# CV-Project2025/Project-NeRF

Measured on AMD Instinct MI355X. Metric: train rays/sec + 800x800 render FPS, NeRF-Synthetic Lego; PSNR parity, higher is better.
Workload: dtype bf16; 1 GPU; Part 2 vanilla NeRF train step (L10/L4 Fourier, 8x256 skip-4 MLP, view 128), batch sampling included; rays_per_gpu=4096, samples_per_ray=64, global_rays=4096, parallelism=ray-dp1, weights=random init (seed 0), frames=100 x 800x800 RGBA resident in HBM (uniform noise)

## Files before the change

### include/nerf_hip.h

```cpp
#ifndef NERF_HIP_H
#define NERF_HIP_H

#include <stddef.h>
#include <stdint.h>

#ifdef __cplusplus
extern "C" {
#endif

#define NERF_OK 0
#define NERF_EINVAL (-22)
#define NERF_ELAUNCH (-5)
#define NERF_ENOSYS (-38)

#define NERF_ABI_VERSION 12

typedef void* nerf_stream_t;

const char* nerf_last_error(void);
int nerf_abi_version(void);

int nerf_set_option(const char* name, int value);
int nerf_get_option(const char* name, int* value_out);

int nerf_sample_rays(const float* rays_o, const float* rays_d, const float* u,
                     int64_t n_rays, int n_samples, float near_plane, float far_plane,
                     float* z_out, float* pts_out, float* dirs_out, nerf_stream_t stream);

int nerf_gather_rays(const float* images, const float* poses, const int64_t* img_idx, const int64_t* pix_y,
                     const int64_t* pix_x, int64_t batch, int n_images, int H, int W, float focal,
                     float scene_scale, float* rays_o, float* rays_d, float* rgba, nerf_stream_t stream);

int nerf_gather_batch(const float* images, const float* poses, const int64_t* flat_idx, int64_t batch, int n_images,
                      int H, int W, float focal, float scene_scale, const float* bg, float* rays_o, float* rays_d,
                      float* rgba, float* target, nerf_stream_t stream);

int nerf_train_batch(const float* images, const float* poses, int n_images, int H, int W, float focal,
                     float scene_scale, const float* bg, uint64_t seed, uint64_t counter, int64_t batch,
                     int n_samples, float near_plane, float far_plane, int perturb, float* rays_o, float* rays_d,
                     float* rgba, float* target, float* z_out, nerf_stream_t stream);

int nerf_train_batch_shard(const float* images, const float* poses, int n_images, int H, int W, float focal,
                     float scene_scale, const float* bg, uint64_t seed, uint64_t counter, int64_t first_ray, int64_t batch,
                     int n_samples, float near_plane, float far_plane, int perturb, float* rays_o, float* rays_d,
                     float* rgba, float* target, float* z_out, nerf_stream_t stream);

int nerf_active_mask(const float* pts, int64_t n, const uint8_t* binary_grid, int resolution,
                     float bound, uint8_t* mask_out, int64_t* idx_out, nerf_stream_t stream);

int nerf_sample_compact(const float* rays_o, const float* rays_d, const float* u, int64_t n_rays,
                        int n_samples, float near_plane, float far_plane, const uint8_t* binary_grid,
                        int resolution, float bound, float* z_out, int* slot_of_sample, float* pts_compact,
                        float* dirs_compact, unsigned* active_count, nerf_stream_t stream);
int nerf_sample_compact_jitter(const float* rays_o, const float* rays_d, uint64_t seed, uint64_t counter,
                               int64_t n_rays, int n_samples, float near_plane, float far_plane,
                               const uint8_t* binary_grid, int resolution, float bound, float* z_out,
                               int* slot_of_sample, float* pts_compact, float* dirs_compact,
                               unsigned* active_count, nerf_stream_t stream);
int nerf_sample_compact_jitter_shard(const float* rays_o, const float* rays_d, uint64_t seed, uint64_t counter,
                                     int64_t first_ray, int64_t n_rays, int n_samples, float near_plane, float far_plane,
                                     const uint8_t* binary_grid, int resolution, float bound, float* z_out,
                                     int* slot_of_sample, float* pts_compact, float* dirs_compact,
                                     unsigned* active_count, nerf_stream_t stream);
#define NERF_COMPACT_CHAIN_WORDS 40
int nerf_sample_compact_jitter_chain(const float* rays_o, const float* rays_d, uint64_t seed, uint64_t counter,
                                     int64_t first_ray, int64_t n_rays, int n_samples, float near_plane, float far_plane,
                                     const uint8_t* binary_grid, int resolution, float bound, float* z_out,
                                     int* slot_of_sample, float* pts_compact, float* dirs_compact,
// ... 41 lines not shown
                        nerf_stream_t stream);

int nerf_composite_fwd(const float* rgb, const float* sigma, const float* z, const float* rays_d,
                       const float* bg, int64_t bg_rows, const float* extra,
                       int64_t n_rays, int n_samples,
                       float* out_rgb, float* out_depth, float* out_acc,
                       float* extra_map, float* weights_out, nerf_stream_t stream);

int nerf_composite_bwd(const float* rgb, const float* sigma, const float* z, const float* rays_d,
                       const float* bg, int64_t bg_rows, const float* extra,
                       const float* g_rgb, const float* g_depth, const float* g_acc,
                       const float* g_extra, int64_t n_rays, int n_samples,
                       float* d_rgb, float* d_sigma, float* d_extra, nerf_stream_t stream);

int nerf_composite_fwd_indexed(const float* rgb_compact, const float* sigma_compact, const int* slot_of_sample,
                               const float* z, const float* rays_d, const float* bg, int64_t bg_rows,
                               int64_t n_rays, int n_samples, float* out_rgb, float* out_depth,
                               float* out_acc, nerf_stream_t stream);
int nerf_composite_bwd_indexed(const float* rgb_compact, const float* sigma_compact, const int* slot_of_sample,
                               const float* z, const float* rays_d, const float* bg, int64_t bg_rows,
                               const float* g_rgb, const float* g_depth, const float* g_acc, int64_t n_rays,
                               int n_samples, float* d_rgb_compact, float* d_sigma_compact,
                               nerf_stream_t stream);

#define NERF_MLP_PARAM_COUNT 595844

size_t nerf_mlp_packed_bytes(void);
int nerf_mlp_pack(const float* params_f32, void* packed, nerf_stream_t stream);
int nerf_mlp_pack_streams(const float* params_f32, void* packed, int which, nerf_stream_t stream);

size_t nerf_mlp_stash_bytes(int64_t n);
int nerf_mlp_fwd(const void* packed, const float* rays_o, const float* rays_d, const float* z,
                 int64_t n, int n_samples, float* rgb, float* sigma, void* stash,
                 nerf_stream_t stream);

int nerf_mlp_fwd_encoded(const void* packed, const float* x_enc, const float* d_enc, int64_t n, float* rgb,
                         float* sigma, void* stash, nerf_stream_t stream);

size_t nerf_mlp_bwd_workspace_bytes(int64_t n);
int nerf_mlp_bwd(const void* packed, const void* stash, const float* rgb, const float* sigma,
                 const float* d_rgb, const float* d_sigma, int64_t n, float* grads_f32,
                 void* workspace, nerf_stream_t stream);
int nerf_mlp_bwd_dgrad(const void* packed, const void* stash, const float* rgb, const float* sigma,
                       const float* d_rgb, const float* d_sigma, int64_t n, void* workspace,
                       nerf_stream_t stream);
int nerf_mlp_bwd_dgrad_ex(const void* packed, const void* stash, const float* rgb, const float* sigma,
                          const float* d_rgb, const float* d_sigma, int64_t n, void* workspace,
                          const float* amax_dev, nerf_stream_t stream);
int64_t nerf_mlp_wgrad_part_split(void);
int nerf_mlp_bwd_wgrad_part(const void* stash, const void* workspace, int64_t n, float* grads_f32, int part,
                            nerf_stream_t stream);
int nerf_mlp_bwd_wgrad(const void* stash, const void* workspace, int64_t n, float* grads_f32,
                       nerf_stream_t stream);

int nerf_hash_encode_fwd(const float* pts, int64_t n, const float* table, int n_levels,
                         const float* scale_host, const unsigned* res_host, const unsigned* size_host,
                         const unsigned* offset_host, const unsigned* dense_host, float bound,
                         float* out_f32, void* out_nat_bf16, unsigned* idx_out, nerf_stream_t stream);
int nerf_hash_encode_fwd_f16(const float* pts, int64_t n, const void* table_f16, int n_levels,
                         const float* scale_host, const unsigned* res_host, const unsigned* size_host,
                         const unsigned* offset_host, const unsigned* dense_host, float bound,
                         float* out_f32, void* out_nat_bf16, nerf_stream_t stream);
int nerf_hash_encode_fwd_nat(const float* pts, int64_t n, const float* table_f32, const void* table_f16, int n_levels,
                             const float* scale_host, const unsigned* res_host, const unsigned* size_host,
                             const unsigned* offset_host, const unsigned* dense_host, float bound,
                             void* out_nat, int nat_dtype, nerf_stream_t stream);
int nerf_hash_encode_fwd_nat_tables(const float* pts, int64_t n, const void* tables_f16, int n_tables, int64_t table_stride,
                                    int n_levels, const float* scale_host, const unsigned* res_host, const unsigned* size_host,
                                    const unsigned* offset_host, const unsigned* dense_host, float bound, void* out_nat,
                                    int64_t out_stride_bytes, int nat_dtype, nerf_stream_t stream);
int nerf_f32_to_f16(const float* src, void* dst_f16, int64_t n, nerf_stream_t stream);
int nerf_hash_encode_bwd(const float* pts, int64_t n, int n_levels, const float* scale_host,
                         const unsigned* res_host, const unsigned* size_host, const unsigned* offset_host,
                         const unsigned* dense_host, float bound, const float* d_feat, float* d_table,
                         nerf_stream_t stream);
int nerf_hash_encode_bwd_levels(const float* pts, int64_t n, int n_levels, const float* scale_host,
                         const unsigned* res_host, const unsigned* size_host, const unsigned* offset_host,
                         const unsigned* dense_host, float bound, const float* d_feat, float* d_table, int first_level, int end_level,
                         nerf_stream_t stream);
size_t nerf_hash_encode_bwd_workspace_bytes(int64_t n, int n_levels);
int nerf_hash_encode_bwd_ws(const float* pts, int64_t n, int n_levels, const float* scale_host,
                         const unsigned* res_host, const unsigned* size_host, const unsigned* offset_host,
                         const unsigned* dense_host, float bound, const float* d_feat, float* d_table, int first_level, int end_level,
                         void* workspace, size_t workspace_bytes, nerf_stream_t stream);
int nerf_hash_encode_bwd_ws_store(const float* pts, int64_t n, int n_levels, const float* scale_host,
                                  const unsigned* res_host, const unsigned* size_host, const unsigned* offset_host,
                                  const unsigned* dense_host, float bound, const float* d_feat, float* d_table,
                                  int first_level, int end_level, void* workspace, size_t workspace_bytes,
                                  nerf_stream_t stream);
size_t nerf_hash_encode_bwd_tables_workspace_bytes(int64_t n, int n_levels, int n_tables);
int nerf_hash_encode_bwd_ws_store_tables(const float* pts, int64_t n, int n_tables, int64_t table_stride, int n_levels,
                                         const float* scale_host, const unsigned* res_host, const unsigned* size_host,
                                         const unsigned* offset_host, const unsigned* dense_host, float bound,
                                         const float* d_feat, int64_t dfeat_stride, float* d_table, void* workspace,
                                         size_t workspace_bytes, nerf_stream_t stream);
int nerf_hash_encode_bwd_ws_store_tables_spec(const float* pts, int64_t n, int n_tables, int64_t table_stride, int n_levels,
                                              const float* scale_host, const unsigned* res_host, const unsigned* size_host,
                                              const unsigned* offset_host, const unsigned* dense_host, float bound,
                                              const float* d_feat, int64_t dfeat_stride, float* d_table, void* workspace,
                                              size_t workspace_bytes, void* status_host, nerf_stream_t stream);
int nerf_hash_encode_fwd_f16_hist(const float* pts, int64_t n, const void* table_f16, int n_levels,
                                  const float* scale_host, const unsigned* res_host, const unsigned* size_host,
                                  const unsigned* offset_host, const unsigned* dense_host, float bound,
                                  void* out_nat_bf16, void* bwd_workspace, size_t bwd_workspace_bytes, nerf_stream_t stream);
#define NERF_AMAX_WORDS 32
int nerf_hash_encode_bwd_ws_slots(void* workspace, int64_t n, int n_levels, void** amax_bits_out, void** grad_lm_out);
// ... 21 lines not shown
int nerf_hash_encode_bwd_input_f16_accum(const float* pts, int64_t n, const void* table_f16, int n_levels,
                                         const float* scale_host, const unsigned* res_host, const unsigned* size_host,
                                         const unsigned* offset_host, const unsigned* dense_host, float bound,
                                         const float* d_feat, float* d_pts, nerf_stream_t stream);
int nerf_hash_encode_bwd_input_lm_f16(const float* pts, int64_t n, const void* table_f16, int n_levels,
                                      const float* scale_host, const unsigned* res_host, const unsigned* size_host,
                                      const unsigned* offset_host, const unsigned* dense_host, float bound,
                                      const void* grad_lm, float* d_pts, int accumulate, nerf_stream_t stream);


size_t nerf_imlp_packed_bytes(void);
size_t nerf_imlp_workspace_bytes(int64_t n);
size_t nerf_imlp_hash_operand_offset(int64_t n);
int nerf_imlp_pack(const float* params_f32, void* packed, nerf_stream_t stream);
int nerf_imlp_fwd(const void* packed, void* workspace, const float* dirs, int64_t n, float* rgb,
                  float* sigma, int train, nerf_stream_t stream);
int nerf_imlp_fwd_encoded(const void* packed, void* workspace, const float* x_enc, const float* d_enc, int64_t n,
                          float* rgb, float* sigma, int train, nerf_stream_t stream);
int nerf_imlp_bwd(const void* packed, void* workspace, const float* rgb, const float* sigma,
                  const float* d_rgb, const float* d_sigma, int64_t n, float* grads_f32,
                  float* d_feat, nerf_stream_t stream);
int nerf_imlp_bwd_lm(const void* packed, void* workspace, const float* rgb, const float* sigma,
                     const float* d_rgb, const float* d_sigma, int64_t n, float* grads_f32,
                     void* grad_lm, void* amax_bits, nerf_stream_t stream);

size_t nerf_render_rays_workspace_bytes(int64_t chunk_rays, int n_samples);
int nerf_render_rays_fwd(const void* packed, const float* rays_o, const float* rays_d, int64_t n_rays,
                         int n_samples, float near_plane, float far_plane, const float* bg, int64_t bg_rows,
                         int64_t chunk_rays, void* workspace, float* out_rgb, float* out_depth, float* out_acc,
                         nerf_stream_t stream);

size_t nerf_instant_render_workspace_bytes(int64_t chunk_rays, int n_samples);
int nerf_instant_render_rays_fwd(const void* imlp_packed, const float* table_f32, const void* table_f16, int n_levels,
                                 const float* scale_host, const unsigned* res_host, const unsigned* size_host,
                                 const unsigned* offset_host, const unsigned* dense_host, float hash_bound,
                                 const uint8_t* binary_grid, int grid_resolution, float grid_bound,
                                 const float* rays_o, const float* rays_d, int64_t n_rays, int n_samples,
                                 float near_plane, float far_plane, const float* bg, int64_t bg_rows,
                                 int64_t chunk_rays, void* workspace, float* out_rgb, float* out_depth, float* out_acc,
                                 nerf_stream_t stream);

size_t nerf_render_rays_grid_workspace_bytes(int64_t chunk_rays, int n_samples);
int nerf_render_rays_grid_fwd(const void* packed, const uint8_t* binary_grid, int grid_resolution, float grid_bound,
                              const float* rays_o, const float* rays_d, int64_t n_rays, int n_samples,
                              float near_plane, float far_plane, const float* bg, int64_t bg_rows,
                              int64_t chunk_rays, void* workspace, float* out_rgb, float* out_depth, float* out_acc,
                              nerf_stream_t stream);

#define NERF_SUM_WS_FLOATS 12288
int nerf_composite_mse_bwd(const float* rgb, const float* sigma, const int* slot_of_sample, const float* z,
                           const float* rays_d, const float* bg, int64_t bg_rows, const float* target,
                           float loss_weight, int64_t n_rays, int n_samples, float* pred_out, float* loss_accum,
                           float* d_rgb, float* d_sigma, float* amax_accum, float* sum_ws, nerf_stream_t stream);
int nerf_composite_mse_reg_bwd(const float* rgb, const float* sigma, const int* slot_of_sample, const float* z,
                               const float* rays_d, const float* bg, int64_t bg_rows, const float* target,
                               float loss_weight, const float* extra, float reg_weight, int64_t n_rays, int n_samples,
                               float* pred_out, float* extra_map, float* loss_accum, float* reg_accum, float* d_rgb,
                               float* d_sigma, float* d_extra, float* sum_ws, nerf_stream_t stream);

int nerf_adam_step(float* params, const float* grads, float* exp_avg, float* exp_avg_sq,
                   int64_t n, int step, float lr, float beta1, float beta2, float eps,
                   float weight_decay, const float* grad_scale_dev, nerf_stream_t stream);

#define NERF_NORMSQ_WS_FLOATS 4136
int nerf_tv_normsq(const float* params, float* grads, int64_t n, float tv_weight, float grad_scale,
                   float* normsq_dev, nerf_stream_t stream);
int nerf_tv_normsq_accum(const float* params, float* grads, int64_t n, float tv_weight, float grad_scale,
                         float* normsq_dev, nerf_stream_t stream);
int nerf_tv_normsq_accum_tables(const float* params, float* grads, int64_t n, int n_tables, float tv_weight, float grad_scale,
                                float* normsq_dev, nerf_stream_t stream);
int nerf_adamw_clip_step(float* params, const float* grads, float* exp_avg, float* exp_avg_sq, int64_t n,
                         int step, float lr, float beta1, float beta2, float eps, float weight_decay,
                         const float* normsq_dev, float max_norm, float grad_scale, nerf_stream_t stream);
int nerf_adamw_clip_step_shadow(float* params, const float* grads, float* exp_avg, float* exp_avg_sq, int64_t n,
                         int step, float lr, float beta1, float beta2, float eps, float weight_decay,
                         const float* normsq_dev, float max_norm, float grad_scale, void* params_f16_out, nerf_stream_t stream);

size_t nerf_tv_codes_bytes(int64_t n);
int nerf_tv_normsq_codes(const float* params, const float* grads, int64_t n, int n_tables, float tv_weight, float grad_scale,
                         float* normsq_dev, int accumulate, void* tv_codes, nerf_stream_t stream);
int nerf_adamw_clip_step_tv(float* params, const float* grads, float* exp_avg, float* exp_avg_sq, int64_t n, int step, float lr,
                            float beta1, float beta2, float eps, float weight_decay, const float* normsq_dev, float max_norm,
                            float grad_scale, const void* tv_codes, int64_t tv_split, float tv_weight_lo, int64_t seg_lo,
                            float tv_weight_hi, int64_t seg_hi, int64_t lr_split, float lr_hi, void* params_f16_out,
                            nerf_stream_t stream);

int nerf_tv_normsq_codes_piece(const float* params, const float* grads, int64_t n, int64_t table_elems, int halo, float tv_weight,
                               float grad_scale, float* normsq_dev, int accumulate, void* tv_codes, nerf_stream_t stream);
int nerf_adamw_clip_step_tv_piece(float* params, const float* grads, float* exp_avg, float* exp_avg_sq, int64_t n, int step, float lr,
                                  float beta1, float beta2, float eps, float weight_decay, const float* normsq_dev, float max_norm,
                                  float grad_scale, const void* tv_codes, float tv_weight, int64_t table_elems, int halo_lo,
                                  void* params_f16_out, nerf_stream_t stream);

int nerf_clip_adamw_small(float* params, float* grads, float* exp_avg, float* exp_avg_sq, int64_t n, int step, float lr, float beta1,
                          float beta2, float eps, float weight_decay, float max_norm, float grad_scale, float* normsq_out,
                          int zero_grads, nerf_stream_t stream);

int64_t nerf_p4_param_count(void);
size_t nerf_p4_packed_bytes(void);
size_t nerf_p4_workspace_bytes(int64_t n);
size_t nerf_p4_infer_workspace_bytes(int64_t n);
size_t nerf_p4_workspace_offset(int64_t n, int which);
int nerf_p4_pack(const float* params_f32, void* packed, nerf_stream_t stream);
int nerf_p4_sample_inputs(const int* slot_of_sample, const float* pts_compact, const float* ray_times, int64_t n_rays,
                          int n_samples, float coord_noise_std, float time_noise_std, uint64_t seed, uint64_t counter,
                          int64_t first_ray, float* x_deform, float* t_deform, nerf_stream_t stream);
int nerf_p4_deform_fwd(const void* packed, const float* params_f32, void* workspace, const float* pts, const float* t_deform,
                       const float* blend, int64_t n, float* delta_x, float* x_canonical, int train, nerf_stream_t stream);
int nerf_p4_canon_fwd(const void* packed, void* workspace, const float* t_deform, const float* dirs, int64_t n, float* rgb,
                      float* sigma, int train, nerf_stream_t stream);
int nerf_p4_canon_bwd(const void* packed, void* workspace, const float* rgb, const float* sigma, const float* d_rgb,
                      const float* d_sigma, int64_t n, float* grads_f32, void* amax_bits, void* grad_lm, nerf_stream_t stream);
int nerf_p4_deform_bwd(const void* packed, const float* params_f32, void* workspace, const float* d_delta_x, int64_t n,
                       float* grads_f32, void* amax_bits, void* grad_lm, nerf_stream_t stream);

// ... 58 lines not shown
```

### project-nerf_amd/_lib.py

```python
import ctypes
import os

_HERE = os.path.dirname(os.path.abspath(__file__))
LIB_PATH = os.path.join(_HERE, "libnerf_hip.so")

c_f32p = ctypes.c_void_p
c_ptr = ctypes.c_void_p
i64 = ctypes.c_int64
i32 = ctypes.c_int
f32 = ctypes.c_float
size_t = ctypes.c_size_t

PROTOTYPES = {
    "nerf_last_error": (ctypes.c_char_p, []),
    "nerf_abi_version": (i32, []),
    "nerf_set_option": (i32, [ctypes.c_char_p, i32]),
    "nerf_get_option": (i32, [ctypes.c_char_p, ctypes.POINTER(i32)]),
    "nerf_sample_rays": (i32, [c_ptr, c_ptr, c_ptr, i64, i32, f32, f32, c_ptr, c_ptr, c_ptr, c_ptr]),
    "nerf_gather_rays": (i32, [c_ptr, c_ptr, c_ptr, c_ptr, c_ptr, i64, i32, i32, i32, f32, f32, c_ptr, c_ptr, c_ptr, c_ptr]),
    "nerf_gather_batch": (i32, [c_ptr, c_ptr, c_ptr, i64, i32, i32, i32, f32, f32, c_ptr, c_ptr, c_ptr, c_ptr, c_ptr, c_ptr]),
    "nerf_train_batch": (i32, [c_ptr, c_ptr, i32, i32, i32, f32, f32, c_ptr, ctypes.c_uint64, ctypes.c_uint64, i64, i32, f32, f32,
                               i32, c_ptr, c_ptr, c_ptr, c_ptr, c_ptr, c_ptr]),
    "nerf_train_batch_shard": (i32, [c_ptr, c_ptr, i32, i32, i32, f32, f32, c_ptr, ctypes.c_uint64, ctypes.c_uint64, i64, i64, i32, f32, f32,
                                     i32, c_ptr, c_ptr, c_ptr, c_ptr, c_ptr, c_ptr]),
    "nerf_active_mask": (i32, [c_ptr, i64, c_ptr, i32, f32, c_ptr, c_ptr, c_ptr]),
    "nerf_sample_compact": (i32, [c_ptr, c_ptr, c_ptr, i64, i32, f32, f32, c_ptr, i32, f32, c_ptr, c_ptr, c_ptr, c_ptr, c_ptr, c_ptr]),
    "nerf_sample_compact_jitter": (i32, [c_ptr, c_ptr, ctypes.c_uint64, ctypes.c_uint64, i64, i32, f32, f32, c_ptr, i32, f32,
                                         c_ptr, c_ptr, c_ptr, c_ptr, c_ptr, c_ptr]),
    "nerf_sample_compact_jitter_shard": (i32, [c_ptr, c_ptr, ctypes.c_uint64, ctypes.c_uint64, i64, i64, i32, f32, f32, c_ptr, i32, f32,
                                               c_ptr, c_ptr, c_ptr, c_ptr, c_ptr, c_ptr]),
    "nerf_sample_compact_jitter_chain": (i32, [c_ptr, c_ptr, ctypes.c_uint64, ctypes.c_uint64, i64, i64, i32, f32, f32, c_ptr, i32, f32,
                                               c_ptr, c_ptr, c_ptr, c_ptr, c_ptr, i32, c_ptr, ctypes.c_uint32, c_ptr]),
    "nerf_train_batch_compact": (i32, [c_ptr, c_ptr, i32, i32, i32, f32, f32, c_ptr, ctypes.c_uint64, ctypes.c_uint64, i64, i64, i32, f32, f32,
                                       c_ptr, i32, f32, c_ptr, c_ptr, c_ptr, c_ptr, c_ptr, c_ptr, c_ptr, c_ptr, c_ptr, c_ptr]),
    "nerf_train_batch_compact_chain": (i32, [c_ptr, c_ptr, i32, i32, i32, f32, f32, c_ptr, ctypes.c_uint64, ctypes.c_uint64, i64, i64, i32, f32,
                                             f32, c_ptr, i32, f32, c_ptr, c_ptr, c_ptr, c_ptr, c_ptr, c_ptr, c_ptr, c_ptr, c_ptr, i32, c_ptr,
                                             ctypes.c_uint32, c_ptr]),
    "nerf_composite_fwd_indexed": (i32, [c_ptr, c_ptr, c_ptr, c_ptr, c_ptr, c_ptr, i64, i64, i32, c_ptr, c_ptr, c_ptr, c_ptr]),
    "nerf_composite_bwd_indexed": (i32, [c_ptr, c_ptr, c_ptr, c_ptr, c_ptr, c_ptr, i64, c_ptr, c_ptr, c_ptr, i64, i32, c_ptr, c_ptr, c_ptr]),
    "nerf_sample_pdf": (i32, [c_ptr, c_ptr, c_ptr, i64, i32, i32, c_ptr, c_ptr]),
    "nerf_grid_lattice": (i32, [f32, i32, c_ptr, c_ptr]),
    "nerf_grid_update": (i32, [c_ptr, c_ptr, c_ptr, i64, f32, i32, f32, c_ptr, c_ptr]),
    "nerf_instant_grid_update_workspace_bytes": (size_t, [i64]),
    "nerf_instant_grid_update": (i32, [c_ptr, c_ptr, c_ptr, i32, c_ptr, c_ptr, c_ptr, c_ptr, c_ptr, f32, c_ptr, i64, i32, f32, c_ptr, c_ptr, f32, i32,
                                       f32, c_ptr, i64, c_ptr, c_ptr]),
    "nerf_fourier_encode": (i32, [c_ptr, i64, i32, i32, c_ptr, c_ptr]),
    "nerf_composite_fwd": (i32, [c_ptr, c_ptr, c_ptr, c_ptr, c_ptr, i64, c_ptr, i64, i32,
                                 c_ptr, c_ptr, c_ptr, c_ptr, c_ptr, c_ptr]),
    "nerf_composite_bwd": (i32, [c_ptr, c_ptr, c_ptr, c_ptr, c_ptr, i64, c_ptr, c_ptr, c_ptr, c_ptr,
                                 c_ptr, i64, i32, c_ptr, c_ptr, c_ptr, c_ptr]),
    "nerf_render_rays_workspace_bytes": (size_t, [i64, i32]),
    "nerf_render_rays_fwd": (i32, [c_ptr, c_ptr, c_ptr, i64, i32, f32, f32, c_ptr, i64, i64, c_ptr, c_ptr, c_ptr, c_ptr, c_ptr]),
    "nerf_instant_render_workspace_bytes": (size_t, [i64, i32]),
    "nerf_instant_render_rays_fwd": (i32, [c_ptr, c_ptr, c_ptr, i32, c_ptr, c_ptr, c_ptr, c_ptr, c_ptr, f32, c_ptr, i32, f32, c_ptr, c_ptr, i64, i32,
                                           f32, f32, c_ptr, i64, i64, c_ptr, c_ptr, c_ptr, c_ptr, c_ptr]),
    "nerf_render_rays_grid_workspace_bytes": (size_t, [i64, i32]),
    "nerf_render_rays_grid_fwd": (i32, [c_ptr, c_ptr, i32, f32, c_ptr, c_ptr, i64, i32, f32, f32, c_ptr, i64, i64, c_ptr, c_ptr, c_ptr, c_ptr,
                                        c_ptr]),
    "nerf_mlp_packed_bytes": (size_t, []),
    "nerf_mlp_pack": (i32, [c_ptr, c_ptr, c_ptr]),
    "nerf_mlp_pack_streams": (i32, [c_ptr, c_ptr, i32, c_ptr]),
    "nerf_mlp_stash_bytes": (size_t, [i64]),
    "nerf_mlp_fwd": (i32, [c_ptr, c_ptr, c_ptr, c_ptr, i64, i32, c_ptr, c_ptr, c_ptr, c_ptr]),
    "nerf_mlp_fwd_encoded": (i32, [c_ptr, c_ptr, c_ptr, i64, c_ptr, c_ptr, c_ptr, c_ptr]),
    "nerf_mlp_bwd_workspace_bytes": (size_t, [i64]),
    "nerf_mlp_bwd": (i32, [c_ptr, c_ptr, c_ptr, c_ptr, c_ptr, c_ptr, i64, c_ptr, c_ptr, c_ptr]),
    "nerf_mlp_bwd_dgrad": (i32, [c_ptr, c_ptr, c_ptr, c_ptr, c_ptr, c_ptr, i64, c_ptr, c_ptr]),
    "nerf_mlp_bwd_wgrad": (i32, [c_ptr, c_ptr, i64, c_ptr, c_ptr]),
    "nerf_mlp_bwd_dgrad_ex": (i32, [c_ptr, c_ptr, c_ptr, c_ptr, c_ptr, c_ptr, i64, c_ptr, c_ptr, c_ptr]),
    "nerf_composite_mse_bwd": (i32, [c_ptr, c_ptr, c_ptr, c_ptr, c_ptr, c_ptr, i64, c_ptr, f32, i64, i32, c_ptr, c_ptr,
                                     c_ptr, c_ptr, c_ptr, c_ptr, c_ptr]),
    "nerf_mlp_wgrad_part_split": (i64, []),
    "nerf_mlp_bwd_wgrad_part": (i32, [c_ptr, c_ptr, i64, c_ptr, i32, c_ptr]),
    "nerf_hash_encode_fwd": (i32, [c_ptr, i64, c_ptr, i32, c_ptr, c_ptr, c_ptr, c_ptr, c_ptr, f32, c_ptr, c_ptr, c_ptr, c_ptr]),
    "nerf_hash_encode_fwd_f16": (i32, [c_ptr, i64, c_ptr, i32, c_ptr, c_ptr, c_ptr, c_ptr, c_ptr, f32, c_ptr, c_ptr, c_ptr]),
    "nerf_hash_encode_fwd_nat": (i32, [c_ptr, i64, c_ptr, c_ptr, i32, c_ptr, c_ptr, c_ptr, c_ptr, c_ptr, f32, c_ptr, i32, c_ptr]),
    "nerf_hash_encode_fwd_nat_tables": (i32, [c_ptr, i64, c_ptr, i32, i64, i32, c_ptr, c_ptr, c_ptr, c_ptr, c_ptr, f32, c_ptr, i64, i32, c_ptr]),
    "nerf_f32_to_f16": (i32, [c_ptr, c_ptr, i64, c_ptr]),
    "nerf_hash_encode_bwd": (i32, [c_ptr, i64, i32, c_ptr, c_ptr, c_ptr, c_ptr, c_ptr, f32, c_ptr, c_ptr, c_ptr]),
    "nerf_hash_encode_bwd_levels": (i32, [c_ptr, i64, i32, c_ptr, c_ptr, c_ptr, c_ptr, c_ptr, f32, c_ptr, c_ptr, i32, i32, c_ptr]),
    "nerf_hash_encode_bwd_workspace_bytes": (size_t, [i64, i32]),
    "nerf_hash_encode_bwd_ws": (i32, [c_ptr, i64, i32, c_ptr, c_ptr, c_ptr, c_ptr, c_ptr, f32, c_ptr, c_ptr, i32, i32, c_ptr, size_t, c_ptr]),
    "nerf_hash_encode_bwd_ws_store": (i32, [c_ptr, i64, i32, c_ptr, c_ptr, c_ptr, c_ptr, c_ptr, f32, c_ptr, c_ptr, i32, i32, c_ptr, size_t, c_ptr]),
    "nerf_hash_encode_bwd_tables_workspace_bytes": (size_t, [i64, i32, i32]),
    "nerf_hash_encode_bwd_ws_store_tables": (i32, [c_ptr, i64, i32, i64, i32, c_ptr, c_ptr, c_ptr, c_ptr, c_ptr, f32, c_ptr, i64, c_ptr, c_ptr, size_t, c_ptr]),
    "nerf_hash_encode_bwd_ws_store_tables_spec": (i32, [c_ptr, i64, i32, i64, i32, c_ptr, c_ptr, c_ptr, c_ptr, c_ptr, f32, c_ptr, i64, c_ptr, c_ptr, size_t,
                                                        c_ptr, c_ptr]),
    "nerf_hash_encode_fwd_f16_hist": (i32, [c_ptr, i64, c_ptr, i32, c_ptr, c_ptr, c_ptr, c_ptr, c_ptr, f32, c_ptr, c_ptr, size_t, c_ptr]),
    "nerf_hash_encode_bwd_ws_slots": (i32, [c_ptr, i64, i32, ctypes.POINTER(c_ptr), ctypes.POINTER(c_ptr)]),
    "nerf_hash_encode_bwd_ws_store_precounted": (i32, [c_ptr, i64, i32, c_ptr, c_ptr, c_ptr, c_ptr, c_ptr, f32, c_ptr, c_ptr, size_t, c_ptr]),
    "nerf_hash_encode_bwd_spec_begin": (i32, [c_ptr, c_ptr]),
    "nerf_hash_encode_bwd_ws_store_spec": (i32, [c_ptr, i64, i32, c_ptr, c_ptr, c_ptr, c_ptr, c_ptr, f32, c_ptr, c_ptr, c_ptr, size_t, c_ptr, c_ptr]),
    "nerf_imlp_bwd_amax": (i32, [c_ptr, c_ptr, c_ptr, c_ptr, c_ptr, c_ptr, i64, c_ptr, c_ptr, c_ptr, c_ptr]),
    "nerf_hash_encode_bwd_spec_status": (c_ptr, [c_ptr]),
    "nerf_imlp_bwd_lm": (i32, [c_ptr, c_ptr, c_ptr, c_ptr, c_ptr, c_ptr, i64, c_ptr, c_ptr, c_ptr, c_ptr]),
    "nerf_hash_encode_bwd_input": (i32, [c_ptr, i64, c_ptr, i32, c_ptr, c_ptr, c_ptr, c_ptr, c_ptr, f32, c_ptr, c_ptr, c_ptr]),
    "nerf_hash_encode_bwd_input_f16": (i32, [c_ptr, i64, c_ptr, i32, c_ptr, c_ptr, c_ptr, c_ptr, c_ptr, f32, c_ptr, c_ptr, c_ptr]),
    "nerf_hash_encode_bwd_input_f16_accum": (i32, [c_ptr, i64, c_ptr, i32, c_ptr, c_ptr, c_ptr, c_ptr, c_ptr, f32, c_ptr, c_ptr, c_ptr]),
    "nerf_hash_encode_bwd_input_lm_f16": (i32, [c_ptr, i64, c_ptr, i32, c_ptr, c_ptr, c_ptr, c_ptr, c_ptr, f32, c_ptr, c_ptr, i32, c_ptr]),
    "nerf_imlp_packed_bytes": (size_t, []),
    "nerf_imlp_workspace_bytes": (size_t, [i64]),
    "nerf_imlp_hash_operand_offset": (size_t, [i64]),
    "nerf_imlp_pack": (i32, [c_ptr, c_ptr, c_ptr]),
    "nerf_imlp_fwd": (i32, [c_ptr, c_ptr, c_ptr, i64, c_ptr, c_ptr, i32, c_ptr]),
    "nerf_imlp_fwd_encoded": (i32, [c_ptr, c_ptr, c_ptr, c_ptr, i64, c_ptr, c_ptr, i32, c_ptr]),
    "nerf_imlp_bwd": (i32, [c_ptr, c_ptr, c_ptr, c_ptr, c_ptr, c_ptr, i64, c_ptr, c_ptr, c_ptr]),
    "nerf_adam_step": (i32, [c_ptr, c_ptr, c_ptr, c_ptr, i64, i32, f32, f32, f32, f32, f32, c_ptr, c_ptr]),
    "nerf_tv_normsq": (i32, [c_ptr, c_ptr, i64, f32, f32, c_ptr, c_ptr]),
    "nerf_tv_normsq_accum": (i32, [c_ptr, c_ptr, i64, f32, f32, c_ptr, c_ptr]),
    "nerf_tv_normsq_accum_tables": (i32, [c_ptr, c_ptr, i64, i32, f32, f32, c_ptr, c_ptr]),
    "nerf_composite_mse_reg_bwd": (i32, [c_ptr, c_ptr, c_ptr, c_ptr, c_ptr, c_ptr, i64, c_ptr, f32, c_ptr, f32, i64, i32, c_ptr, c_ptr,
                                         c_ptr, c_ptr, c_ptr, c_ptr, c_ptr, c_ptr, c_ptr]),
    "nerf_sample_compact_ordered_scratch_bytes": (size_t, [i64, i32]),
    "nerf_sample_compact_ordered": (i32, [c_ptr, c_ptr, c_ptr, i32, ctypes.c_uint64, ctypes.c_uint64, i64, i64, i32, f32, f32, c_ptr, i32, f32,
                                          c_ptr, c_ptr, c_ptr, c_ptr, c_ptr, c_ptr, size_t, c_ptr]),
    "nerf_p4_param_count": (i64, []),
    "nerf_p4_packed_bytes": (size_t, []),
    "nerf_p4_workspace_bytes": (size_t, [i64]),
    "nerf_p4_infer_workspace_bytes": (size_t, [i64]),
    "nerf_p4_workspace_offset": (size_t, [i64, i32]),
    "nerf_p4_pack": (i32, [c_ptr, c_ptr, c_ptr]),
    "nerf_p4_sample_inputs": (i32, [c_ptr, c_ptr, c_ptr, i64, i32, f32, f32, ctypes.c_uint64, ctypes.c_uint64, i64, c_ptr, c_ptr, c_ptr]),
    "nerf_p4_deform_fwd": (i32, [c_ptr, c_ptr, c_ptr, c_ptr, c_ptr, c_ptr, i64, c_ptr, c_ptr, i32, c_ptr]),
    "nerf_p4_canon_fwd": (i32, [c_ptr, c_ptr, c_ptr, c_ptr, i64, c_ptr, c_ptr, i32, c_ptr]),
    "nerf_p4_canon_bwd": (i32, [c_ptr, c_ptr, c_ptr, c_ptr, c_ptr, c_ptr, i64, c_ptr, c_ptr, c_ptr, c_ptr]),
    "nerf_p4_deform_bwd": (i32, [c_ptr, c_ptr, c_ptr, c_ptr, i64, c_ptr, c_ptr, c_ptr, c_ptr]),
    "nerf_p3_deform_param_count": (i64, []),
    "nerf_p3_deform_packed_bytes": (size_t, []),
    "nerf_p3_deform_workspace_bytes": (size_t, [i64]),
    "nerf_p3_deform_pack": (i32, [c_ptr, c_ptr, c_ptr]),
    "nerf_p3_deform_fwd": (i32, [c_ptr, c_ptr, c_ptr, c_ptr, c_ptr, i64, c_ptr, c_ptr, i32, c_ptr]),
    "nerf_p3_deform_bwd": (i32, [c_ptr, c_ptr, c_ptr, i64, c_ptr, c_ptr]),
    "nerf_p3_canon_param_count": (i64, [i32]),
    "nerf_p3_canon_packed_bytes": (size_t, []),
    "nerf_p3_canon_workspace_bytes": (size_t, [i64]),
    "nerf_p3_canon_pack": (i32, [c_ptr, i32, c_ptr, c_ptr]),
    "nerf_p3_canon_fwd": (i32, [c_ptr, c_ptr, c_ptr, c_ptr, c_ptr, i64, c_ptr, c_ptr, i32, c_ptr]),
    "nerf_p3_canon_bwd": (i32, [c_ptr, c_ptr, c_ptr, c_ptr, c_ptr, c_ptr, c_ptr, i64, i32, c_ptr, c_ptr, c_ptr]),
    "nerf_p1_param_count": (i64, [i32, i32, i32, i32]),
    "nerf_p1_packed_bytes": (size_t, [i32, i32, i32, i32]),
    "nerf_p1_workspace_bytes": (size_t, [i64, i32, i32, i32, i32]),
    "nerf_p1_pack": (i32, [c_ptr, i32, i32, i32, i32, c_ptr, c_ptr]),
    "nerf_p1_fwd": (i32, [c_ptr, c_ptr, i64, i32, i32, i32, i32, c_ptr, c_ptr]),
    "nerf_p1_fwd_loss_bwd": (i32, [c_ptr, c_ptr, c_ptr, c_ptr, c_ptr, i64, i32, i32, i32, i32, c_ptr, c_ptr, c_ptr]),
    "nerf_p2_param_count": (i64, [i32] * 6),
    "nerf_p2_packed_bytes": (size_t, [i32] * 6),
    "nerf_p2_workspace_bytes": (size_t, [i64] + [i32] * 6),
    "nerf_p2_pack": (i32, [c_ptr] + [i32] * 6 + [c_ptr, c_ptr]),
    "nerf_p2_fwd": (i32, [c_ptr, c_ptr, c_ptr, c_ptr, i64, i32] + [i32] * 6 + [c_ptr, c_ptr, c_ptr]),
    "nerf_p2_fwd_train": (i32, [c_ptr, c_ptr, c_ptr, c_ptr, c_ptr, i64, i32] + [i32] * 6 + [c_ptr, c_ptr, c_ptr]),
    "nerf_p2_bwd": (i32, [c_ptr, c_ptr, c_ptr, c_ptr, c_ptr, c_ptr, i64] + [i32] * 6 + [c_ptr, c_ptr]),
    "nerf_imlp_shape_param_count": (i64, [i32] * 3),
    "nerf_imlp_shape_packed_bytes": (size_t, [i32] * 3),
    "nerf_imlp_shape_workspace_bytes": (size_t, [i64] + [i32] * 3),
    "nerf_imlp_shape_hash_operand_offset": (size_t, [i64] + [i32] * 3),
    "nerf_imlp_shape_pack": (i32, [c_ptr] + [i32] * 3 + [c_ptr, c_ptr]),
    "nerf_imlp_shape_fwd": (i32, [c_ptr, c_ptr, c_ptr, i64] + [i32] * 3 + [c_ptr, c_ptr, i32, c_ptr]),
    "nerf_imlp_shape_bwd": (i32, [c_ptr, c_ptr, c_ptr, c_ptr, c_ptr, c_ptr, i64] + [i32] * 3 + [c_ptr, c_ptr, c_ptr]),
    "nerf_tv_codes_bytes": (size_t, [i64]),
    "nerf_tv_normsq_codes": (i32, [c_ptr, c_ptr, i64, i32, f32, f32, c_ptr, i32, c_ptr, c_ptr]),
    "nerf_clip_adamw_small": (i32, [c_ptr, c_ptr, c_ptr, c_ptr, i64, i32, f32, f32, f32, f32, f32, f32, f32, c_ptr, i32, c_ptr]),
    "nerf_adamw_clip_step_tv": (i32, [c_ptr, c_ptr, c_ptr, c_ptr, i64, i32, f32, f32, f32, f32, f32, c_ptr, f32, f32, c_ptr, i64, f32, i64,
                                      f32, i64, i64, f32, c_ptr, c_ptr]),
    "nerf_tv_normsq_codes_piece": (i32, [c_ptr, c_ptr, i64, i64, i32, f32, f32, c_ptr, i32, c_ptr, c_ptr]),
    "nerf_adamw_clip_step_tv_piece": (i32, [c_ptr, c_ptr, c_ptr, c_ptr, i64, i32, f32, f32, f32, f32, f32, c_ptr, f32, f32, c_ptr, f32, i64, i32,
                                            c_ptr, c_ptr]),
    "nerf_adamw_clip_step": (i32, [c_ptr, c_ptr, c_ptr, c_ptr, i64, i32, f32, f32, f32, f32, f32, c_ptr, f32, f32, c_ptr]),
    "nerf_adamw_clip_step_shadow": (i32, [c_ptr, c_ptr, c_ptr, c_ptr, i64, i32, f32, f32, f32, f32, f32, c_ptr, f32, f32, c_ptr, c_ptr]),
}

ABI_VERSION = 12

_lib = None


class NerfHipError(RuntimeError):
    pass


def load():
    global _lib
    if _lib is not None:
        return _lib
    if not os.path.exists(LIB_PATH):
        raise NerfHipError(
            f"{LIB_PATH} not found: build it with `python project-nerf_amd/build.py` "
            "(hipcc --offload-arch=gfx950).  There is no fallback path.")
    import torch
    lib = ctypes.CDLL(LIB_PATH, mode=ctypes.RTLD_GLOBAL)
    for name, (res, args) in PROTOTYPES.items():
        fn = getattr(lib, name)
        fn.restype = res
        fn.argtypes = args
    if lib.nerf_abi_version() != ABI_VERSION:
        raise NerfHipError(f"ABI version mismatch: {LIB_PATH} reports {lib.nerf_abi_version()}, this binding was written against "
                           f"{ABI_VERSION} (rebuild with `python project-nerf_amd/build.py`)")
    _lib = lib
    return lib


NORMSQ_WS_FLOATS = 4136
COMPACT_CHAIN_WORDS = 40
SUM_WS_FLOATS = 12288


def set_option(name: str, value: int) -> None:
    check(load().nerf_set_option(name.encode(), int(value)), f"nerf_set_option({name})")


def get_option(name: str) -> int:
    out = i32(0)
    check(load().nerf_get_option(name.encode(), ctypes.byref(out)), f"nerf_get_option({name})")
    return out.value


def check(code, what):
    if code != 0:
        msg = load().nerf_last_error().decode("utf-8", "replace")
        raise NerfHipError(f"{what} failed ({code}): {msg}")
```

### project-nerf_amd/csrc/adam.hip

```cpp
#include "common.h"

namespace nerf {

typedef float f4 __attribute__((ext_vector_type(4)));

__device__ __forceinline__ void adam_update(float& p, float g, float& m, float& v, float lr, float beta1, float beta2,
                                            float eps, float wd, float inv_bc1, float inv_sqrt_bc2) {
  float pi = p;
  if (wd != 0.0f) pi *= (1.0f - lr * wd);
  const float mi = beta1 * m + (1.0f - beta1) * g;
  const float vi = beta2 * v + (1.0f - beta2) * g * g;
  m = mi;
  v = vi;
  p = pi - (lr * inv_bc1) * (mi / (sqrtf(vi) * inv_sqrt_bc2 + eps));
}

template <bool VEC>
__device__ __forceinline__ void adam_sweep(float* __restrict__ p, const float* __restrict__ g, float* __restrict__ m,
                                           float* __restrict__ v, int64_t n, float gs, float lr, float beta1, float beta2,
                                           float eps, float wd, float inv_bc1, float inv_sqrt_bc2, _Float16* __restrict__ shadow = nullptr) {
  const int64_t tid = blockIdx.x * (int64_t)blockDim.x + threadIdx.x, stride = (int64_t)gridDim.x * blockDim.x;
  const int64_t n4 = VEC ? n / 4 : 0;
  for (int64_t i = tid; i < n4; i += stride) {
    f4 pp = reinterpret_cast<f4*>(p)[i], mm = reinterpret_cast<f4*>(m)[i], vv = reinterpret_cast<f4*>(v)[i];
    const f4 gg = reinterpret_cast<const f4*>(g)[i];
#pragma unroll
    for (int e = 0; e < 4; ++e) {
      float pe = pp[e], me = mm[e], ve = vv[e];
      adam_update(pe, gg[e] * gs, me, ve, lr, beta1, beta2, eps, wd, inv_bc1, inv_sqrt_bc2);
      pp[e] = pe; mm[e] = me; vv[e] = ve;
    }
    reinterpret_cast<f4*>(m)[i] = mm;
    reinterpret_cast<f4*>(v)[i] = vv;
    reinterpret_cast<f4*>(p)[i] = pp;
    if (shadow != nullptr) {
      typedef _Float16 h4 __attribute__((ext_vector_type(4)));
      h4 hh = {(_Float16)pp[0], (_Float16)pp[1], (_Float16)pp[2], (_Float16)pp[3]};
      reinterpret_cast<h4*>(shadow)[i] = hh;
    }
  }
  for (int64_t i = 4 * n4 + tid; i < n; i += stride) {
    adam_update(p[i], g[i] * gs, m[i], v[i], lr, beta1, beta2, eps, wd, inv_bc1, inv_sqrt_bc2);
    if (shadow != nullptr) shadow[i] = (_Float16)p[i];
  }
}

template <bool VEC>
__global__ void __launch_bounds__(256)
adam_kernel(float* __restrict__ p, const float* __restrict__ g, float* __restrict__ m,
            float* __restrict__ v, int64_t n, float lr, float beta1, float beta2, float eps, float wd,
            float inv_bc1, float inv_sqrt_bc2, const float* __restrict__ grad_scale) {
  adam_sweep<VEC>(p, g, m, v, n, grad_scale ? *grad_scale : 1.0f, lr, beta1, beta2, eps, wd, inv_bc1, inv_sqrt_bc2);
}

__host__ inline bool aligned16(const void* a, const void* b, const void* c, const void* d) {
  return (((uintptr_t)a | (uintptr_t)b | (uintptr_t)c | (uintptr_t)d) & 15) == 0;
}

}

extern "C" int nerf_adam_step(float* params, const float* grads, float* exp_avg, float* exp_avg_sq,
                              int64_t n, int step, float lr, float beta1, float beta2, float eps,
                              float weight_decay, const float* grad_scale_dev, nerf_stream_t stream) {
  NERF_REQUIRE(n >= 0 && step >= 1, "nerf_adam_step: n=%lld step=%d", (long long)n, step);
  if (n == 0) return NERF_OK;
  NERF_REQUIRE(params && grads && exp_avg && exp_avg_sq, "nerf_adam_step: NULL pointer");
  const double bc1 = 1.0 - pow((double)beta1, step), bc2 = 1.0 - pow((double)beta2, step);
  int64_t blocks = (n / 4 + 255) / 256 + 1;
  if (blocks > 2048) blocks = 2048;
  if (nerf::aligned16(params, grads, exp_avg, exp_avg_sq))
    hipLaunchKernelGGL(nerf::adam_kernel<true>, dim3((int)blocks), dim3(256), 0, nerf::as_stream(stream), params,
                       grads, exp_avg, exp_avg_sq, n, lr, beta1, beta2, eps, weight_decay,
                       (float)(1.0 / bc1), (float)(1.0 / sqrt(bc2)), grad_scale_dev);
  else
    hipLaunchKernelGGL(nerf::adam_kernel<false>, dim3((int)blocks), dim3(256), 0, nerf::as_stream(stream), params,
                       grads, exp_avg, exp_avg_sq, n, lr, beta1, beta2, eps, weight_decay,
                       (float)(1.0 / bc1), (float)(1.0 / sqrt(bc2)), grad_scale_dev);
  return nerf::check_launch("nerf_adam_step");
}

namespace nerf {

__device__ __forceinline__ float sgn(float x) { return (x > 0.0f) - (x < 0.0f); }

__device__ __forceinline__ float tv_term(float prev, float cur, float next, bool has_prev, bool has_next) {
  float t = 0.0f;
  if (has_prev) t += sgn(cur - prev);
  if (has_next) t -= sgn(next - cur);
  return t;
}

template <bool VEC>
__global__ void __launch_bounds__(256)
tv_normsq_kernel(const float* __restrict__ p, float* __restrict__ g, int64_t n, float tv_scale, float grad_scale,
                 float* __restrict__ normsq, int64_t seg) {
  auto starts = [seg](int64_t e) { return e == 0 || e == seg || e == 2 * seg || e == 3 * seg; };
  const bool rewrite = tv_scale != 0.0f || grad_scale != 1.0f;
  float local = 0.0f;
  const int64_t tid = blockIdx.x * (int64_t)blockDim.x + threadIdx.x, stride = (int64_t)gridDim.x * blockDim.x;
  const int64_t n4 = VEC ? n / 4 : 0;
  for (int64_t i = tid; i < n4; i += stride) {
    f4 gg = reinterpret_cast<f4*>(g)[i];
    gg[0] *= grad_scale; gg[1] *= grad_scale; gg[2] *= grad_scale; gg[3] *= grad_scale;
    if (tv_scale != 0.0f) {
      const f4 pp = reinterpret_cast<const f4*>(p)[i];
      const int64_t e0 = 4 * i;
      const bool has_prev = !starts(e0), has_next = e0 + 4 < n && !starts(e0 + 4);
      const float before = has_prev ? p[e0 - 1] : 0.0f, after = has_next ? p[e0 + 4] : 0.0f;
      gg[0] += tv_scale * tv_term(before, pp[0], pp[1], has_prev, true);
      gg[1] += tv_scale * tv_term(pp[0], pp[1], pp[2], true, true);
      gg[2] += tv_scale * tv_term(pp[1], pp[2], pp[3], true, true);
      gg[3] += tv_scale * tv_term(pp[2], pp[3], after, true, has_next);
    }
    if (rewrite) reinterpret_cast<f4*>(g)[i] = gg;
    local += gg[0] * gg[0] + gg[1] * gg[1] + gg[2] * gg[2] + gg[3] * gg[3];
  }
  for (int64_t i = 4 * n4 + tid; i < n; i += stride) {
    float gi = g[i] * grad_scale;
    if (tv_scale != 0.0f) {
      const bool has_prev = !starts(i), has_next = i + 1 < n && !starts(i + 1);
      gi += tv_scale * tv_term(has_prev ? p[i - 1] : 0.0f, p[i], has_next ? p[i + 1] : 0.0f, has_prev, has_next);
    }
    if (rewrite) g[i] = gi;
    local += gi * gi;
  }
  __shared__ float part[4];
  local = wave_sum(local);
  if ((threadIdx.x & 63) == 0) part[threadIdx.x >> 6] = local;
  __syncthreads();
  const float val[1] = {(part[0] + part[1]) + (part[2] + part[3])};
// ... 445 lines not shown
```

### project-nerf_amd/csrc/api.cpp

```cpp
#include <stdlib.h>
#include <string.h>
#include <mutex>
#include "common.h"

namespace nerf {
static thread_local char g_err[512] = "";

int fail(int code, const char* fmt, ...) {
  va_list ap;
  va_start(ap, fmt);
  vsnprintf(g_err, sizeof(g_err), fmt, ap);
  va_end(ap);
  return code;
}

struct OptionSlot { const char* name; const char* env; int Options::*field; };
static const OptionSlot kSlots[] = {
    {"chain_legacy", "NERF_CHAIN_LEGACY", &Options::chain_legacy},
    {"fwd_cycles", "NERF_FWD_CYCLES", &Options::fwd_cycles},
    {"wgrad_overhead", "NERF_WGRAD_OVH", &Options::wgrad_overhead},
    {"wgrad_bw_x16", "NERF_WGRAD_BW", &Options::wgrad_bw_x16},
    {"wgrad_fixed", "NERF_WGRAD_FIXED", &Options::wgrad_fixed},
    {"wgrad_debug", "NERF_WGRAD_DEBUG", &Options::wgrad_debug},
    {"wgrad_small_span", "NERF_WGRAD_SMALL_SPAN", &Options::wgrad_small_span},
    {"wgrad_small_cap", "NERF_WGRAD_SMALL_CAP", &Options::wgrad_small_cap},
    {"wgrad_only", "NERF_WGRAD_ONLY", &Options::wgrad_only},
    {"hash_bwd_only_level", "NERF_HASH_BWD_ONLY_LEVEL", &Options::hash_bwd_only_level},
    {"hash_bwd_atomic", "NERF_HASH_BWD_ATOMIC", &Options::hash_bwd_atomic},
    {"wgrad_atomic", "NERF_WGRAD_ATOMIC", &Options::wgrad_atomic},
    {"wgrad_k16", "NERF_WGRAD_K16", &Options::wgrad_k16},
    {"wgrad_big_only", "NERF_WGRAD_BIG_ONLY", &Options::wgrad_big_only},
    {"infer_shape32", "NERF_INFER_SHAPE32", &Options::infer_shape32},
    {"infer64", "NERF_INFER64", &Options::infer64},
    {"stash_fp8", "NERF_STASH_FP8", &Options::stash_fp8},
    {"chain_grid", "NERF_CHAIN_GRID", &Options::chain_grid},
    {"wgrad_grid", "NERF_WGRAD_GRID", &Options::wgrad_grid},
    {"hash_fwd_lds_kb", "NERF_HASH_FWD_LDS_KB", &Options::hash_fwd_lds_kb},
    {"hash_xcd", "NERF_HASH_XCD", &Options::hash_xcd},
    {"composite_wgs_per_cu", "NERF_COMPOSITE_WGS", &Options::composite_wgs_per_cu},
    {"deterministic", "NERF_DETERMINISTIC", &Options::deterministic},
    {"tv_blocks", "NERF_TV_BLOCKS", &Options::tv_blocks},
};

Options& options() {
  static Options o;
  static std::once_flag once;
  std::call_once(once, [] {
    for (const OptionSlot& s : kSlots)
      if (const char* v = getenv(s.env)) o.*(s.field) = (*v == 0) ? 1 : atoi(v);
  });
  return o;
}

namespace {
constexpr int kMaxDevices = 64, kMaxKernels = 64;
struct DeviceFacts {
  int n_cu = 0;
  int n_kernels = 0;
  const void* kernels[kMaxKernels];
};
DeviceFacts g_dev[kMaxDevices];
std::mutex g_dev_mutex;
}

int device_cu_count(int* n_cu) {
  int dev = 0;
  if (hipGetDevice(&dev) != hipSuccess || dev < 0 || dev >= kMaxDevices) return fail(NERF_ELAUNCH, "cannot query the current device");
  std::lock_guard<std::mutex> lock(g_dev_mutex);
  if (g_dev[dev].n_cu == 0) {
    hipDeviceProp_t prop;
    if (hipGetDeviceProperties(&prop, dev) != hipSuccess) return fail(NERF_ELAUNCH, "cannot query device %d", dev);
    g_dev[dev].n_cu = prop.multiProcessorCount;
  }
  *n_cu = g_dev[dev].n_cu;
  return NERF_OK;
}

int ensure_dynamic_lds(const void* kernel, int bytes, const char* what) {
  int dev = 0;
  if (hipGetDevice(&dev) != hipSuccess || dev < 0 || dev >= kMaxDevices) return fail(NERF_ELAUNCH, "cannot query the current device");
  std::lock_guard<std::mutex> lock(g_dev_mutex);
  DeviceFacts& d = g_dev[dev];
  for (int i = 0; i < d.n_kernels; ++i)
    if (d.kernels[i] == kernel) return NERF_OK;
  if (hipFuncSetAttribute(kernel, hipFuncAttributeMaxDynamicSharedMemorySize, bytes) != hipSuccess)
    return fail(NERF_ELAUNCH, "%s: cannot raise the dynamic LDS limit to %d on device %d", what, bytes, dev);
  if (d.n_kernels < kMaxKernels) d.kernels[d.n_kernels++] = kernel;
  return NERF_OK;
}
}

extern "C" const char* nerf_last_error(void) { return nerf::g_err; }
extern "C" int nerf_abi_version(void) { return NERF_ABI_VERSION; }

// ... 20 lines not shown
```

### project-nerf_amd/csrc/common.h

```cpp
#pragma once
#include <hip/hip_runtime.h>
#include <stdarg.h>
#include <stdint.h>
#include <stdio.h>
#include "../../include/nerf_hip.h"

namespace nerf {

constexpr int kWave = 64;

int fail(int code, const char* fmt, ...);

inline int check_launch(const char* what) {
  hipError_t e = hipGetLastError();
  if (e != hipSuccess) return fail(NERF_ELAUNCH, "%s: %s", what, hipGetErrorString(e));
  return NERF_OK;
}

inline hipStream_t as_stream(nerf_stream_t s) { return reinterpret_cast<hipStream_t>(s); }

struct Options {
  int chain_legacy = 0;
  int fwd_cycles = 0;
  int wgrad_overhead = 98304;
  int wgrad_bw_x16 = 192;
  int wgrad_fixed = 2000;
  int wgrad_debug = 0;
  int wgrad_small_span = 32;
  int wgrad_small_cap = 3;
  int wgrad_only = -1;
  int hash_bwd_only_level = -1;
  int wgrad_big_only = 0;
  int wgrad_k16 = 0;
  int wgrad_atomic = 0;
  int hash_bwd_atomic = 0;
  int infer_shape32 = 0;
  int infer64 = 1;
  int stash_fp8 = 0;
  int chain_grid = 0;
  int wgrad_grid = 0;
  int composite_wgs_per_cu = 2;
  int hash_xcd = 1;
  int hash_fwd_lds_kb = 36;
  int tv_blocks = 0;
  int deterministic = 0;
};
Options& options();

int device_cu_count(int* n_cu);
int ensure_dynamic_lds(const void* kernel, int bytes, const char* what);

int hash_fwd_counted(const float* pts, const unsigned* count, int64_t capacity, const float* table_f32, const void* table_f16,
                     int n_levels, const float* scale_host, const unsigned* res_host, const unsigned* size_host,
                     const unsigned* offset_host, const unsigned* dense_host, float bound, void* out_nat, nerf_stream_t stream);
int imlp_fwd_counted(const void* packed, const void* hash_nat, const float* dirs, const unsigned* count, int64_t capacity, float* rgb,
                     float* sigma, nerf_stream_t stream);
int hash_fwd_lattice(int64_t cell0, int64_t n_cells, int resolution, float grid_bound, const float* table_f32, const void* table_f16,
                     int n_levels, const float* scale_host, const unsigned* res_host, const unsigned* size_host,
                     const unsigned* offset_host, const unsigned* dense_host, float bound, void* out_nat, nerf_stream_t stream);
int imlp_sigma_grid(const void* packed, const void* hash_nat, int64_t n_cells, float* grid, uint8_t* binary_grid, float decay, int dynamic,
                    float threshold, unsigned long long* active_count, nerf_stream_t stream);
int mlp_fwd_counted(const void* packed, const float* pts, const float* dirs, const unsigned* count, int64_t capacity, float* rgb,
                    float* sigma, nerf_stream_t stream);

#define NERF_REQUIRE(cond, ...) \
  do {                          \
    if (!(cond)) return ::nerf::fail(NERF_EINVAL, __VA_ARGS__); \
  } while (0)

__device__ __forceinline__ uint32_t squares32(uint64_t ctr, uint64_t key) {
  uint64_t x = ctr * key, y = x, z = y + key;
  x = x * x + y; x = (x >> 32) | (x << 32);
  x = x * x + z; x = (x >> 32) | (x << 32);
  x = x * x + y; x = (x >> 32) | (x << 32);
  return (uint32_t)((x * x + z) >> 32);
}

inline uint64_t squares_key(uint64_t seed) {
  uint64_t key = seed + 0x9E3779B97F4A7C15ull;
  key = (key ^ (key >> 30)) * 0xBF58476D1CE4E5B9ull;
  key = (key ^ (key >> 27)) * 0x94D049BB133111EBull;
  return (key ^ (key >> 31)) | 1ull;
}
__device__ __forceinline__ float squares_uniform(uint64_t counter, uint64_t index, uint64_t key) {
  return (float)(squares32((counter << 40) + index, key) >> 8) * 5.9604644775390625e-08f;
}

__device__ __forceinline__ float mul_rn(float a, float b) {
#pragma clang fp contract(off)
  return a * b;
}
__device__ __forceinline__ float add_rn(float a, float b) {
#pragma clang fp contract(off)
  return a + b;
}
__device__ __forceinline__ float sub_rn(float a, float b) {
#pragma clang fp contract(off)
// ... 111 lines not shown
```

### project-nerf_amd/csrc/composite.hip

```cpp
#include "common.h"

namespace nerf {

constexpr int kMaxPerLane = 16;

template <int K>
struct RayCtx {
  float e[K];
  float alpha[K];
  float q[K];
  float T[K];
  float z[K];
  float delta[K];
};

__device__ __forceinline__ int64_t row_of(const int* __restrict__ slots, int64_t dense_index) {
  return slots == nullptr ? dense_index : (int64_t)slots[dense_index];
}

template <int K>
__device__ __forceinline__ void ray_setup(const float* __restrict__ sigma, const float* __restrict__ z,
                                          const float* __restrict__ rays_d, const int* __restrict__ slots,
                                          int64_t r, int S, int lane, RayCtx<K>& c, float* sig_out, int64_t* row_out) {
  const float dx = rays_d[r * 3 + 0], dy = rays_d[r * 3 + 1], dz = rays_d[r * 3 + 2];
  const float dnorm = sqrtf(dx * dx + dy * dy + dz * dz);
  const int s0 = lane * K;
  float zn[K + 1];
#pragma unroll
  for (int k = 0; k <= K; ++k) {
    const int s = s0 + k;
    zn[k] = s < S ? z[r * S + s] : 0.0f;
  }
  float local = 1.0f;
#pragma unroll
  for (int k = 0; k < K; ++k) {
    const int s = s0 + k;
    const bool valid = s < S;
    const int64_t row = valid ? row_of(slots, r * S + s) : -1;
    row_out[k] = row;
    const float sg = row >= 0 ? sigma[row] : 0.0f;
    sig_out[k] = sg;
    float dl = (s < S - 1) ? (zn[k + 1] - zn[k]) : 1e10f;
    dl = dl * dnorm;
    const float e = valid ? expf(-sg * dl) : 1.0f;
    c.z[k] = zn[k];
    c.delta[k] = dl;
    c.e[k] = e;
    c.alpha[k] = 1.0f - e;
    c.q[k] = valid ? (1.0f - c.alpha[k] + 1e-10f) : 1.0f;
    local *= c.q[k];
  }
  const float incl = wave_inclusive_prod(local);
  float run = dpp_row_shr<1>(incl, 1.0f);
// ... 227 lines not shown
          }
          float* o = d_rgb + row[k] * 3;
          const float d0 = w[k] * gr0, d1 = w[k] * gr1, d2 = w[k] * gr2;
          o[0] = d0; o[1] = d1; o[2] = d2;
          if (amax_out != nullptr)
            amax = fmaxf(amax, fmaxf(fabsf(d0 * col[k][0] * (1.0f - col[k][0])),
                                     fmaxf(fabsf(d1 * col[k][1] * (1.0f - col[k][1])), fabsf(d2 * col[k][2] * (1.0f - col[k][2])))));
        }
        G[k] = g;
        local += g * w[k];
      }
    }
    float after = wave_exclusive_suffix_sum(local);
#pragma unroll
    for (int k = K - 1; k >= 0; --k) {
      const int s = lane * K + k;
      if (s < S && row[k] >= 0) {
        const float dalpha = G[k] * c.T[k] - after / c.q[k];
        const float ds = dalpha * c.delta[k] * c.e[k];
        d_sigma[row[k]] = ds;
        if (amax_out != nullptr && sg[k] > 0.0f) amax = fmaxf(amax, fabsf(ds));
      }
      after += G[k] * w[k];
    }
  }
  __shared__ float part[12];
  loss_local = wave_sum(loss_local);
  reg_local = wave_sum(reg_local);
#pragma unroll
  for (int off = 32; off > 0; off >>= 1) amax = fmaxf(amax, __shfl_xor(amax, off));
  if (lane == 0) { part[threadIdx.x >> 6] = loss_local; part[4 + (threadIdx.x >> 6)] = amax; part[8 + (threadIdx.x >> 6)] = reg_local; }
  __syncthreads();
  if (sum_ws != nullptr) {
    if (threadIdx.x == 0) {
      float* ws = reinterpret_cast<float*>(sum_ws);
      ws[blockIdx.x] = (part[0] + part[1]) + (part[2] + part[3]);
      ws[gridDim.x + blockIdx.x] = (part[8] + part[9]) + (part[10] + part[11]);
      ws[2 * gridDim.x + blockIdx.x] = fmaxf(fmaxf(part[4], part[5]), fmaxf(part[6], part[7]));
    }
    return;
  }
  if (threadIdx.x == 0) {
    atomicAdd(loss_out, (part[0] + part[1]) + (part[2] + part[3]));
    if (reg_out != nullptr) atomicAdd(reg_out, (part[8] + part[9]) + (part[10] + part[11]));
    if (amax_out != nullptr) {
      const float m = fmaxf(fmaxf(part[4], part[5]), fmaxf(part[6], part[7]));
      if (m == m && m < 3.0e38f) atomicMax(reinterpret_cast<unsigned*>(amax_out), __builtin_bit_cast(unsigned, m));
    }
  }
}

__global__ void __launch_bounds__(256) composite_sums_kernel(const float* __restrict__ ws, int n_blocks, float* __restrict__ loss_out,
                                                             float* __restrict__ reg_out, float* __restrict__ amax_out) {
  __shared__ float part[3][4];
  float s0 = 0.0f, s1 = 0.0f, m = 0.0f;
  for (int b = threadIdx.x; b < n_blocks; b += 256) {
    s0 += ws[b];
    s1 += ws[n_blocks + b];
    const float v = ws[2 * n_blocks + b];
    if (v == v && v < 3.0e38f) m = fmaxf(m, v);
  }
  s0 = wave_sum(s0);
  s1 = wave_sum(s1);
#pragma unroll
  for (int off = 32; off > 0; off >>= 1) m = fmaxf(m, __shfl_xor(m, off));
  if ((threadIdx.x & 63) == 0) { part[0][threadIdx.x >> 6] = s0; part[1][threadIdx.x >> 6] = s1; part[2][threadIdx.x >> 6] = m; }
  __syncthreads();
  if (threadIdx.x == 0) {
    *loss_out += (part[0][0] + part[0][1]) + (part[0][2] + part[0][3]);
    if (reg_out != nullptr) *reg_out += (part[1][0] + part[1][1]) + (part[1][2] + part[1][3]);
    if (amax_out != nullptr) *amax_out = fmaxf(*amax_out, fmaxf(fmaxf(part[2][0], part[2][1]), fmaxf(part[2][2], part[2][3])));
  }
}

static int per_lane(int S) {
  const int k = (S + 63) / 64;
  return k <= 4 ? k : (k <= 6 ? 6 : (k <= 8 ? 8 : (k <= 12 ? 12 : 16)));
}

}

using namespace nerf;

#define DISPATCH_K(K, KERNEL, ...)                                                        \
  switch (K) {                                                                            \
    case 1: hipLaunchKernelGGL(KERNEL<1>, grid, dim3(256), 0, as_stream(stream), __VA_ARGS__); break; \
    case 2: hipLaunchKernelGGL(KERNEL<2>, grid, dim3(256), 0, as_stream(stream), __VA_ARGS__); break; \
    case 3: hipLaunchKernelGGL(KERNEL<3>, grid, dim3(256), 0, as_stream(stream), __VA_ARGS__); break; \
    case 4: hipLaunchKernelGGL(KERNEL<4>, grid, dim3(256), 0, as_stream(stream), __VA_ARGS__); break; \
    case 6: hipLaunchKernelGGL(KERNEL<6>, grid, dim3(256), 0, as_stream(stream), __VA_ARGS__); break; \
    case 8: hipLaunchKernelGGL(KERNEL<8>, grid, dim3(256), 0, as_stream(stream), __VA_ARGS__); break; \
    case 12: hipLaunchKernelGGL(KERNEL<12>, grid, dim3(256), 0, as_stream(stream), __VA_ARGS__); break; \
    default: hipLaunchKernelGGL(KERNEL<16>, grid, dim3(256), 0, as_stream(stream), __VA_ARGS__); break; \
  }

static int composite_fwd_impl(const float* rgb, const float* sigma, const float* z, const float* rays_d,
                              const float* bg, int64_t bg_rows, const float* extra, const int* slots,
                              int64_t n_rays, int n_samples, float* out_rgb, float* out_depth, float* out_acc,
                              float* extra_map, float* weights_out, nerf_stream_t stream) {
  NERF_REQUIRE(n_rays >= 0 && n_samples >= 1 && n_samples <= 64 * kMaxPerLane,
               "nerf_composite_fwd: n_rays=%lld n_samples=%d (max %d)", (long long)n_rays, n_samples,
               64 * kMaxPerLane);
  if (n_rays == 0) return NERF_OK;
  NERF_REQUIRE(rgb && sigma && z && rays_d && out_rgb && out_depth && out_acc,
               "nerf_composite_fwd: NULL pointer");
  NERF_REQUIRE(bg == nullptr || bg_rows == 1 || bg_rows == n_rays, "nerf_composite_fwd: bg_rows=%lld",
               (long long)bg_rows);
  NERF_REQUIRE((extra == nullptr) == (extra_map == nullptr), "nerf_composite_fwd: extra/extra_map mismatch");
  int64_t blocks = (n_rays + 3) / 4;
  if (blocks > 256 * 8) blocks = 256 * 8;
  const dim3 grid((int)blocks);
  DISPATCH_K(per_lane(n_samples), composite_fwd_kernel, rgb, sigma, z, rays_d, bg, bg_rows, extra, slots, n_rays,
             n_samples, out_rgb, out_depth, out_acc, extra_map, weights_out);
  return check_launch("nerf_composite_fwd");
}

extern "C" int nerf_composite_fwd(const float* rgb, const float* sigma, const float* z,
                                  const float* rays_d, const float* bg, int64_t bg_rows,
                                  const float* extra, int64_t n_rays, int n_samples, float* out_rgb,
                                  float* out_depth, float* out_acc, float* extra_map,
                                  float* weights_out, nerf_stream_t stream) {
  return composite_fwd_impl(rgb, sigma, z, rays_d, bg, bg_rows, extra, nullptr, n_rays, n_samples, out_rgb, out_depth,
                            out_acc, extra_map, weights_out, stream);
}

extern "C" int nerf_composite_fwd_indexed(const float* rgb_compact, const float* sigma_compact, const int* slot_of_sample,
                                          const float* z, const float* rays_d, const float* bg, int64_t bg_rows,
                                          int64_t n_rays, int n_samples, float* out_rgb, float* out_depth,
                                          float* out_acc, nerf_stream_t stream) {
  NERF_REQUIRE(n_rays == 0 || slot_of_sample != nullptr, "nerf_composite_fwd_indexed: slot map is NULL");
  return composite_fwd_impl(rgb_compact, sigma_compact, z, rays_d, bg, bg_rows, nullptr, slot_of_sample, n_rays, n_samples,
                            out_rgb, out_depth, out_acc, nullptr, nullptr, stream);
}

static int composite_bwd_impl(const float* rgb, const float* sigma, const float* z, const float* rays_d,
                              const float* bg, int64_t bg_rows, const float* extra, const float* g_rgb,
                              const float* g_depth, const float* g_acc, const float* g_extra, const int* slots,
                              int64_t n_rays, int n_samples, float* d_rgb, float* d_sigma, float* d_extra,
                              nerf_stream_t stream) {
  NERF_REQUIRE(n_rays >= 0 && n_samples >= 1 && n_samples <= 64 * kMaxPerLane,
               "nerf_composite_bwd: n_rays=%lld n_samples=%d", (long long)n_rays, n_samples);
  if (n_rays == 0) return NERF_OK;
  NERF_REQUIRE(rgb && sigma && z && rays_d && g_rgb && d_rgb && d_sigma, "nerf_composite_bwd: NULL pointer");
  NERF_REQUIRE(bg == nullptr || bg_rows == 1 || bg_rows == n_rays, "nerf_composite_bwd: bg_rows=%lld",
               (long long)bg_rows);
  int64_t blocks = (n_rays + 3) / 4;
  if (blocks > 256 * 8) blocks = 256 * 8;
  const dim3 grid((int)blocks);
  DISPATCH_K(per_lane(n_samples), composite_bwd_kernel, rgb, sigma, z, rays_d, bg, bg_rows, extra, g_rgb,
             g_depth, g_acc, g_extra, slots, n_rays, n_samples, d_rgb, d_sigma, d_extra);
  return check_launch("nerf_composite_bwd");
}

extern "C" int nerf_composite_bwd(const float* rgb, const float* sigma, const float* z,
                                  const float* rays_d, const float* bg, int64_t bg_rows,
                                  const float* extra, const float* g_rgb, const float* g_depth,
                                  const float* g_acc, const float* g_extra, int64_t n_rays,
                                  int n_samples, float* d_rgb, float* d_sigma, float* d_extra,
                                  nerf_stream_t stream) {
  return composite_bwd_impl(rgb, sigma, z, rays_d, bg, bg_rows, extra, g_rgb, g_depth, g_acc, g_extra, nullptr, n_rays,
                            n_samples, d_rgb, d_sigma, d_extra, stream);
}

extern "C" int nerf_composite_bwd_indexed(const float* rgb_compact, const float* sigma_compact, const int* slot_of_sample,
                                          const float* z, const float* rays_d, const float* bg, int64_t bg_rows,
                                          const float* g_rgb, const float* g_depth, const float* g_acc, int64_t n_rays,
                                          int n_samples, float* d_rgb_compact, float* d_sigma_compact,
                                          nerf_stream_t stream) {
  NERF_REQUIRE(n_rays == 0 || slot_of_sample != nullptr, "nerf_composite_bwd_indexed: slot map is NULL");
  return composite_bwd_impl(rgb_compact, sigma_compact, z, rays_d, bg, bg_rows, nullptr, g_rgb, g_depth, g_acc, nullptr,
                            slot_of_sample, n_rays, n_samples, d_rgb_compact, d_sigma_compact, nullptr, stream);
}

static int64_t mse_blocks(int64_t n_rays, bool partials) {
  int n_cu = 256;
  (void)device_cu_count(&n_cu);
  const int per_cu = partials ? 8 : (options().composite_wgs_per_cu < 1 ? 1 : options().composite_wgs_per_cu);
  int64_t cap = (int64_t)n_cu * per_cu;
  if (cap > kOrderedSumMaxBlocks) cap = kOrderedSumMaxBlocks;
  const int64_t blocks = (n_rays + 3) / 4;
  return blocks < cap ? blocks : cap;
}
static int finish_sums(const float* sum_ws, unsigned n_blocks, float* loss, float* reg, float* amax, nerf_stream_t stream) {
  static_assert(NERF_SUM_WS_FLOATS >= 3 * kOrderedSumMaxBlocks, "three partials per workgroup");
  if (sum_ws == nullptr) return NERF_OK;
  hipLaunchKernelGGL(composite_sums_kernel, dim3(1), dim3(256), 0, as_stream(stream), sum_ws, (int)n_blocks, loss, reg, amax);
  return check_launch("nerf_composite_mse_bwd (sums)");
}

extern "C" int nerf_composite_mse_bwd(const float* rgb, const float* sigma, const int* slot_of_sample, const float* z,
                                      const float* rays_d, const float* bg, int64_t bg_rows, const float* target,
                                      float loss_weight, int64_t n_rays, int n_samples, float* pred_out, float* loss_accum,
                                      float* d_rgb, float* d_sigma, float* amax_accum, float* sum_ws, nerf_stream_t stream) {
  NERF_REQUIRE(n_rays >= 0 && n_samples >= 1 && n_samples <= 64 * kMaxPerLane,
               "nerf_composite_mse_bwd: n_rays=%lld n_samples=%d (max %d)", (long long)n_rays, n_samples, 64 * kMaxPerLane);
  if (n_rays == 0) return NERF_OK;
  NERF_REQUIRE(rgb && sigma && z && rays_d && target && loss_accum && d_rgb && d_sigma, "nerf_composite_mse_bwd: NULL pointer");
  NERF_REQUIRE(bg == nullptr || bg_rows == 1 || bg_rows == n_rays, "nerf_composite_mse_bwd: bg_rows=%lld", (long long)bg_rows);
  const dim3 grid((unsigned)mse_blocks(n_rays, sum_ws != nullptr));
  DISPATCH_K(per_lane(n_samples), composite_mse_bwd_kernel, rgb, sigma, z, rays_d, bg, bg_rows, target, loss_weight,
             slot_of_sample, n_rays, n_samples, pred_out, loss_accum, d_rgb, d_sigma, amax_accum,
             (const float*)nullptr, 0.0f, (float*)nullptr, (float*)nullptr, (float*)nullptr, reinterpret_cast<unsigned*>(sum_ws));
  if (int rc = check_launch("nerf_composite_mse_bwd"); rc != NERF_OK) return rc;
  return finish_sums(sum_ws, grid.x, loss_accum, nullptr, amax_accum, stream);
}

extern "C" int nerf_composite_mse_reg_bwd(const float* rgb, const float* sigma, const int* slot_of_sample, const float* z,
                                          const float* rays_d, const float* bg, int64_t bg_rows, const float* target,
                                          float loss_weight, const float* extra, float reg_weight, int64_t n_rays, int n_samples,
                                          float* pred_out, float* extra_map, float* loss_accum, float* reg_accum, float* d_rgb,
                                          float* d_sigma, float* d_extra, float* sum_ws, nerf_stream_t stream) {
  NERF_REQUIRE(n_rays >= 0 && n_samples >= 1 && n_samples <= 64 * kMaxPerLane,
               "nerf_composite_mse_reg_bwd: n_rays=%lld n_samples=%d (max %d)", (long long)n_rays, n_samples, 64 * kMaxPerLane);
  if (n_rays == 0) return NERF_OK;
  NERF_REQUIRE(rgb && sigma && z && rays_d && target && loss_accum && d_rgb && d_sigma && extra && d_extra && reg_accum,
               "nerf_composite_mse_reg_bwd: NULL pointer");
  NERF_REQUIRE(bg == nullptr || bg_rows == 1 || bg_rows == n_rays, "nerf_composite_mse_reg_bwd: bg_rows=%lld", (long long)bg_rows);
  const dim3 grid((unsigned)mse_blocks(n_rays, sum_ws != nullptr));
  DISPATCH_K(per_lane(n_samples), composite_mse_bwd_kernel, rgb, sigma, z, rays_d, bg, bg_rows, target, loss_weight,
             slot_of_sample, n_rays, n_samples, pred_out, loss_accum, d_rgb, d_sigma, (float*)nullptr, extra, reg_weight, d_extra,
             reg_accum, extra_map, reinterpret_cast<unsigned*>(sum_ws));
  if (int rc = check_launch("nerf_composite_mse_reg_bwd"); rc != NERF_OK) return rc;
  return finish_sums(sum_ws, grid.x, loss_accum, reg_accum, nullptr, stream);
}
```

### project-nerf_amd/csrc/mlp_bwd.hip

```cpp
#include "mlp_chain_body.h"
#include "mlp_stash.h"

namespace nerf {
using namespace plan;

struct BwdArgs {
  const char* packed;
  const float* rgb;
  const float* sigma;
  const float* d_rgb;
  const float* d_sigma;
  int64_t n, n_pad;
  const uint4* st_mask;
  __bf16* dsmall;
  __bf16* dhv;
  __bf16* dfeat;
  __bf16* dh;
  float* amax;
  const float* amax_src;
};

__global__ void __launch_bounds__(256) bwd_amax_kernel(const BwdArgs a) {
  float m = 0.0f;
  for (int64_t n = blockIdx.x * 256 + threadIdx.x; n < a.n; n += (int64_t)gridDim.x * 256) {
    float g0, g1, g2, gs;
    out_derivs(a, n, g0, g1, g2, gs);
    m = fmaxf(fmaxf(m, fabsf(g0)), fmaxf(fmaxf(fabsf(g1), fabsf(g2)), fabsf(gs)));
  }
#pragma unroll
  for (int off = 32; off > 0; off >>= 1) m = fmaxf(m, __shfl_xor(m, off));
  __shared__ float part[4];
  if ((threadIdx.x & 63) == 0) part[threadIdx.x >> 6] = m;
  __syncthreads();
  if (threadIdx.x == 0) {
    m = fmaxf(fmaxf(part[0], part[1]), fmaxf(part[2], part[3]));
    if (m == m && m < 3.0e38f) atomicMax(reinterpret_cast<unsigned*>(a.amax), __builtin_bit_cast(unsigned, m));
  }
}

__global__ void __launch_bounds__(kChainThreads, 2) mlp_bwd_kernel(const BwdArgs a) {
  extern __shared__ __attribute__((aligned(16))) char smem[];
  const int tid = threadIdx.x, lane = tid & 63;
  const int wave = __builtin_amdgcn_readfirstlane(tid >> 6);
  const int col = lane & 31, half = lane >> 5;
  chain_dgrad<kPackBwdOff>(a, smem, tid, lane, wave, col, half);
}

}

#include <stddef.h>
#include "mlp_stream_asm.h"

namespace nerf {

// ... 14 lines not shown
  asm volatile("s_waitcnt vmcnt(0)" ::: "memory");
  __syncthreads();

  const unsigned ab0 = lds_addr(smem + kBiasLdsBytes) + 16u * lane, ab1 = ab0 + kRingSlotBytes;
  const unsigned ldsw = __builtin_amdgcn_readfirstlane(lds_addr(smem + kBiasLdsBytes) + 1024u * wave);
  const unsigned voff = 1024u * wave + 16u * lane;
  const char* src = a.packed + kPackBwdOff;
  const void* karg = (const void*)__builtin_amdgcn_kernarg_segment_ptr();

  float gscale = 1.0f;
  if constexpr (!IMG16) {
    set_fp8_saturate();
    const float amax_in = *a.amax_src;
    if (a.amax_src != a.amax && blockIdx.x == 0 && tid == 0) *a.amax = amax_in;
    gscale = __builtin_bit_cast(float, __builtin_amdgcn_readfirstlane(__builtin_bit_cast(int, grad_image_scale(amax_in))));
  }
  const int64_t n_tiles = a.n_pad / kTileSamples;
  for (int64_t tile = blockIdx.x; tile < n_tiles; tile += gridDim.x) {
    const int64_t wave_tile = tile * 8 + wave;
    const int64_t n = wave_tile * kWaveSamples + col;
    const bool live = n < a.n;
    float g0 = 0.f, g1 = 0.f, g2 = 0.f, gs = 0.f;
    if (live) out_derivs(a, n, g0, g1, g2, gs);
    bf16x8 small, in_rgb, in_sigma;
#pragma unroll
    for (int j = 0; j < 8; ++j) small[j] = in_sigma[j] = (__bf16)0.0f;
    if (half == 0) {
      small[0] = (__bf16)g0; small[1] = (__bf16)g1; small[2] = (__bf16)g2; small[3] = (__bf16)gs;
      in_sigma[0] = (__bf16)gs;
    }
    if constexpr (IMG16) stash_nat(a.dsmall, wave_tile, 1, 0, col, half, small);
    else stash_nat8<true>(reinterpret_cast<char*>(a.dsmall), wave_tile, 1, 0, col, half, small, gscale);
    in_rgb = small;
    in_rgb[3] = (__bf16)0.0f;

    const unsigned lane32 = IMG16 ? block_lane_offset(col, half) : block8_lane_offset(col, half);
    const unsigned blk = IMG16 ? 2048u : 1024u;
    const unsigned so8 = (unsigned)wave_tile * (8u * blk) + lane32, so4 = (unsigned)wave_tile * (4u * blk) + lane32;
    const unsigned mo0 = (unsigned)tile * (72u * 512u * 2u) + 2u * tid;
    const bool more = tile + gridDim.x < n_tiles;
    const unsigned mo0n = more ? (unsigned)(tile + gridDim.x) * (72u * 512u * 2u) + 2u * tid : mo0;
    const unsigned first = __builtin_amdgcn_readfirstlane(tile == (int64_t)blockIdx.x ? 1u : 0u);
    if constexpr (IMG16) bwd16_stream_pass(ab0, ab1, in_rgb, in_sigma, src, voff, ldsw, so8, so4, mo0, mo0n, first, karg, gscale);
    else bwd_stream_pass(ab0, ab1, in_rgb, in_sigma, src, voff, ldsw, so8, so4, mo0, mo0n, first, karg, gscale);
  }
  asm volatile("s_waitcnt vmcnt(0)" ::: "memory");
}

}

using namespace nerf;

int nerf_launch_wgrad(const char* stash, const StashLayout& sl, const char* work, const BwdLayout& bl,
                      int64_t n, float* grads, int part, hipStream_t stream, size_t zero_lo, size_t zero_hi);

extern "C" size_t nerf_mlp_bwd_workspace_bytes(int64_t n) { return n > 0 ? bwd_layout(n).total : 0; }

static int launch_dgrad(const void* packed, const void* stash, const float* rgb, const float* sigma,
                        const float* d_rgb, const float* d_sigma, int64_t n, void* workspace,
                        const float* amax_dev, nerf_stream_t stream) {
  NERF_REQUIRE(n > 0 && n < (int64_t)1 << 31, "nerf_mlp_bwd: n=%lld out of range", (long long)n);
  NERF_REQUIRE(packed && stash && rgb && sigma && d_rgb && d_sigma && workspace, "nerf_mlp_bwd: NULL pointer");
  NERF_REQUIRE(((uintptr_t)packed & 255) == 0 && ((uintptr_t)stash & 255) == 0 && ((uintptr_t)workspace & 255) == 0,
               "nerf_mlp_bwd: packed/stash/workspace must be 256-byte aligned");
  const StashLayout sl = stash_layout(n);
  const BwdLayout bl = bwd_layout(n);
  BwdArgs a{};
  a.packed = static_cast<const char*>(packed);
  a.rgb = rgb; a.sigma = sigma; a.d_rgb = d_rgb; a.d_sigma = d_sigma;
  a.n = n; a.n_pad = bl.n_pad;
  a.st_mask = reinterpret_cast<const uint4*>(static_cast<const char*>(stash) + sl.mask);
  char* w = static_cast<char*>(workspace);
  a.dsmall = reinterpret_cast<__bf16*>(w + bl.dsmall);
  a.dhv = reinterpret_cast<__bf16*>(w + bl.dhv);
  a.dfeat = reinterpret_cast<__bf16*>(w + bl.dfeat);
  a.dh = reinterpret_cast<__bf16*>(w + bl.dh);
  a.amax = reinterpret_cast<float*>(w + bl.amax);
  a.amax_src = amax_dev != nullptr ? amax_dev : a.amax;
  int n_cu = 0;
  if (int rc = device_cu_count(&n_cu); rc != NERF_OK) return rc;
  const bool stream_family = chain_use_stream(n, true);
  const void* kernel = stream_family ? (bl.fp8 ? (const void*)mlp_bwd_stream_kernel<false> : (const void*)mlp_bwd_stream_kernel<true>)
                                     : (const void*)mlp_bwd_kernel;
  if (int rc = ensure_dynamic_lds(kernel, kChainLds, "nerf_mlp_bwd"); rc != NERF_OK) return rc;
  const int64_t tiles = bl.n_pad / kTileSamples;
  if (options().chain_grid > 0 && options().chain_grid < n_cu) n_cu = options().chain_grid;
  const int grid = (int)(tiles < n_cu ? tiles : n_cu);
  if (bl.fp8 && amax_dev == nullptr) {
    if (hipMemsetAsync(a.amax, 0, sizeof(float), as_stream(stream)) != hipSuccess)
      return fail(NERF_ELAUNCH, "nerf_mlp_bwd: memset failed");
    const int64_t want = (n + 1023) / 1024;
    hipLaunchKernelGGL(bwd_amax_kernel, dim3((int)(want < 1024 ? want : 1024)), dim3(256), 0, as_stream(stream), a);
  }
  if (stream_family && bl.fp8)
    hipLaunchKernelGGL(mlp_bwd_stream_kernel<false>, dim3(grid), dim3(kChainThreads), kChainLds, as_stream(stream), a);
  else if (stream_family)
    hipLaunchKernelGGL(mlp_bwd_stream_kernel<true>, dim3(grid), dim3(kChainThreads), kChainLds, as_stream(stream), a);
  else
    hipLaunchKernelGGL(mlp_bwd_kernel, dim3(grid), dim3(kChainThreads), kChainLds, as_stream(stream), a);
  return check_launch("nerf_mlp_bwd (dgrad chain)");
}

static int launch_wgrad(const void* stash, const void* workspace, int64_t n, float* grads_f32, int part,
                        nerf_stream_t stream) {
  NERF_REQUIRE(grads_f32 != nullptr, "nerf_mlp_bwd: grads_f32 is NULL");
  NERF_REQUIRE(part >= 0 && part <= 2, "nerf_mlp_bwd_wgrad_part: part=%d (0 all, 1 late layers, 2 early layers)", part);
  const size_t lo = part == 1 ? (size_t)plan::kW4 : 0, hi = part == 2 ? (size_t)plan::kW4 : (size_t)plan::kParamCount;
  if (n == 0) {
    if (hipMemsetAsync(grads_f32 + lo, 0, sizeof(float) * (hi - lo), as_stream(stream)) != hipSuccess)
      return fail(NERF_ELAUNCH, "nerf_mlp_bwd: memset failed");
    return NERF_OK;
  }
  NERF_REQUIRE(stash && workspace, "nerf_mlp_bwd: NULL pointer");
  return nerf_launch_wgrad(static_cast<const char*>(stash), stash_layout(n), static_cast<const char*>(workspace),
                           bwd_layout(n), n, grads_f32, part, as_stream(stream), lo, hi);
}

extern "C" int nerf_mlp_bwd_dgrad(const void* packed, const void* stash, const float* rgb, const float* sigma,
                                  const float* d_rgb, const float* d_sigma, int64_t n, void* workspace,
                                  nerf_stream_t stream) {
  if (n == 0) return NERF_OK;
  return launch_dgrad(packed, stash, rgb, sigma, d_rgb, d_sigma, n, workspace, nullptr, stream);
}

extern "C" int nerf_mlp_bwd_dgrad_ex(const void* packed, const void* stash, const float* rgb, const float* sigma,
                                     const float* d_rgb, const float* d_sigma, int64_t n, void* workspace,
                                     const float* amax_dev, nerf_stream_t stream) {
  if (n == 0) return NERF_OK;
  return launch_dgrad(packed, stash, rgb, sigma, d_rgb, d_sigma, n, workspace, amax_dev, stream);
}

extern "C" int nerf_mlp_bwd_wgrad(const void* stash, const void* workspace, int64_t n, float* grads_f32,
                                  nerf_stream_t stream) {
  return launch_wgrad(stash, workspace, n, grads_f32, 0, stream);
}

extern "C" int64_t nerf_mlp_wgrad_part_split(void) { return plan::kW4; }

extern "C" int nerf_mlp_bwd_wgrad_part(const void* stash, const void* workspace, int64_t n, float* grads_f32, int part,
                                       nerf_stream_t stream) {
  return launch_wgrad(stash, workspace, n, grads_f32, part, stream);
}

extern "C" int nerf_mlp_bwd(const void* packed, const void* stash, const float* rgb, const float* sigma,
                            const float* d_rgb, const float* d_sigma, int64_t n, float* grads_f32,
                            void* workspace, nerf_stream_t stream) {
  NERF_REQUIRE(n >= 0, "nerf_mlp_bwd: n=%lld", (long long)n);
  if (n > 0) {
    const int rc = launch_dgrad(packed, stash, rgb, sigma, d_rgb, d_sigma, n, workspace, nullptr, stream);
    if (rc != NERF_OK) return rc;
  }
  return launch_wgrad(stash, workspace, n, grads_f32, 0, stream);
}
```

### project-nerf_amd/csrc/mlp_pack.hip

```cpp
#include "common.h"
#include "mlp_plan.h"

namespace nerf {
using namespace plan;

struct FragTable {
  int v[kFwdFrags + kBwdFrags];
};

constexpr FragTable make_frag_table() {
  FragTable t{};
  int f = 0;
  for (int kind = 0; kind < kNumKinds; ++kind) {
    const int ks = step_ks(kind);
    for (int m = 0; m < step_of(kind).mt; ++m)
      for (int k = 0; k < ks; ++k) t.v[f++] = (kind << 16) | (m << 8) | k;
  }
  return t;
}
__constant__ FragTable g_frag_table = make_frag_table();

__device__ __forceinline__ int src_index(int kind, int row, int k, bool nat) {
  if (kind <= F_PTS7) {
    const int l = kind;
    const int in_dim = pts_in_dim(l);
    int col;
    if (l == 0) col = k < 63 ? k : -1;
    else if (l == 4) col = nat ? (k < 63 ? 256 + k : -1) : k;
    else col = k;
    return col < 0 ? -1 : pts_weight_off(l) + row * in_dim + col;
  }
  switch (kind) {
    case F_HEAD: return row < 256 ? kWFeat + row * 256 + k : (row == 256 ? kWSigma + k : -1);
    case F_VIEW: return nat ? (k < 27 ? kWView + row * 283 + 256 + k : -1) : kWView + row * 283 + k;
    case F_RGB: return row < 3 ? kWRgb + row * 128 + k : -1;
    case B_RGB: return k < 3 ? kWRgb + k * 128 + row : -1;
    case B_VIEW: return kWView + k * 283 + row;
    case B_HEAD: return nat ? (k == 0 ? kWSigma + row : -1) : kWFeat + k * 256 + row;
    default: {
      const int l = 7 - (kind - B_PTS7);
      return pts_weight_off(l) + k * pts_in_dim(l) + row;
    }
  }
}

__global__ void __launch_bounds__(256) pack16_kernel(const float* __restrict__ params, __bf16* __restrict__ packed_fwd16) {
  const int total = kFwdFrags * 64;
  for (int t = blockIdx.x * blockDim.x + threadIdx.x; t < total; t += gridDim.x * blockDim.x) {
    const int frag = t >> 6, lane = t & 63;
    const int desc = g_frag_table.v[frag];
    const int kind = desc >> 16, mt = (desc >> 8) & 0xFF, ks = desc & 0xFF;
    const Step st = step_of(kind);
    const int row = mt * 32 + 16 * (ks & 1) + (lane & 15), q = lane >> 4;
    const bool nat = ks >= st.ks_acc;
    const int kk = nat ? (ks - st.ks_acc) >> 1 : ks >> 1;
    typedef __bf16 bf16x8 __attribute__((ext_vector_type(8)));
    bf16x8 out;
#pragma unroll
    for (int j = 0; j < 8; ++j) {
      const int k = nat ? 32 * kk + 8 * q + j : 32 * kk + 16 * (j >> 2) + 4 * q + (j & 3);
      const int src = src_index(kind, row, k, nat);
      out[j] = (__bf16)(src >= 0 ? params[src] : 0.0f);
    }
    *reinterpret_cast<bf16x8*>(packed_fwd16 + (size_t)frag * 512 + lane * 8) = out;
  }
}

__global__ void __launch_bounds__(256)
pack_kernel(const float* __restrict__ params, __bf16* __restrict__ packed_fwd,
            __bf16* __restrict__ packed_bwd, float* __restrict__ bias) {
  const int total = (kFwdFrags + kBwdFrags) * 64;
  for (int t = blockIdx.x * blockDim.x + threadIdx.x; t < total; t += gridDim.x * blockDim.x) {
    const int frag = t >> 6, lane = t & 63;
    const int desc = g_frag_table.v[frag];
    const int kind = desc >> 16, mt = (desc >> 8) & 0xFF, ks = desc & 0xFF;
    const Step st = step_of(kind);
    const int row = mt * 32 + (lane & 31), h = lane >> 5;
    const bool nat = ks >= st.ks_acc;
    typedef __bf16 bf16x8 __attribute__((ext_vector_type(8)));
    bf16x8 out;
#pragma unroll
    for (int j = 0; j < 8; ++j) {
      const int k = frag_column(nat ? ks - st.ks_acc : ks, h, j, nat);
      const int src = src_index(kind, row, k, nat);
      out[j] = (__bf16)(src >= 0 ? params[src] : 0.0f);
    }
    __bf16* dst = frag < kFwdFrags ? packed_fwd + (size_t)frag * 512 : packed_bwd + (size_t)(frag - kFwdFrags) * 512;
    *reinterpret_cast<bf16x8*>(dst + lane * 8) = out;
  }
  for (int i = blockIdx.x * blockDim.x + threadIdx.x; i < kBiasFloats; i += gridDim.x * blockDim.x) {
    float b = 0.0f;
    if (i < 2048) b = params[pts_bias_off(i >> 8) + (i & 255)];
    else if (i < 2048 + 288) { const int r = i - 2048; b = r < 256 ? params[kBFeat + r] : (r == 256 ? params[kBSigma] : 0.0f); }
    else if (i < 2048 + 288 + 128) b = params[kBView + (i - 2048 - 288)];
    else { const int r = i - 2048 - 288 - 128; b = r < 3 ? params[kBRgb + r] : 0.0f; }
    bias[i] = b;
  }
}

}

extern "C" size_t nerf_mlp_packed_bytes(void) { return nerf::plan::kPackBytes; }

extern "C" int nerf_mlp_pack_streams(const float* params_f32, void* packed, int which, nerf_stream_t stream) {
  using namespace nerf;
  NERF_REQUIRE(params_f32 && packed, "nerf_mlp_pack: NULL pointer");
  NERF_REQUIRE(((uintptr_t)packed & 255) == 0, "nerf_mlp_pack: packed buffer must be 256-byte aligned");
  NERF_REQUIRE(which >= 1 && which <= 3, "nerf_mlp_pack_streams: which=%d (1 training streams + biases, 2 inference stream, 3 all)", which);
  char* base = static_cast<char*>(packed);
  if (which & 1)
    hipLaunchKernelGGL(pack_kernel, dim3(512), dim3(256), 0, as_stream(stream), params_f32,
                       reinterpret_cast<__bf16*>(base + plan::kPackFwdOff),
                       reinterpret_cast<__bf16*>(base + plan::kPackBwdOff),
                       reinterpret_cast<float*>(base + plan::kPackBiasOff));
  if (which & 2)
    hipLaunchKernelGGL(pack16_kernel, dim3(304), dim3(256), 0, as_stream(stream), params_f32,
                       reinterpret_cast<__bf16*>(base + plan::kPackFwd16Off));
  return check_launch("nerf_mlp_pack");
}

extern "C" int nerf_mlp_pack(const float* params_f32, void* packed, nerf_stream_t stream) {
  return nerf_mlp_pack_streams(params_f32, packed, 3, stream);
}
```

### project-nerf_amd/csrc/mlp_wgrad.h

```cpp
#pragma once
#include <hip/hip_runtime.h>
#include <stdint.h>

namespace nerf {

constexpr int kMaxJobs = 12;
constexpr int kWgStages = 4;
constexpr int kWgStageA = 16 * 1024, kWgStageB = 16 * 1024, kWgStageN = 4 * 1024;
constexpr int kWgStageBytes = kWgStageA + kWgStageB + kWgStageN;
constexpr int kWgLds = kWgStages * kWgStageBytes;
constexpr int kWgScratch = 256;
constexpr int kMaxTiles = 10;
constexpr size_t kSmallSlabBytes = 8u << 20;

struct WgradJob {
  const char* a;
  const char* b_acc;
  const char* b_nat;
  int a_bytes;
  int b_acc_bytes, b_nat_bytes;
  int a_nat;
  int mt_a;
  int nt_acc, nt_nat, ones;
  int split_n;
  int kind;
  int w_off, w_ld;
  int o_row0, o_valid;
  int acc_valid, acc_col0;
  int nat_valid, nat_col0;
  int bias_off, bias_nat_col;
  const char* a2;
  int w2_off, bias2_off, o2_row, n2;
  long long cost0;
  int cost;
  long long slab_off;
  int part0, n_parts, p_stride;
};

struct WgradArgs {
  WgradJob jobs[kMaxJobs];
  int n_jobs;
  int wave_tiles;
  long long total_cost;
  float* grads;
  float* slab;
  int slab_accumulate;
  const float* amax;
  int k16;
  int debug;
};

static inline WgradJob make_job(const char* w, size_t a_off, int a_bytes, int mt_a, size_t b_off, int nt_acc, size_t bn_off, int nt_nat,
                                int kind) {
  WgradJob j{};
  j.a = w + a_off; j.a_bytes = a_bytes; j.mt_a = mt_a;
  if (nt_acc) { j.b_acc = w + b_off; j.b_acc_bytes = nt_acc * 2048; j.nt_acc = nt_acc; }
  if (nt_nat) { j.b_nat = w + bn_off; j.b_nat_bytes = nt_nat * 2048; j.nt_nat = nt_nat; }
  j.bias_nat_col = -1; j.kind = kind;
  return j;
}

struct InstantImages { size_t hs1, h16, denc, hc1, hc2, dzs2, dzc1, dzc2, dsmall; };
static inline void instant_common_jobs(WgradArgs& wa, const char* w, const InstantImages& o, int s2, int c1, int c2, int c3) {
  { WgradJob j = make_job(w, o.dzs2, 2048, 1, o.hs1, 2, 0, 0, 7); j.w_off = s2; j.w_ld = 64; j.o_valid = 16; j.acc_valid = 64; wa.jobs[1] = j; }
  { WgradJob j = make_job(w, o.dzc1, 4096, 2, o.h16, 1, o.denc, 1, 8); j.w_off = c1; j.w_ld = 48; j.o_valid = 64; j.acc_valid = 16; j.nat_valid = 27; j.nat_col0 = 16; wa.jobs[2] = j; }
  { WgradJob j = make_job(w, o.dzc2, 4096, 2, o.hc1, 2, 0, 0, 7); j.w_off = c2; j.w_ld = 64; j.o_valid = 64; j.acc_valid = 64; wa.jobs[3] = j; }
  { WgradJob j = make_job(w, o.dsmall, 1024, 1, o.hc2, 2, 0, 0, 9); j.a_nat = 1; j.split_n = 1; j.w_off = c3; j.w_ld = 64; j.o_valid = 3; j.acc_valid = 64; wa.jobs[4] = j; }
}

int wgrad_launch(WgradArgs& args, int64_t n_samples, float* grads, hipStream_t stream, float* slab = nullptr,
                 size_t slab_bytes = 0, size_t zero_lo = 0, size_t zero_hi = 0);

}
```

### project-nerf_amd/csrc/mlp_wgrad.hip

```cpp
#include <stdlib.h>
#include "mlp_chain.h"
#include "mlp_stash.h"
#include "mlp_wgrad.h"

namespace nerf {
using namespace plan;

typedef short s16x4 __attribute__((ext_vector_type(4)));
typedef short s16x8 __attribute__((ext_vector_type(8)));
typedef __attribute__((address_space(3))) s16x4* lds_s16x4_t;

__device__ __forceinline__ void dma_1k(const char* gsrc_lane, unsigned lds_dst) {
  unsigned keep;
  asm volatile("s_mov_b32 %0, m0\n\ts_mov_b32 m0, %2\n\ts_nop 0\n\tglobal_load_lds_dwordx4 %1, off nt\n\ts_mov_b32 m0, %0"
               : "=&s"(keep) : "v"(gsrc_lane), "s"(lds_dst) : "memory");
}

template <int STRIDE>
__device__ __forceinline__ bf16x8 tr_frag(const char* p) {
  const s16x4 lo = __builtin_amdgcn_ds_read_tr16_b64_v4i16((lds_s16x4_t)(p));
  const s16x4 hi = __builtin_amdgcn_ds_read_tr16_b64_v4i16((lds_s16x4_t)(p + STRIDE));
  s16x8 v = {lo[0], lo[1], lo[2], lo[3], hi[0], hi[1], hi[2], hi[3]};
  return __builtin_bit_cast(bf16x8, v);
}
// ... 569 lines not shown
      case 6: run_job<0, 1, false, false, false>(args, job, wt0, wt1, smem, g); break;
      case 7: run_job<2, 0, false, false, false>(args, job, wt0, wt1, smem, g); break;
      case 8: run_job<1, 1, false, false, false>(args, job, wt0, wt1, smem, g); break;
      default: run_job<2, 0, false, true, false>(args, job, wt0, wt1, smem, g); break;
    }
    }
  }
}

template <bool P4>
__global__ void __launch_bounds__(512, P4 ? 4 : 6) mlp_wgrad_small_kernel(const WgradArgs args) {
  using Stage = std::conditional_t<P4, SmallStageP4, SmallStage>;
  extern __shared__ __attribute__((aligned(16))) char smem[];
  LaneGeo g;
  g.lane = threadIdx.x & 63;
  g.wave = __builtin_amdgcn_readfirstlane(threadIdx.x >> 6);
  const int grp = g.lane >> 4, i16 = g.lane & 15, q = i16 >> 2, p = i16 & 3;
  const int hh = grp >> 1;
  g.fhalf = grp & 1;
  g.off_acc = 512 * hh + 128 * g.fhalf + 64 * (p & 1) + 16 * q + 8 * (p >> 1);
  g.off_nat = 32 * (8 * hh + q) + 16 * (p >> 1) + 8 * (p & 1) + 1024 * g.fhalf;
  g.off_acc8 = g.off_nat8 = 0;
  const long long lo = args.total_cost * blockIdx.x / gridDim.x;
  const long long hi = args.total_cost * (blockIdx.x + 1) / gridDim.x;
  for (int j = 0; j < args.n_jobs; ++j) {
    const WgradJob job = args.jobs[j];
    const long long j0 = job.cost0, j1 = job.cost0 + (long long)job.cost * args.wave_tiles;
    if (hi <= j0 || lo >= j1) continue;
    const long long a0 = lo > j0 ? lo - j0 : 0, a1 = (hi < j1 ? hi : j1) - j0;
    const int wt0 = (int)((a0 + job.cost - 1) / job.cost), wt1 = (int)((a1 + job.cost - 1) / job.cost);
    if (wt0 >= wt1) continue;
    if constexpr (P4) {
      switch (job.kind) {
        case 10: run_job16<4, 4, 0, 2, 0, true, false, false, Stage>(args, job, wt0, wt1, smem, g); continue;
        case 11: run_job16<4, 4, 2, 2, 1, false, false, false, Stage>(args, job, wt0, wt1, smem, g); continue;
        case 12: run_job16<4, 0, 4, 0, 2, false, false, false, Stage>(args, job, wt0, wt1, smem, g); continue;
        default: break;
      }
    }
    switch (job.kind) {
      case 6: run_job16<4, 0, 2, 0, 1, false, false, false, Stage>(args, job, wt0, wt1, smem, g); break;
      case 7:
        if (job.mt_a == 2) run_job16<4, 4, 0, 2, 0, false, false, false, Stage>(args, job, wt0, wt1, smem, g);
        else run_job16<2, 4, 0, 2, 0, false, false, false, Stage>(args, job, wt0, wt1, smem, g);
        break;
      case 8: run_job16<4, 2, 2, 1, 1, false, false, false, Stage>(args, job, wt0, wt1, smem, g); break;
      default: run_job16<1, 4, 0, 2, 0, false, true, false, Stage>(args, job, wt0, wt1, smem, g); break;
    }
  }
}

__global__ void __launch_bounds__(256) wgrad_reduce_kernel(const WgradArgs args) {
  const WgradJob& job = args.jobs[blockIdx.y];
  const int n_w = job.o_valid * job.w_ld, n_b = n_w + job.o_valid, n_all = n_b + job.n2;
  const float* tile = args.slab + job.slab_off;
  for (int i = blockIdx.x * blockDim.x + threadIdx.x; i < n_all; i += gridDim.x * blockDim.x) {
    float s0 = 0.0f, s1 = 0.0f, s2 = 0.0f, s3 = 0.0f;
    int t = 0;
    for (; t + 4 <= job.n_parts; t += 4) {
      s0 += tile[(long long)(t + 0) * job.p_stride + i];
      s1 += tile[(long long)(t + 1) * job.p_stride + i];
      s2 += tile[(long long)(t + 2) * job.p_stride + i];
      s3 += tile[(long long)(t + 3) * job.p_stride + i];
    }
    for (; t < job.n_parts; ++t) s0 += tile[(long long)t * job.p_stride + i];
    const float sum = (s0 + s1) + (s2 + s3);
    float* dst = i < n_w ? args.grads + job.w_off + i
               : i < n_b ? ((job.ones || job.bias_nat_col >= 0) ? args.grads + job.bias_off + (i - n_w) : nullptr)
               : i < n_all - 1 ? args.grads + job.w2_off + (i - n_b)
                               : args.grads + job.bias2_off;
    if (dst != nullptr) *dst = args.slab_accumulate ? *dst + sum : sum;
  }
}

}

using namespace nerf;

int nerf_launch_wgrad(const char* stash, const StashLayout& sl, const char* work, const BwdLayout& bl,
                      int64_t n, float* grads, int part, hipStream_t stream, size_t zero_lo, size_t zero_hi) {
  WgradArgs args{};
  const size_t np = (size_t)sl.n_pad, eb = sl.fp8 ? 1 : 2;
  if (sl.fp8 != bl.fp8) return fail(NERF_EINVAL, "nerf_mlp_bwd: stash and workspace disagree on the image width");
  args.amax = sl.fp8 ? reinterpret_cast<const float*>(work + bl.amax) : nullptr;
  const char* xenc = stash + sl.xenc;
  const char* denc = stash + sl.denc;
  auto st_h = [&](int l) { return stash + sl.h + (size_t)l * np * 256 * eb; };
  auto dh = [&](int l) { return work + bl.dh + (size_t)l * np * 256 * eb; };
  int nj = 0;
  auto add = [&](WgradJob j) {
    args.jobs[nj++] = j;
  };
  {
    WgradJob j{};
    j.a = dh(0); j.a_bytes = 16384; j.mt_a = 8;
    j.b_nat = xenc; j.b_nat_bytes = 4096; j.nt_nat = 2;
    j.w_off = kW0; j.w_ld = 63; j.o_valid = 256; j.nat_valid = 63; j.nat_col0 = 0;
    j.bias_off = kB0; j.bias_nat_col = 63; j.kind = 2;
    add(j);
  }
  for (int l = 1; l < 8; ++l) {
    WgradJob j{};
    j.a = dh(l); j.a_bytes = 16384; j.mt_a = 8;
    j.b_acc = st_h(l - 1); j.b_acc_bytes = 16384; j.nt_acc = 8;
    j.w_off = pts_weight_off(l); j.w_ld = pts_in_dim(l); j.o_valid = 256; j.acc_valid = 256;
    j.bias_off = pts_bias_off(l);
    if (l == 4) {
      j.b_nat = xenc; j.b_nat_bytes = 4096; j.nt_nat = 2; j.nat_valid = 63; j.nat_col0 = 256; j.bias_nat_col = 63;
      j.kind = 1;
    } else {
      j.ones = 1; j.bias_nat_col = -1; j.kind = 0;
    }
    add(j);
  }
  {
    WgradJob j{};
    j.a = work + bl.dfeat; j.a_bytes = 16384; j.mt_a = 8;
    j.b_acc = st_h(7); j.b_acc_bytes = 16384; j.nt_acc = 8; j.ones = 1; j.bias_nat_col = -1;
    j.w_off = kWFeat; j.w_ld = 256; j.o_valid = 256; j.acc_valid = 256; j.bias_off = kBFeat; j.kind = 0;
    if (!sl.fp8) {
      j.a2 = work + bl.dsmall; j.w2_off = kWSigma; j.bias2_off = kBSigma; j.o2_row = 3; j.n2 = 257; j.kind = 13;
    }
    add(j);
  }
  if (sl.fp8) {
    WgradJob j{};
    j.a = work + bl.dsmall; j.a_bytes = 1024; j.a_nat = 1; j.mt_a = 1; j.split_n = 1;
    j.b_acc = st_h(7); j.b_acc_bytes = 16384; j.nt_acc = 8; j.ones = 1; j.bias_nat_col = -1;
    j.w_off = kWSigma; j.w_ld = 256; j.o_row0 = 3; j.o_valid = 1; j.acc_valid = 256; j.bias_off = kBSigma; j.kind = 4;
    add(j);
  }
  {
    WgradJob j{};
    j.a = work + bl.dhv; j.a_bytes = 8192; j.mt_a = 4;
    j.b_acc = stash + sl.feat; j.b_acc_bytes = 16384; j.nt_acc = 8;
    j.b_nat = denc; j.b_nat_bytes = 2048; j.nt_nat = 1; j.nat_valid = 27; j.nat_col0 = 256; j.bias_nat_col = 27;
    j.w_off = kWView; j.w_ld = 283; j.o_valid = 128; j.acc_valid = 256; j.bias_off = kBView; j.kind = 3;
    add(j);
  }
  {
    WgradJob j{};
    j.a = work + bl.dsmall; j.a_bytes = 1024; j.a_nat = 1; j.mt_a = 1; j.split_n = 1;
    j.b_acc = stash + sl.hv; j.b_acc_bytes = 8192; j.nt_acc = 4; j.ones = 1; j.bias_nat_col = -1;
    j.w_off = kWRgb; j.w_ld = 128; j.o_row0 = 0; j.o_valid = 3; j.acc_valid = 128; j.bias_off = kBRgb; j.kind = 5;
    add(j);
  }
  if (part != 0) {
    const int lo = part == 1 ? 4 : 0, hi = part == 1 ? nj : 4;
    for (int j = lo; j < hi; ++j) args.jobs[j - lo] = args.jobs[j];
    nj = hi - lo;
  }
  args.n_jobs = nj;
  float* slab = bl.slab_bytes ? reinterpret_cast<float*>(const_cast<char*>(work) + bl.slab) : nullptr;
  return wgrad_launch(args, n, grads, stream, slab, bl.slab_bytes, zero_lo, zero_hi);
}

int nerf::wgrad_launch(WgradArgs& args, int64_t n, float* grads, hipStream_t stream, float* slab, size_t slab_bytes,
                       size_t zero_lo, size_t zero_hi) {
  int nj = args.n_jobs;
  const int overhead = options().wgrad_overhead;
  for (int j = 0; j < nj; ++j) {
    WgradJob& jb = args.jobs[j];
    const int bytes = jb.a_bytes + jb.b_acc_bytes + jb.b_nat_bytes + (jb.a2 ? 1024 : 0);
    jb.cost = bytes + overhead;
    if (args.amax != nullptr) {
      const int nt = jb.nt_acc + jb.nt_nat + jb.ones;
      const int per_simd = jb.split_n ? (jb.nt_acc > 4 ? 3 : 2) : (jb.mt_a > 4 ? 2 : 1) * nt;
      const int t_mfma = (jb.split_n || options().wgrad_k16 ? 32 * 4 : 64) * per_simd, t_dma = bytes * 16 / options().wgrad_bw_x16;
      jb.cost = (t_mfma > t_dma ? t_mfma : t_dma) + options().wgrad_fixed;
    }
  }
  args.wave_tiles = args.amax != nullptr ? (int)((n + 63) / 64) : (int)((n + 31) / 32);
  long long c = 0;
  for (int j = 0; j < nj; ++j) {
    args.jobs[j].cost0 = c;
    c += (long long)args.jobs[j].cost * args.wave_tiles;
  }
  args.total_cost = c;
  args.grads = grads;
  args.debug = options().wgrad_debug;
  args.k16 = options().wgrad_k16;
  if (options().wgrad_only >= 0) {
    const int kind = options().wgrad_only;
    int m = 0;
    for (int j = 0; j < args.n_jobs; ++j) if (args.jobs[j].kind == kind) args.jobs[m++] = args.jobs[j];
    args.n_jobs = m;
    nj = m;
    long long cc = 0;
    for (int j = 0; j < nj; ++j) { args.jobs[j].cost0 = cc; cc += (long long)args.jobs[j].cost * args.wave_tiles; }
    args.total_cost = cc;
  }

  int n_cu = 0;
  if (int rc = device_cu_count(&n_cu); rc != NERF_OK) return rc;
  const bool fp8 = args.amax != nullptr;
  if (int rc = ensure_dynamic_lds(fp8 ? (const void*)mlp_wgrad_kernel<true> : (const void*)mlp_wgrad_kernel<false>, kWgLds + kWgScratch,
                                  "nerf_mlp_bwd (wgrad)"); rc != NERF_OK) return rc;
  bool small = args.amax == nullptr && !options().wgrad_big_only, p4 = false;
  for (int j = 0; j < args.n_jobs; ++j) {
    const WgradJob& jb = args.jobs[j];
    p4 = p4 || (jb.kind >= 10 && jb.kind <= 12);
    small = small && jb.kind >= 6 && jb.a_bytes <= SmallStage::A && jb.b_acc_bytes <= SmallStage::B && jb.b_nat_bytes <= SmallStageP4::N;
  }
  if (p4 && !small) return fail(NERF_EINVAL, "wgrad: Part 4 job kinds run on the small-stage kernel only");
  long long want = (long long)args.wave_tiles * nj / 4;
  if (options().wgrad_grid > 0 && options().wgrad_grid < n_cu) n_cu = options().wgrad_grid;
  int grid = (int)(want < 1 ? 1 : (want > n_cu ? n_cu : want));
  if (small) {
    const long long span = options().wgrad_small_span > 0 ? options().wgrad_small_span : 4;
    const long long cap = (long long)(slab != nullptr ? 1 : (options().wgrad_small_cap > 0 ? options().wgrad_small_cap : 3)) * n_cu;
    const long long want3 = (long long)args.wave_tiles * nj / span;
    grid = (int)(want3 < 1 ? 1 : (want3 > cap ? cap : want3));
  }
  args.slab = nullptr;
  args.slab_accumulate = small ? 1 : 0;
  if (slab != nullptr && args.n_jobs > 0 && args.total_cost > 0) {
    bool ok = true;
    long long off = 0;
    for (int j = 0; j < args.n_jobs && ok; ++j) {
      WgradJob& jb = args.jobs[j];
      const long long j0 = jb.cost0, j1 = jb.cost0 + (long long)jb.cost * args.wave_tiles;
      int first = -1, last = -1, count = 0;
      for (int b = 0; b < grid; ++b) {
        const long long lo = args.total_cost * b / grid, hi = args.total_cost * (b + 1) / grid;
        if (hi <= j0 || lo >= j1) continue;
        const long long a0 = lo > j0 ? lo - j0 : 0, a1 = (hi < j1 ? hi : j1) - j0;
        const int wt0 = (int)((a0 + jb.cost - 1) / jb.cost), wt1 = (int)((a1 + jb.cost - 1) / jb.cost);
        if (wt0 >= wt1) continue;
        if (first < 0) first = b;
        last = b;
        ++count;
      }
      ok = count > 0 && count == last - first + 1;
      jb.part0 = first;
      jb.n_parts = count;
      jb.p_stride = (jb.o_valid * jb.w_ld + jb.o_valid + jb.n2 + 63) / 64 * 64;
      jb.slab_off = off;
      off += (long long)count * jb.p_stride;
    }
    if (ok && (size_t)off * sizeof(float) <= slab_bytes) args.slab = slab;
    if (args.slab != nullptr && small && hipMemsetAsync(slab, 0, (size_t)off * sizeof(float), stream) != hipSuccess)
      return fail(NERF_ELAUNCH, "tiny-MLP wgrad: memset failed");
    if (args.slab == nullptr && small) return fail(NERF_EINVAL, "tiny-MLP wgrad (option \"deterministic\"): partial tiles need %zu bytes, %zu given%s",
                                (size_t)off * sizeof(float), slab_bytes, ok ? "" : " (a job's workgroups are not contiguous)");
  }
  if (args.slab == nullptr && zero_hi > zero_lo &&
      hipMemsetAsync(grads + zero_lo, 0, sizeof(float) * (zero_hi - zero_lo), stream) != hipSuccess)
    return fail(NERF_ELAUNCH, "nerf_mlp_bwd: memset failed");
  if (small) {
    if (p4) hipLaunchKernelGGL(mlp_wgrad_small_kernel<true>, dim3(grid), dim3(512), kWgStages * SmallStageP4::Bytes, stream, args);
    else hipLaunchKernelGGL(mlp_wgrad_small_kernel<false>, dim3(grid), dim3(512), kWgStages * SmallStage::Bytes, stream, args);
    if (args.slab != nullptr) {
      if (int rc = check_launch("tiny-MLP wgrad"); rc != NERF_OK) return rc;
      hipLaunchKernelGGL(wgrad_reduce_kernel, dim3(16, args.n_jobs), dim3(256), 0, stream, args);
      return check_launch("tiny-MLP wgrad (reduce)");
    }
    return check_launch("tiny-MLP wgrad");
  }
  if (fp8) hipLaunchKernelGGL(mlp_wgrad_kernel<true>, dim3(grid), dim3(512), kWgLds + kWgScratch, stream, args);
  else hipLaunchKernelGGL(mlp_wgrad_kernel<false>, dim3(grid), dim3(512), kWgLds + kWgScratch, stream, args);
  if (args.slab != nullptr) {
    if (int rc = check_launch("nerf_mlp_bwd (wgrad)"); rc != NERF_OK) return rc;
    hipLaunchKernelGGL(wgrad_reduce_kernel, dim3(160, args.n_jobs), dim3(256), 0, stream, args);
    return check_launch("nerf_mlp_bwd (wgrad reduce)");
  }
  return check_launch("nerf_mlp_bwd (wgrad)");
}
```

### project-nerf_amd/engine.py

```python
from __future__ import annotations

import os
from typing import Dict, Optional, Tuple

import torch

from . import flat_params, ops
from .flat_engine import LapSlots, ViewSlots, cosine_lr, render_chunks, render_counted_chain

Tensor = torch.Tensor


def param_shapes():
    return [(k, shape) for k, _, shape in flat_params.nerf_decoder_table("", 63, 27)]


def default_init(seed: int = 0) -> Tensor:
    g = torch.Generator().manual_seed(seed)
    parts, fan_in = [], 1
    for name, shape in param_shapes():
        if name.endswith("weight"):
            fan_in = shape[1]
        parts.append(((torch.rand(shape, generator=g) * 2 - 1) / fan_in ** 0.5).reshape(-1))
    return torch.cat(parts)


def flatten_state_dict(sd: Dict[str, Tensor], prefix: str = "decoder.") -> Tensor:
    return flat_params.flatten(flat_params.nerf_decoder_table(prefix, 63, 27), sd)


def unflatten(flat: Tensor, prefix: str = "decoder.") -> Dict[str, Tensor]:
    return flat_params.unflatten(flat_params.nerf_decoder_table(prefix, 63, 27), flat)


class VanillaNerfEngine:
    def __init__(self, params: Optional[Tensor] = None, device: str = "cuda", lr: float = 5e-4,
                 near: float = 2.0, far: float = 6.0, white_bkgd: bool = True, seed: int = 0,
                 world_size: int = 1, grid_resolution: int = 128, bound: float = 1.5, grid_threshold: float = 0.01):
        self.device = torch.device(device)
        flat = default_init(seed) if params is None else params.detach().float().reshape(-1)
        assert flat.numel() == ops.MLP_PARAM_COUNT
        self.params = flat.to(self.device).contiguous()
        self.exp_avg = torch.zeros_like(self.params)
        self.exp_avg_sq = torch.zeros_like(self.params)
        self.grads = torch.empty_like(self.params)
        self.packed = torch.empty(ops.mlp_packed_bytes(), dtype=torch.uint8, device=self.device)
        self.lr, self.near, self.far = lr, near, far
        self.bg = (torch.ones(3) if white_bkgd else torch.zeros(3)).to(self.device)
        self.step_count = 0
        self.world_size = world_size
        self.grad_scale = torch.full((1,), 1.0 / world_size, device=self.device)
        self._ws: Dict[Tuple[str, int], Tensor] = {}
        self._scalars = torch.zeros(2, 1024, device=self.device)
        self._slots = LapSlots(self._scalars)
        self._infer_stale = False
        self.grid_resolution, self.bound, self.grid_threshold = int(grid_resolution), float(bound), float(grid_threshold)
        self.grid: Optional[Tensor] = None
        self.binary_grid: Optional[Tensor] = None
        self._grid_ws: Dict[Tuple[int, int], Tensor] = {}
        self.seed, self._jitter_counter = int(seed), 0
        self._grid_train_ws: Dict[str, Tensor] = {}
        self.repack()

    def repack(self, training_only: bool = False) -> None:
        ops.mlp_pack(self.params, self.packed, which=1 if training_only else 3)
        self._infer_stale = training_only

    def _inference_weights(self) -> Tensor:
        if self._infer_stale:
            ops.mlp_pack(self.params, self.packed, which=2)
            self._infer_stale = False
        return self.packed

    def state_dict(self, prefix: str = "decoder.") -> Dict[str, Tensor]:
        return {k: v.clone() for k, v in unflatten(self.params, prefix).items()}

    def load_state_dict(self, sd: Dict[str, Tensor], prefix: str = "decoder.") -> None:
        self.params.copy_(flatten_state_dict(sd, prefix).to(self.device))
        self.repack()

    def _buf(self, kind: str, nbytes: int) -> Tensor:
        key = (kind, nbytes)
        if key not in self._ws:
            self._ws[key] = torch.empty(nbytes, dtype=torch.uint8, device=self.device)
        return self._ws[key]

    GRID_SLACK = (1.25, 1 << 20)

    def _grid_buf(self, kind: str, nbytes: int) -> Tensor:
        buf = self._grid_train_ws.get(kind)
        if buf is None or buf.numel() < nbytes:
            buf = None
            self._grid_train_ws.pop(kind, None)
            buf = self._grid_train_ws[kind] = torch.empty(int(nbytes * self.GRID_SLACK[0]) + self.GRID_SLACK[1], dtype=torch.uint8,
                                                          device=self.device)
        return buf

    def prepare_batch(self, rays_o: Tensor, rays_d: Tensor, n_samples: int = 64, u: Optional[Tensor] = None, first_ray: int = 0):
        grid = self._require_grid("prepare_batch")
        jitter = None
        if u is None:
            self._jitter_counter += 1
            jitter = (self.seed, self._jitter_counter)
        return ops.sample_compact_async(rays_o, rays_d, self.near, self.far, n_samples, grid, self.bound, u=u, jitter=jitter,
                                        first_ray=first_ray)

    def _grid_gradients(self, rays_o: Tensor, rays_d: Tensor, target: Tensor, n_samples: int, u, sync_grads, sync_grads_async, mark,
                        prepared) -> Tensor:
        mark = mark or (lambda name: None)
        if prepared is None:
            prepared = self.prepare_batch(rays_o, rays_d, n_samples, u=u)
        z, slots, pts, dirs = prepared.get()
        mark("sample")
        R, n = rays_o.shape[0], pts.shape[0]
        if n == 0:
            self.grads.zero_()
            loss = ((self.bg.expand(R, 3) - target) ** 2).mean()
            mark("fwd")
            mark("loss")
            mark("dgrad")
            if sync_grads_async is not None:
                split = ops._lib.load().nerf_mlp_wgrad_part_split()
                for h in [sync_grads_async(view) for view in (self.grads[split:], self.grads[:split])]:
                    if h is not None:
                        h.wait()
            mark("wgrad")
            if sync_grads is not None:
                sync_grads(self.grads)
            return loss
        stash = self._grid_buf("stash", ops.mlp_stash_bytes(n))
        rgb, sigma = ops.mlp_fwd(self.packed, pts, dirs, None, stash)
        mark("fwd")
        loss, amax = self._slots.take()
        d_rgb, d_sigma, _ = ops.composite_mse_bwd(rgb, sigma, z, rays_d, self.bg, target, loss, slots=slots, amax_accum=amax)
        mark("loss")
        ws = self._grid_buf("bwd", ops.mlp_bwd_workspace_bytes(n))
        if sync_grads_async is not None:
            ops.mlp_bwd_overlapped(self.packed, stash, rgb, sigma, d_rgb, d_sigma, self.grads, ws, sync_grads_async, amax=amax, mark=mark)
        else:
            ops.mlp_bwd(self.packed, stash, rgb, sigma, d_rgb, d_sigma, self.grads, ws, amax=amax, mark=mark)
        mark("wgrad")
        if sync_grads is not None:
            sync_grads(self.grads)
        return LapSlots.keep(loss)

    def compute_gradients(self, rays_o: Tensor, rays_d: Tensor, target: Tensor, n_samples: int = 64,
                   u: Optional[Tensor] = None, sync_grads=None, sync_grads_async=None, mark=None,
                   z: Optional[Tensor] = None, grid: bool = False, prepared=None) -> Tensor:
        if grid or prepared is not None:
            if z is not None:
                raise ValueError("compute_gradients: the grid step draws its own depths (z is for the dense step)")
            return self._grid_gradients(rays_o, rays_d, target, n_samples, u, sync_grads, sync_grads_async, mark, prepared)
        mark = mark or (lambda name: None)
        R = rays_o.shape[0]
        n = R * n_samples
        if z is None:
            if u is None:
                u = torch.rand(R, n_samples, device=self.device)
            z = ops.sample_rays(rays_o, rays_d, self.near, self.far, n_samples, u=u)
            mark("sample")
        stash = self._buf("stash", ops.mlp_stash_bytes(n))
        rgb, sigma = ops.mlp_fwd(self.packed, rays_o, rays_d, z, stash)
        mark("fwd")
        loss, amax = self._slots.take()
        d_rgb, d_sigma, _ = ops.composite_mse_bwd(rgb.view(R, n_samples, 3), sigma.view(R, n_samples), z, rays_d, self.bg,
                                                  target, loss, amax_accum=amax)
        mark("loss")
        if sync_grads_async is not None:
            ops.mlp_bwd_overlapped(self.packed, stash, rgb, sigma, d_rgb.view(n, 3), d_sigma.view(n), self.grads,
                                   self._buf("bwd", ops.mlp_bwd_workspace_bytes(n)), sync_grads_async, amax=amax, mark=mark)
        else:
            ops.mlp_bwd(self.packed, stash, rgb, sigma, d_rgb.view(n, 3), d_sigma.view(n), self.grads,
                        self._buf("bwd", ops.mlp_bwd_workspace_bytes(n)), amax=amax, mark=mark)
        mark("wgrad")
        if sync_grads is not None:
            sync_grads(self.grads)
        return LapSlots.keep(loss)

    def apply_gradients(self) -> None:
        self.step_count += 1
        ops.adam_step(self.params, self.grads, self.exp_avg, self.exp_avg_sq, self.step_count, self.lr,
                      grad_scale=self.grad_scale if self.world_size > 1 else None)
        self.repack(training_only=True)

    def train_step(self, rays_o: Tensor, rays_d: Tensor, target: Tensor, n_samples: int = 64,
                   u: Optional[Tensor] = None, sync_grads=None, sync_grads_async=None, mark=None,
                   z: Optional[Tensor] = None, grid: bool = False, prepared=None) -> Tensor:
        loss = self.compute_gradients(rays_o, rays_d, target, n_samples, u=u, sync_grads=sync_grads,
                                      sync_grads_async=sync_grads_async, mark=mark, z=z, grid=grid, prepared=prepared)
        self.apply_gradients()
        if mark is not None:
            mark("adam+pack")
        return loss

    @torch.no_grad()
    def render_rays(self, rays_o: Tensor, rays_d: Tensor, n_samples: int, u: Optional[Tensor] = None):
        z = ops.sample_rays(rays_o, rays_d, self.near, self.far, n_samples, u=u)
        rgb, sigma = ops.mlp_fwd(self._inference_weights(), rays_o, rays_d, z)
        R = rays_o.shape[0]
        c, depth, acc, _, _ = ops.composite_fwd(rgb.view(R, n_samples, 3), sigma.view(R, n_samples), z, rays_d, self.bg)
        return c, depth, acc

    @torch.no_grad()
    def render_rays_hierarchical(self, rays_o: Tensor, rays_d: Tensor, n_coarse: int, n_fine: int):
        R = rays_o.shape[0]
        z = ops.sample_rays(rays_o, rays_d, self.near, self.far, n_coarse)
        rgb, sigma = ops.mlp_fwd(self._inference_weights(), rays_o, rays_d, z)
        w = ops.composite_fwd(rgb.view(R, n_coarse, 3), sigma.view(R, n_coarse), z, rays_d, self.bg, want_weights=True)[4]
        z_all = ops.sample_pdf(z, w, n_fine)
        S = n_coarse + n_fine
        rgb, sigma = ops.mlp_fwd(self._inference_weights(), rays_o, rays_d, z_all)
        c, depth, acc, _, _ = ops.composite_fwd(rgb.view(R, S, 3), sigma.view(R, S), z_all, rays_d, self.bg)
        return c, depth, acc

    @torch.no_grad()
    def update_grid(self) -> float:
        res = self.grid_resolution
        pts = ops.grid_lattice(self.bound, res, self.device)
        sig = torch.empty(res ** 3, device=self.device)
        zeros = torch.zeros(2 ** 18, 3, device=self.device)
        packed = self._inference_weights()
        for i in range(0, pts.shape[0], 2 ** 18):
            p = pts[i:i + 2 ** 18]
            sig[i:i + 2 ** 18] = ops.mlp_fwd(packed, p, zeros[:p.shape[0]], None)[1]
        binary, ratio = ops.grid_threshold(sig.view(res, res, res), self.grid_threshold)
        if ratio <= 0.0:
            return 0.0
        self.grid, self.binary_grid = sig.view(res, res, res), binary
        return ratio

    def _require_grid(self, what: str) -> Tensor:
        if self.binary_grid is None:
            raise ValueError(f"{what}: no occupancy grid (call update_grid() or set binary_grid first)")
        return self.binary_grid

    @torch.no_grad()
    def render_rays_grid(self, rays_o: Tensor, rays_d: Tensor, n_samples: int):
        grid = self._require_grid("render_rays_grid")
        z, slots, pts, dirs = ops.sample_compact(rays_o, rays_d, self.near, self.far, n_samples, grid, self.bound)
        R = rays_o.shape[0]
        if pts.shape[0] == 0:
            bg = self.bg.expand(R, 3).clone() if self.bg.dim() == 1 else self.bg.clone()
            return bg, torch.zeros(R, device=self.device), torch.zeros(R, device=self.device)
# ... 351 lines not shown
```

### project-nerf_amd/ops.py

```python
from __future__ import annotations

import weakref
from typing import Optional, Tuple

import torch

from . import _lib

Tensor = torch.Tensor


def _stream() -> int:
    return torch._C._cuda_getCurrentRawStream(torch._C._cuda_getDevice())


def _dev(t: Tensor, name: str, dtype=torch.float32) -> Tensor:
    if not isinstance(t, Tensor):
        raise TypeError(f"{name}: expected a tensor")
    if t.device.type != "cuda":
        raise _lib.NerfHipError(f"{name} is on {t.device}; the hot path only runs on a HIP device (no CPU fallback)")
    if t.dtype != dtype:
        raise TypeError(f"{name}: expected {dtype}, got {t.dtype}")
    return t if t.is_contiguous() else t.contiguous()

# ... 345 lines not shown
    lib = _lib.load()
    x = _dev(x, "x")
    n, dim = x.shape
    out = torch.empty(n, dim + 2 * dim * n_freq, device=x.device, dtype=torch.float32)
    _lib.check(lib.nerf_fourier_encode(_p(x), n, dim, n_freq, _p(out), _stream()), "nerf_fourier_encode")
    return out


def composite_fwd(rgb: Tensor, sigma: Tensor, z: Tensor, rays_d: Tensor, bg: Optional[Tensor] = None,
                  extra: Optional[Tensor] = None, want_weights: bool = False):
    lib = _lib.load()
    rgb, sigma, z, rays_d = _dev(rgb, "rgb"), _dev(sigma, "sigma"), _dev(z, "z"), _dev(rays_d, "rays_d")
    R, S = z.shape
    bg = None if bg is None else _dev(bg, "bg")
    bg_rows = _bg_rows(bg)
    out_rgb = torch.empty(R, 3, device=z.device, dtype=torch.float32)
    depth = torch.empty(R, device=z.device, dtype=torch.float32)
    acc = torch.empty(R, device=z.device, dtype=torch.float32)
    extra_map = None
    if extra is not None:
        extra = _dev(extra, "extra")
        extra_map = torch.empty(R, 3, device=z.device, dtype=torch.float32)
    w = torch.empty(R, S, device=z.device, dtype=torch.float32) if want_weights else None
    _lib.check(lib.nerf_composite_fwd(_p(rgb), _p(sigma), _p(z), _p(rays_d), _p(bg), bg_rows, _p(extra),
                                      R, S, _p(out_rgb), _p(depth), _p(acc), _p(extra_map), _p(w), _stream()),
               "nerf_composite_fwd")
    return out_rgb, depth, acc, extra_map, w


def composite_bwd(rgb, sigma, z, rays_d, bg, extra, g_rgb, g_depth, g_acc, g_extra):
    lib = _lib.load()
    rgb, sigma, z, rays_d = _dev(rgb, "rgb"), _dev(sigma, "sigma"), _dev(z, "z"), _dev(rays_d, "rays_d")
    R, S = z.shape
    bg = None if bg is None else _dev(bg, "bg")
    bg_rows = _bg_rows(bg)
    g_rgb = _dev(g_rgb, "g_rgb")
    g_depth = None if g_depth is None else _dev(g_depth, "g_depth")
    g_acc = None if g_acc is None else _dev(g_acc, "g_acc")
    d_rgb = torch.empty(R, S, 3, device=z.device, dtype=torch.float32)
    d_sigma = torch.empty(R, S, device=z.device, dtype=torch.float32)
    d_extra = None
    if extra is not None and g_extra is not None:
        extra, g_extra = _dev(extra, "extra"), _dev(g_extra, "g_extra")
        d_extra = torch.empty(R, S, 3, device=z.device, dtype=torch.float32)
    else:
        extra = g_extra = None
    _lib.check(lib.nerf_composite_bwd(_p(rgb), _p(sigma), _p(z), _p(rays_d), _p(bg), bg_rows, _p(extra),
                                      _p(g_rgb), _p(g_depth), _p(g_acc), _p(g_extra), R, S,
                                      _p(d_rgb), _p(d_sigma), _p(d_extra), _stream()), "nerf_composite_bwd")
    return d_rgb, d_sigma, d_extra


def composite_mse_bwd(rgb: Tensor, sigma: Tensor, z: Tensor, rays_d: Tensor, bg: Optional[Tensor], target: Tensor,
                      loss_accum: Tensor, slots: Optional[Tensor] = None, amax_accum: Optional[Tensor] = None,
                      loss_weight: Optional[float] = None, want_pred: bool = False):
    lib = _lib.load()
    rgb, sigma, z, rays_d, target = _dev(rgb, "rgb"), _dev(sigma, "sigma"), _dev(z, "z"), _dev(rays_d, "rays_d"), _dev(target, "target")
    R, S = z.shape
    bg = None if bg is None else _dev(bg, "bg")
    bg_rows = _bg_rows(bg)
    d_rgb, d_sigma = torch.empty_like(rgb), torch.empty_like(sigma)
    pred = torch.empty(R, 3, device=z.device) if want_pred else None
    w = 1.0 / (3 * R) if loss_weight is None else loss_weight
    _lib.check(lib.nerf_composite_mse_bwd(_p(rgb), _p(sigma), _p(slots), _p(z), _p(rays_d), _p(bg), bg_rows, _p(target), w, R, S,
                                          _p(pred), _p(loss_accum), _p(d_rgb), _p(d_sigma), _p(amax_accum), _p(sum_ws(z.device)), _stream()),
               "nerf_composite_mse_bwd")
    return d_rgb, d_sigma, pred


class _Composite(torch.autograd.Function):

    @staticmethod
    def forward(ctx, rgb, sigma, z, rays_d, bg, extra):
        out_rgb, depth, acc, extra_map, _ = composite_fwd(rgb, sigma, z, rays_d, bg, extra)
        ctx.save_for_backward(rgb, sigma, z, rays_d, bg, extra)
        if extra_map is None:
            extra_map = out_rgb.new_zeros(0)
        return out_rgb, depth, acc, extra_map

    @staticmethod
    def backward(ctx, g_rgb, g_depth, g_acc, g_extra):
        rgb, sigma, z, rays_d, bg, extra = ctx.saved_tensors
        d_rgb, d_sigma, d_extra = composite_bwd(rgb, sigma, z, rays_d, bg, extra, g_rgb.contiguous(),
                                                g_depth.contiguous(), g_acc.contiguous(),
                                                None if extra is None else g_extra.contiguous())
        return d_rgb, d_sigma, None, None, None, d_extra


def composite(rgb: Tensor, sigma: Tensor, z: Tensor, rays_d: Tensor, bg: Optional[Tensor] = None,
              extra: Optional[Tensor] = None):
    out_rgb, depth, acc, extra_map = _Composite.apply(rgb, sigma, z, rays_d, bg, extra)
    return out_rgb, depth, acc, (extra_map if extra is not None else None)


MLP_PARAM_COUNT = 595844


def mlp_packed_bytes() -> int:
    return _lib.load().nerf_mlp_packed_bytes()


def mlp_pack(params: Tensor, packed: Optional[Tensor] = None, which: int = 3) -> Tensor:
    lib = _lib.load()
    params = _dev(params, "params")
    if params.numel() != MLP_PARAM_COUNT:
        raise ValueError(f"params must have {MLP_PARAM_COUNT} elements, got {params.numel()}")
    if packed is None:
        packed = torch.empty(lib.nerf_mlp_packed_bytes(), device=params.device, dtype=torch.uint8)
    _lib.check(lib.nerf_mlp_pack_streams(_p(params), _p(packed), which, _stream()), "nerf_mlp_pack")
    return packed


def mlp_stash_bytes(n: int) -> int:
    return _lib.load().nerf_mlp_stash_bytes(n)


# ... 19 lines not shown
    rays_o, rays_d = _dev(rays_o, "rays_o"), _dev(rays_d, "rays_d")
    R = rays_o.shape[0]
    chunk = max(1, min(chunk, max(R, 1)))
    need = lib.nerf_render_rays_workspace_bytes(chunk, n_samples)
    if workspace is None or workspace.numel() < need:
        workspace = torch.empty(need, device=rays_o.device, dtype=torch.uint8)
    bg = None if bg is None else _dev(bg, "bg")
    bg_rows = _bg_rows(bg)
    out = torch.empty(R, 3, device=rays_o.device)
    depth, acc = torch.empty(R, device=rays_o.device), torch.empty(R, device=rays_o.device)
    _lib.check(lib.nerf_render_rays_fwd(_p(packed), _p(rays_o), _p(rays_d), R, n_samples, float(near), float(far), _p(bg), bg_rows,
                                        chunk, _p(workspace), _p(out), _p(depth), _p(acc), _stream()), "nerf_render_rays_fwd")
    return out, depth, acc


def render_rays_grid_workspace_bytes(chunk: int, n_samples: int) -> int:
    return _lib.load().nerf_render_rays_grid_workspace_bytes(chunk, n_samples)


def _counted_render_args(name: str, workspace_bytes, packed, binary_grid, rays_o, rays_d, n_samples, bg, chunk, workspace):
    rays_o, rays_d = _dev(rays_o, "rays_o"), _dev(rays_d, "rays_d")
    grid = _dev(binary_grid, "binary_grid", torch.bool)
    packed = _dev(packed, "packed", torch.uint8)
    R = rays_o.shape[0]
    chunk = max(1, min(int(chunk), max(R, 1)))
    need = workspace_bytes(chunk, n_samples)
    if workspace is None:
        workspace = torch.empty(need, device=rays_o.device, dtype=torch.uint8)
    elif _dev(workspace, "workspace", torch.uint8).numel() < need:
        raise ValueError(f"{name}: workspace of {workspace.numel()} bytes, {need} needed for chunk {chunk} x {n_samples}")
    bg = None if bg is None else _dev(bg, "bg")
    out = torch.empty(R, 3, device=rays_o.device)
    depth, acc = torch.empty(R, device=rays_o.device), torch.empty(R, device=rays_o.device)
    return packed, grid, rays_o, rays_d, R, bg, _bg_rows(bg), chunk, workspace, out, depth, acc


def render_rays_grid_fwd(packed: Tensor, binary_grid: Tensor, grid_bound: float, rays_o: Tensor, rays_d: Tensor, n_samples: int,
                         near: float, far: float, bg: Optional[Tensor] = None, chunk: int = 65536, workspace: Optional[Tensor] = None):
    lib = _lib.load()
    packed, grid, rays_o, rays_d, R, bg, bg_rows, chunk, workspace, out, depth, acc = _counted_render_args(
        "render_rays_grid_fwd", lib.nerf_render_rays_grid_workspace_bytes, packed, binary_grid, rays_o, rays_d, n_samples, bg, chunk, workspace)
    _lib.check(lib.nerf_render_rays_grid_fwd(_p(packed), _p(grid), grid.shape[0], float(grid_bound), _p(rays_o), _p(rays_d), R, n_samples,
                                             float(near), float(far), _p(bg), bg_rows, chunk, _p(workspace), _p(out), _p(depth),
                                             _p(acc), _stream()), "nerf_render_rays_grid_fwd")
    return out, depth, acc


def mlp_bwd_workspace_bytes(n: int) -> int:
    return _lib.load().nerf_mlp_bwd_workspace_bytes(n)


def mlp_bwd(packed: Tensor, stash: Tensor, rgb: Tensor, sigma: Tensor, d_rgb: Tensor, d_sigma: Tensor,
            grads: Optional[Tensor] = None, workspace: Optional[Tensor] = None, amax: Optional[Tensor] = None,
            mark=None) -> Tensor:
    lib = _lib.load()
    rgb, sigma = _dev(rgb, "rgb"), _dev(sigma, "sigma")
    d_rgb, d_sigma = _dev(d_rgb, "d_rgb"), _dev(d_sigma, "d_sigma")
    n = sigma.numel()
    if grads is None:
        grads = torch.empty(MLP_PARAM_COUNT, device=rgb.device, dtype=torch.float32)
    if workspace is None:
        workspace = torch.empty(lib.nerf_mlp_bwd_workspace_bytes(n), device=rgb.device, dtype=torch.uint8)
    if amax is None:
        _lib.check(lib.nerf_mlp_bwd(_p(packed), _p(stash), _p(rgb), _p(sigma), _p(d_rgb), _p(d_sigma), n,
                                    _p(grads), _p(workspace), _stream()), "nerf_mlp_bwd")
    else:
        _lib.check(lib.nerf_mlp_bwd_dgrad_ex(_p(packed), _p(stash), _p(rgb), _p(sigma), _p(d_rgb), _p(d_sigma), n,
                                             _p(workspace), _p(amax), _stream()), "nerf_mlp_bwd_dgrad_ex")
        if mark is not None:
            mark("dgrad")
        _lib.check(lib.nerf_mlp_bwd_wgrad(_p(stash), _p(workspace), n, _p(grads), _stream()), "nerf_mlp_bwd_wgrad")
    return grads


def mlp_bwd_overlapped(packed: Tensor, stash: Tensor, rgb: Tensor, sigma: Tensor, d_rgb: Tensor, d_sigma: Tensor,
                       grads: Tensor, workspace: Tensor, reduce_async, amax: Optional[Tensor] = None, mark=None) -> None:
    lib = _lib.load()
    n = sigma.numel()
    _lib.check(lib.nerf_mlp_bwd_dgrad_ex(_p(packed), _p(stash), _p(rgb), _p(sigma), _p(d_rgb), _p(d_sigma), n,
                                         _p(workspace), _p(amax), _stream()), "nerf_mlp_bwd_dgrad")
    if mark is not None:
        mark("dgrad")
    split = lib.nerf_mlp_wgrad_part_split()
    handles = []
    for part, view in ((1, grads[split:]), (2, grads[:split])):
        _lib.check(lib.nerf_mlp_bwd_wgrad_part(_p(stash), _p(workspace), n, _p(grads), part, _stream()),
                   "nerf_mlp_bwd_wgrad_part")
        handles.append(reduce_async(view))
    for h in handles:
        if h is not None:
            h.wait()


class _Decoder(torch.autograd.Function):

    @staticmethod
    def forward(ctx, params, packed, rays_o, rays_d, z):
        n = z.numel() if z is not None else rays_o.shape[0]
        stash = torch.empty(mlp_stash_bytes(n), device=params.device, dtype=torch.uint8)
        rgb, sigma = mlp_fwd(packed, rays_o, rays_d, z, stash)
        ctx.save_for_backward(packed, stash, rgb, sigma)
        return rgb, sigma

    @staticmethod
    def backward(ctx, d_rgb, d_sigma):
        packed, stash, rgb, sigma = ctx.saved_tensors
        grads = mlp_bwd(packed, stash, rgb, sigma, d_rgb.contiguous(), d_sigma.contiguous())
        return grads, None, None, None, None


class _DecoderEncoded(torch.autograd.Function):

    @staticmethod
    def forward(ctx, params, packed, x_enc, d_enc, train):
        lib = _lib.load()
        n = x_enc.shape[0]
        rgb = torch.empty(n, 3, device=x_enc.device)
        sigma = torch.empty(n, device=x_enc.device)
        stash = torch.empty(mlp_stash_bytes(n), device=x_enc.device, dtype=torch.uint8) if train else None
        _lib.check(lib.nerf_mlp_fwd_encoded(_p(packed), _p(x_enc), _p(d_enc), n, _p(rgb), _p(sigma), _p(stash), _stream()),
                   "nerf_mlp_fwd_encoded")
        if train:
            ctx.save_for_backward(packed, stash, rgb, sigma)
        return rgb, sigma
# ... 362 lines not shown
        res, shape = 0, (pts.shape[0],)
    else:
        pts, res = None, int(source)
        if res < 2:
            raise ValueError(f"instant_grid_update: resolution {res} (at least 2)")
        shape = (res, res, res)
    n = 1
    for s in shape:
        n *= s
    slab_cells = int(slab_cells)
    need = lib.nerf_instant_grid_update_workspace_bytes(slab_cells)
    if prev is not None:
        grid = _dev(prev, "prev")
        if grid is not prev or grid.numel() != n:
            raise ValueError("instant_grid_update: prev must be a contiguous tensor of one value per cell (it is updated in place)")
    else:
        grid = torch.empty(shape, device=packed.device, dtype=torch.float32)
    if workspace is None:
        workspace = torch.empty(need, device=packed.device, dtype=torch.uint8)
    elif _dev(workspace, "workspace", torch.uint8).numel() < need:
        raise ValueError(f"instant_grid_update: workspace of {workspace.numel()} bytes, {need} needed for slabs of {slab_cells} cells")
    binary = torch.empty(shape, device=packed.device, dtype=torch.bool)
    if n == 0:
        return grid, binary, torch.zeros(1, device=packed.device, dtype=torch.int64)
    count = torch.empty(1, device=packed.device, dtype=torch.int64)
    _lib.check(lib.nerf_instant_grid_update(_p(packed), table_f32, table_f16, levels.n_levels,
                                            *levels.host_args(), float(hash_bound), _p(pts), n, res, float(grid_bound), _p(grid), _p(binary),
                                            float(decay), 0 if prev is None else 1, float(threshold), _p(count), slab_cells, _p(workspace),
                                            _stream()), "nerf_instant_grid_update")
    return grid, binary, count


def instant_field(table: Tensor, net_params: Tensor, packed: Tensor, pts: Tensor, dirs: Tensor,
                  levels: HashLevelTable, bound: float):
    pts, dirs = _dev(pts, "pts"), _dev(dirs, "dirs")
    if pts.shape[0] == 0:
        return pts.new_zeros(0, 3), pts.new_zeros(0)
    train = torch.is_grad_enabled() and (table.requires_grad or net_params.requires_grad)
    return _InstantField.apply(table, net_params, packed, pts, dirs, levels, bound, train)


def adam_step(params: Tensor, grads: Tensor, exp_avg: Tensor, exp_avg_sq: Tensor, step: int, lr: float,
              beta1: float = 0.9, beta2: float = 0.999, eps: float = 1e-8, weight_decay: float = 0.0,
              grad_scale: Optional[Tensor] = None) -> None:
    lib = _lib.load()
    for t, nm in ((params, "params"), (grads, "grads"), (exp_avg, "exp_avg"), (exp_avg_sq, "exp_avg_sq")):
        if _dev(t, nm) is not t:
            raise ValueError(f"{nm} must be contiguous")
    _lib.check(lib.nerf_adam_step(_p(params), _p(grads), _p(exp_avg), _p(exp_avg_sq), params.numel(), step,
                                  lr, beta1, beta2, eps, weight_decay, _p(grad_scale), _stream()),
               "nerf_adam_step")


SMALL_GROUP = 65536


def tv_clip_adamw_step(params: Tensor, grads: Tensor, exp_avg: Tensor, exp_avg_sq: Tensor, step: int, lr: float,
                       tv_weight: float = 0.0, max_norm: float = 0.0, weight_decay: float = 0.0,
                       beta1: float = 0.9, beta2: float = 0.999, eps: float = 1e-8, grad_scale: float = 1.0,
                       scratch: Optional[Tensor] = None, shadow_f16: Optional[Tensor] = None, tv_codes: Optional[Tensor] = None) -> None:
    lib = _lib.load()
    for t, nm in ((params, "params"), (grads, "grads"), (exp_avg, "exp_avg"), (exp_avg_sq, "exp_avg_sq")):
        if _dev(t, nm) is not t:
            raise ValueError(f"{nm} must be contiguous")
    normsq = scratch if (scratch is not None and scratch.numel() >= _lib.NORMSQ_WS_FLOATS) else normsq_ws(params.device)
    n = params.numel()
    if shadow_f16 is not None and (shadow_f16.dtype != torch.float16 or shadow_f16.numel() != n or not shadow_f16.is_contiguous()):
        raise ValueError("shadow_f16 must be a contiguous torch.float16 tensor of the parameters' size")
    if tv_weight != 0.0:
        if tv_codes is None or tv_codes.numel() < (n + 3) // 4:
            tv_codes = torch.empty((n + 3) // 4, dtype=torch.uint8, device=params.device)
    else:
        tv_codes = None
    if tv_codes is None and shadow_f16 is None and n <= SMALL_GROUP:
        _lib.check(lib.nerf_clip_adamw_small(_p(params), _p(grads), _p(exp_avg), _p(exp_avg_sq), n, step, lr, beta1, beta2, eps, weight_decay,
                                             max_norm, grad_scale, _p(normsq), 0, _stream()), "nerf_clip_adamw_small")
        return
    _lib.check(lib.nerf_tv_normsq_codes(_p(params), _p(grads), n, 1, tv_weight, grad_scale, _p(normsq), 0, _p(tv_codes), _stream()),
               "nerf_tv_normsq_codes")
    _lib.check(lib.nerf_adamw_clip_step_tv(_p(params), _p(grads), _p(exp_avg), _p(exp_avg_sq), n, step, lr, beta1, beta2, eps, weight_decay,
                                           _p(normsq), max_norm, grad_scale, _p(tv_codes), n, tv_weight, n, 0.0, 0, 0, 0.0, _p(shadow_f16),
                                           _stream()), "nerf_adamw_clip_step_tv")
```

Baseline: 3.874 million rays/s.

## Fuse wgrad reduction, loss sum, Adam and repack into a single step-tail kernel

Adds a deferred path for the vanilla train step. The composite loss partial sums and the wgrad final reduction are left unreduced, and a new step-tail kernel finishes the loss sum, completes the gradient reduction, applies Adam and repacks the weights in one launch. The aim is to remove several small kernel launches and a round trip of the gradient buffer at the end of each step. It only runs for single-GPU runs with no gradient sync, and it adds a new fused kernel whose Adam arithmetic has to match the original.

```diff
diff --git a/include/nerf_hip.h b/include/nerf_hip.h
--- a/include/nerf_hip.h
+++ b/include/nerf_hip.h
@@ -13,7 +13,7 @@
 #define NERF_ELAUNCH (-5)
 #define NERF_ENOSYS (-38)
 
-#define NERF_ABI_VERSION 12
+#define NERF_ABI_VERSION 13
 
 typedef void* nerf_stream_t;
 
@@ -161,6 +161,8 @@
                             nerf_stream_t stream);
 int nerf_mlp_bwd_wgrad(const void* stash, const void* workspace, int64_t n, float* grads_f32,
                        nerf_stream_t stream);
+int nerf_mlp_bwd_wgrad_deferred(const void* stash, const void* workspace, int64_t n, float* grads_f32,
+                                nerf_stream_t stream);
 
 int nerf_hash_encode_fwd(const float* pts, int64_t n, const float* table, int n_levels,
                          const float* scale_host, const unsigned* res_host, const unsigned* size_host,
@@ -288,6 +290,10 @@
                            const float* rays_d, const float* bg, int64_t bg_rows, const float* target,
                            float loss_weight, int64_t n_rays, int n_samples, float* pred_out, float* loss_accum,
                            float* d_rgb, float* d_sigma, float* amax_accum, float* sum_ws, nerf_stream_t stream);
+int nerf_composite_mse_bwd_deferred(const float* rgb, const float* sigma, const int* slot_of_sample, const float* z,
+                                    const float* rays_d, const float* bg, int64_t bg_rows, const float* target,
+                                    float loss_weight, int64_t n_rays, int n_samples, float* pred_out, float* d_rgb,
+                                    float* d_sigma, float* sum_ws, nerf_stream_t stream);
 int nerf_composite_mse_reg_bwd(const float* rgb, const float* sigma, const int* slot_of_sample, const float* z,
                                const float* rays_d, const float* bg, int64_t bg_rows, const float* target,
                                float loss_weight, const float* extra, float reg_weight, int64_t n_rays, int n_samples,
@@ -297,6 +303,13 @@
 int nerf_adam_step(float* params, const float* grads, float* exp_avg, float* exp_avg_sq,
                    int64_t n, int step, float lr, float beta1, float beta2, float eps,
                    float weight_decay, const float* grad_scale_dev, nerf_stream_t stream);
+
+int nerf_vanilla_step_tail(const void* workspace, int64_t n, const float* sum_ws, int64_t n_rays, float* loss_out,
+                           float* params, float* grads, float* exp_avg, float* exp_avg_sq, int step, float lr, float beta1,
+                           float beta2, float eps, float weight_decay, const float* grad_scale_dev, void* packed,
+                           nerf_stream_t stream);
+int nerf_vanilla_step_tail_available(int64_t n);
+int nerf_vanilla_step_tail_selfcheck(void);
 
 #define NERF_NORMSQ_WS_FLOATS 4136
 int nerf_tv_normsq(const float* params, float* grads, int64_t n, float tv_weight, float grad_scale,
diff --git a/project-nerf_amd/_lib.py b/project-nerf_amd/_lib.py
--- a/project-nerf_amd/_lib.py
+++ b/project-nerf_amd/_lib.py
@@ -70,6 +70,13 @@
     "nerf_mlp_bwd_dgrad_ex": (i32, [c_ptr, c_ptr, c_ptr, c_ptr, c_ptr, c_ptr, i64, c_ptr, c_ptr, c_ptr]),
     "nerf_composite_mse_bwd": (i32, [c_ptr, c_ptr, c_ptr, c_ptr, c_ptr, c_ptr, i64, c_ptr, f32, i64, i32, c_ptr, c_ptr,
                                      c_ptr, c_ptr, c_ptr, c_ptr, c_ptr]),
+    "nerf_composite_mse_bwd_deferred": (i32, [c_ptr, c_ptr, c_ptr, c_ptr, c_ptr, c_ptr, i64, c_ptr, f32, i64, i32, c_ptr,
+                                              c_ptr, c_ptr, c_ptr, c_ptr]),
+    "nerf_mlp_bwd_wgrad_deferred": (i32, [c_ptr, c_ptr, i64, c_ptr, c_ptr]),
+    "nerf_vanilla_step_tail": (i32, [c_ptr, i64, c_ptr, i64, c_ptr, c_ptr, c_ptr, c_ptr, c_ptr, i32, f32, f32, f32, f32, f32, c_ptr, c_ptr,
+                                     c_ptr]),
+    "nerf_vanilla_step_tail_available": (i32, [i64]),
+    "nerf_vanilla_step_tail_selfcheck": (i32, []),
     "nerf_mlp_wgrad_part_split": (i64, []),
     "nerf_mlp_bwd_wgrad_part": (i32, [c_ptr, c_ptr, i64, c_ptr, i32, c_ptr]),
     "nerf_hash_encode_fwd": (i32, [c_ptr, i64, c_ptr, i32, c_ptr, c_ptr, c_ptr, c_ptr, c_ptr, f32, c_ptr, c_ptr, c_ptr, c_ptr]),
@@ -169,7 +176,7 @@
     "nerf_adamw_clip_step_shadow": (i32, [c_ptr, c_ptr, c_ptr, c_ptr, i64, i32, f32, f32, f32, f32, f32, c_ptr, f32, f32, c_ptr, c_ptr]),
 }
 
-ABI_VERSION = 12
+ABI_VERSION = 13
 
 _lib = None
 
diff --git a/project-nerf_amd/csrc/adam.h b/project-nerf_amd/csrc/adam.h
--- /dev/null
+++ b/project-nerf_amd/csrc/adam.h
@@ -0,0 +1,36 @@
+#pragma once
+#include <math.h>
+#include "common.h"
+
+namespace nerf {
+
+__device__ __forceinline__ void adam_update(float& p, float g, float& m, float& v, float lr, float beta1, float beta2,
+                                            float eps, float wd, float inv_bc1, float inv_sqrt_bc2) {
+  float pi = p;
+  if (wd != 0.0f) pi *= (1.0f - lr * wd);
+  const float mi = beta1 * m + (1.0f - beta1) * g;
+  const float vi = beta2 * v + (1.0f - beta2) * g * g;
+  m = mi;
+  v = vi;
+  p = pi - (lr * inv_bc1) * (mi / (sqrtf(vi) * inv_sqrt_bc2 + eps));
+}
+
+__device__ __forceinline__ void adam_update_fused(float& p, float g, float& m, float& v, float lr, float beta1, float beta2,
+                                                  float eps, float wd, float inv_bc1, float inv_sqrt_bc2) {
+#pragma clang fp contract(off)
+  float pi = p;
+  if (wd != 0.0f) pi *= __builtin_fmaf(-lr, wd, 1.0f);
+  const float mi = __builtin_fmaf(beta1, m, (1.0f - beta1) * g);
+  const float vi = __builtin_fmaf(beta2, v, ((1.0f - beta2) * g) * g);
+  m = mi;
+  v = vi;
+  p = __builtin_fmaf(-(lr * inv_bc1), mi / __builtin_fmaf(sqrtf(vi), inv_sqrt_bc2, eps), pi);
+}
+
+inline void adam_bias_correction(float beta1, float beta2, int step, float* inv_bc1, float* inv_sqrt_bc2) {
+  const double bc1 = 1.0 - pow((double)beta1, step), bc2 = 1.0 - pow((double)beta2, step);
+  *inv_bc1 = (float)(1.0 / bc1);
+  *inv_sqrt_bc2 = (float)(1.0 / sqrt(bc2));
+}
+
+}
diff --git a/project-nerf_amd/csrc/adam.hip b/project-nerf_amd/csrc/adam.hip
--- a/project-nerf_amd/csrc/adam.hip
+++ b/project-nerf_amd/csrc/adam.hip
@@ -1,19 +1,9 @@
 #include "common.h"
+#include "adam.h"
 
 namespace nerf {
 
 typedef float f4 __attribute__((ext_vector_type(4)));
-
-__device__ __forceinline__ void adam_update(float& p, float g, float& m, float& v, float lr, float beta1, float beta2,
-                                            float eps, float wd, float inv_bc1, float inv_sqrt_bc2) {
-  float pi = p;
-  if (wd != 0.0f) pi *= (1.0f - lr * wd);
-  const float mi = beta1 * m + (1.0f - beta1) * g;
-  const float vi = beta2 * v + (1.0f - beta2) * g * g;
-  m = mi;
-  v = vi;
-  p = pi - (lr * inv_bc1) * (mi / (sqrtf(vi) * inv_sqrt_bc2 + eps));
-}
 
 template <bool VEC>
 __device__ __forceinline__ void adam_sweep(float* __restrict__ p, const float* __restrict__ g, float* __restrict__ m,
@@ -65,17 +55,16 @@
   NERF_REQUIRE(n >= 0 && step >= 1, "nerf_adam_step: n=%lld step=%d", (long long)n, step);
   if (n == 0) return NERF_OK;
   NERF_REQUIRE(params && grads && exp_avg && exp_avg_sq, "nerf_adam_step: NULL pointer");
-  const double bc1 = 1.0 - pow((double)beta1, step), bc2 = 1.0 - pow((double)beta2, step);
+  float inv_bc1, inv_sqrt_bc2;
+  nerf::adam_bias_correction(beta1, beta2, step, &inv_bc1, &inv_sqrt_bc2);
   int64_t blocks = (n / 4 + 255) / 256 + 1;
   if (blocks > 2048) blocks = 2048;
   if (nerf::aligned16(params, grads, exp_avg, exp_avg_sq))
     hipLaunchKernelGGL(nerf::adam_kernel<true>, dim3((int)blocks), dim3(256), 0, nerf::as_stream(stream), params,
-                       grads, exp_avg, exp_avg_sq, n, lr, beta1, beta2, eps, weight_decay,
-                       (float)(1.0 / bc1), (float)(1.0 / sqrt(bc2)), grad_scale_dev);
+                       grads, exp_avg, exp_avg_sq, n, lr, beta1, beta2, eps, weight_decay, inv_bc1, inv_sqrt_bc2, grad_scale_dev);
   else
     hipLaunchKernelGGL(nerf::adam_kernel<false>, dim3((int)blocks), dim3(256), 0, nerf::as_stream(stream), params,
-                       grads, exp_avg, exp_avg_sq, n, lr, beta1, beta2, eps, weight_decay,
-                       (float)(1.0 / bc1), (float)(1.0 / sqrt(bc2)), grad_scale_dev);
+                       grads, exp_avg, exp_avg_sq, n, lr, beta1, beta2, eps, weight_decay, inv_bc1, inv_sqrt_bc2, grad_scale_dev);
   return nerf::check_launch("nerf_adam_step");
 }
 
diff --git a/project-nerf_amd/csrc/api.cpp b/project-nerf_amd/csrc/api.cpp
--- a/project-nerf_amd/csrc/api.cpp
+++ b/project-nerf_amd/csrc/api.cpp
@@ -40,6 +40,7 @@
     {"composite_wgs_per_cu", "NERF_COMPOSITE_WGS", &Options::composite_wgs_per_cu},
     {"deterministic", "NERF_DETERMINISTIC", &Options::deterministic},
     {"tv_blocks", "NERF_TV_BLOCKS", &Options::tv_blocks},
+    {"step_tail", "NERF_STEP_TAIL", &Options::step_tail},
 };
 
 Options& options() {
diff --git a/project-nerf_amd/csrc/common.h b/project-nerf_amd/csrc/common.h
--- a/project-nerf_amd/csrc/common.h
+++ b/project-nerf_amd/csrc/common.h
@@ -43,6 +43,7 @@
   int hash_xcd = 1;
   int hash_fwd_lds_kb = 36;
   int tv_blocks = 0;
+  int step_tail = 1;
   int deterministic = 0;
 };
 Options& options();
diff --git a/project-nerf_amd/csrc/composite.hip b/project-nerf_amd/csrc/composite.hip
--- a/project-nerf_amd/csrc/composite.hip
+++ b/project-nerf_amd/csrc/composite.hip
@@ -1,4 +1,5 @@
 #include "common.h"
+#include "composite_sums.h"
 
 namespace nerf {
 
@@ -332,25 +333,7 @@
 
 __global__ void __launch_bounds__(256) composite_sums_kernel(const float* __restrict__ ws, int n_blocks, float* __restrict__ loss_out,
                                                              float* __restrict__ reg_out, float* __restrict__ amax_out) {
-  __shared__ float part[3][4];
-  float s0 = 0.0f, s1 = 0.0f, m = 0.0f;
-  for (int b = threadIdx.x; b < n_blocks; b += 256) {
-    s0 += ws[b];
-    s1 += ws[n_blocks + b];
-    const float v = ws[2 * n_blocks + b];
-    if (v == v && v < 3.0e38f) m = fmaxf(m, v);
-  }
-  s0 = wave_sum(s0);
-  s1 = wave_sum(s1);
-#pragma unroll
-  for (int off = 32; off > 0; off >>= 1) m = fmaxf(m, __shfl_xor(m, off));
-  if ((threadIdx.x & 63) == 0) { part[0][threadIdx.x >> 6] = s0; part[1][threadIdx.x >> 6] = s1; part[2][threadIdx.x >> 6] = m; }
-  __syncthreads();
-  if (threadIdx.x == 0) {
-    *loss_out += (part[0][0] + part[0][1]) + (part[0][2] + part[0][3]);
-    if (reg_out != nullptr) *reg_out += (part[1][0] + part[1][1]) + (part[1][2] + part[1][3]);
-    if (amax_out != nullptr) *amax_out = fmaxf(*amax_out, fmaxf(fmaxf(part[2][0], part[2][1]), fmaxf(part[2][2], part[2][3])));
-  }
+  composite_sums<false>(ws, n_blocks, loss_out, reg_out, amax_out);
 }
 
 static int per_lane(int S) {
@@ -452,7 +435,8 @@
                             slot_of_sample, n_rays, n_samples, d_rgb_compact, d_sigma_compact, nullptr, stream);
 }
 
-static int64_t mse_blocks(int64_t n_rays, bool partials) {
+static int64_t mse_blocks(int64_t n_rays, bool partials) { return composite_mse_blocks(n_rays, partials); }
+int64_t nerf::composite_mse_blocks(int64_t n_rays, bool partials) {
   int n_cu = 256;
   (void)device_cu_count(&n_cu);
   const int per_cu = partials ? 8 : (options().composite_wgs_per_cu < 1 ? 1 : options().composite_wgs_per_cu);
@@ -483,6 +467,23 @@
              (const float*)nullptr, 0.0f, (float*)nullptr, (float*)nullptr, (float*)nullptr, reinterpret_cast<unsigned*>(sum_ws));
   if (int rc = check_launch("nerf_composite_mse_bwd"); rc != NERF_OK) return rc;
   return finish_sums(sum_ws, grid.x, loss_accum, nullptr, amax_accum, stream);
+}
+
+extern "C" int nerf_composite_mse_bwd_deferred(const float* rgb, const float* sigma, const int* slot_of_sample, const float* z,
+                                               const float* rays_d, const float* bg, int64_t bg_rows, const float* target,
+                                               float loss_weight, int64_t n_rays, int n_samples, float* pred_out, float* d_rgb,
+                                               float* d_sigma, float* sum_ws, nerf_stream_t stream) {
+  NERF_REQUIRE(n_rays >= 0 && n_samples >= 1 && n_samples <= 64 * kMaxPerLane,
+               "nerf_composite_mse_bwd_deferred: n_rays=%lld n_samples=%d (max %d)", (long long)n_rays, n_samples, 64 * kMaxPerLane);
+  if (n_rays == 0) return NERF_OK;
+  NERF_REQUIRE(rgb && sigma && z && rays_d && target && d_rgb && d_sigma, "nerf_composite_mse_bwd_deferred: NULL pointer");
+  NERF_REQUIRE(sum_ws != nullptr, "nerf_composite_mse_bwd_deferred: sum_ws is NULL (the partial sums have nowhere to stay)");
+  NERF_REQUIRE(bg == nullptr || bg_rows == 1 || bg_rows == n_rays, "nerf_composite_mse_bwd_deferred: bg_rows=%lld", (long long)bg_rows);
+  const dim3 grid((unsigned)mse_blocks(n_rays, true));
+  DISPATCH_K(per_lane(n_samples), composite_mse_bwd_kernel, rgb, sigma, z, rays_d, bg, bg_rows, target, loss_weight,
+             slot_of_sample, n_rays, n_samples, pred_out, (float*)nullptr, d_rgb, d_sigma, (float*)nullptr,
+             (const float*)nullptr, 0.0f, (float*)nullptr, (float*)nullptr, (float*)nullptr, reinterpret_cast<unsigned*>(sum_ws));
+  return check_launch("nerf_composite_mse_bwd_deferred");
 }
 
 extern "C" int nerf_composite_mse_reg_bwd(const float* rgb, const float* sigma, const int* slot_of_sample, const float* z,
diff --git a/project-nerf_amd/csrc/composite_sums.h b/project-nerf_amd/csrc/composite_sums.h
--- /dev/null
+++ b/project-nerf_amd/csrc/composite_sums.h
@@ -0,0 +1,34 @@
+#pragma once
+#include "common.h"
+
+namespace nerf {
+
+int64_t composite_mse_blocks(int64_t n_rays, bool partials);
+
+template <bool STORE>
+__device__ __forceinline__ void composite_sums(const float* __restrict__ ws, int n_blocks, float* __restrict__ loss_out,
+                                               float* __restrict__ reg_out, float* __restrict__ amax_out) {
+  __shared__ float part[3][4];
+  float s0 = 0.0f, s1 = 0.0f, m = 0.0f;
+  for (int b = threadIdx.x; b < n_blocks; b += 256) {
+    s0 += ws[b];
+    s1 += ws[n_blocks + b];
+    const float v = ws[2 * n_blocks + b];
+    if (v == v && v < 3.0e38f) m = fmaxf(m, v);
+  }
+  s0 = wave_sum(s0);
+  s1 = wave_sum(s1);
+#pragma unroll
+  for (int off = 32; off > 0; off >>= 1) m = fmaxf(m, __shfl_xor(m, off));
+  if ((threadIdx.x & 63) == 0) { part[0][threadIdx.x >> 6] = s0; part[1][threadIdx.x >> 6] = s1; part[2][threadIdx.x >> 6] = m; }
+  __syncthreads();
+  if (threadIdx.x == 0) {
+    const float loss = (part[0][0] + part[0][1]) + (part[0][2] + part[0][3]);
+    if (STORE) *loss_out = 0.0f + loss;
+    else *loss_out += loss;
+    if (reg_out != nullptr) *reg_out += (part[1][0] + part[1][1]) + (part[1][2] + part[1][3]);
+    if (amax_out != nullptr) *amax_out = fmaxf(*amax_out, fmaxf(fmaxf(part[2][0], part[2][1]), fmaxf(part[2][2], part[2][3])));
+  }
+}
+
+}
diff --git a/project-nerf_amd/csrc/mlp_bwd.hip b/project-nerf_amd/csrc/mlp_bwd.hip
--- a/project-nerf_amd/csrc/mlp_bwd.hip
+++ b/project-nerf_amd/csrc/mlp_bwd.hip
@@ -1,5 +1,6 @@
 #include "mlp_chain_body.h"
 #include "mlp_stash.h"
+#include "mlp_wgrad.h"
 
 namespace nerf {
 using namespace plan;
@@ -120,7 +121,8 @@
 using namespace nerf;
 
 int nerf_launch_wgrad(const char* stash, const StashLayout& sl, const char* work, const BwdLayout& bl,
-                      int64_t n, float* grads, int part, hipStream_t stream, size_t zero_lo, size_t zero_hi);
+                      int64_t n, float* grads, int part, hipStream_t stream, size_t zero_lo, size_t zero_hi, WgradMode mode,
+                      WgradArgs* plan_out);
 
 extern "C" size_t nerf_mlp_bwd_workspace_bytes(int64_t n) { return n > 0 ? bwd_layout(n).total : 0; }
 
@@ -170,7 +172,7 @@
 }
 
 static int launch_wgrad(const void* stash, const void* workspace, int64_t n, float* grads_f32, int part,
-                        nerf_stream_t stream) {
+                        nerf_stream_t stream, WgradMode mode = kWgradAll) {
   NERF_REQUIRE(grads_f32 != nullptr, "nerf_mlp_bwd: grads_f32 is NULL");
   NERF_REQUIRE(part >= 0 && part <= 2, "nerf_mlp_bwd_wgrad_part: part=%d (0 all, 1 late layers, 2 early layers)", part);
   const size_t lo = part == 1 ? (size_t)plan::kW4 : 0, hi = part == 2 ? (size_t)plan::kW4 : (size_t)plan::kParamCount;
@@ -181,7 +183,7 @@
   }
   NERF_REQUIRE(stash && workspace, "nerf_mlp_bwd: NULL pointer");
   return nerf_launch_wgrad(static_cast<const char*>(stash), stash_layout(n), static_cast<const char*>(workspace),
-                           bwd_layout(n), n, grads_f32, part, as_stream(stream), lo, hi);
+                           bwd_layout(n), n, grads_f32, part, as_stream(stream), lo, hi, mode, nullptr);
 }
 
 extern "C" int nerf_mlp_bwd_dgrad(const void* packed, const void* stash, const float* rgb, const float* sigma,
@@ -201,6 +203,12 @@
 extern "C" int nerf_mlp_bwd_wgrad(const void* stash, const void* workspace, int64_t n, float* grads_f32,
                                   nerf_stream_t stream) {
   return launch_wgrad(stash, workspace, n, grads_f32, 0, stream);
+}
+
+extern "C" int nerf_mlp_bwd_wgrad_deferred(const void* stash, const void* workspace, int64_t n, float* grads_f32,
+                                           nerf_stream_t stream) {
+  NERF_REQUIRE(n >= 0 && n < (int64_t)1 << 31, "nerf_mlp_bwd_wgrad_deferred: n=%lld out of range", (long long)n);
+  return launch_wgrad(stash, workspace, n, grads_f32, 0, stream, kWgradDeferSum);
 }
 
 extern "C" int64_t nerf_mlp_wgrad_part_split(void) { return plan::kW4; }
diff --git a/project-nerf_amd/csrc/mlp_pack.h b/project-nerf_amd/csrc/mlp_pack.h
--- /dev/null
+++ b/project-nerf_amd/csrc/mlp_pack.h
@@ -0,0 +1,65 @@
+#pragma once
+#include "common.h"
+#include "mlp_plan.h"
+
+namespace nerf {
+using namespace plan;
+
+struct FragTable {
+  int v[kFwdFrags + kBwdFrags];
+};
+
+constexpr FragTable make_frag_table() {
+  FragTable t{};
+  int f = 0;
+  for (int kind = 0; kind < kNumKinds; ++kind) {
+    const int ks = step_ks(kind);
+    for (int m = 0; m < step_of(kind).mt; ++m)
+      for (int k = 0; k < ks; ++k) t.v[f++] = (kind << 16) | (m << 8) | k;
+  }
+  return t;
+}
+static __constant__ FragTable g_frag_table = make_frag_table();
+
+__host__ __device__ __forceinline__ int src_index(int kind, int row, int k, bool nat) {
+  if (kind <= F_PTS7) {
+    const int l = kind;
+    const int in_dim = pts_in_dim(l);
+    int col;
+    if (l == 0) col = k < 63 ? k : -1;
+    else if (l == 4) col = nat ? (k < 63 ? 256 + k : -1) : k;
+    else col = k;
+    return col < 0 ? -1 : pts_weight_off(l) + row * in_dim + col;
+  }
+  switch (kind) {
+    case F_HEAD: return row < 256 ? kWFeat + row * 256 + k : (row == 256 ? kWSigma + k : -1);
+    case F_VIEW: return nat ? (k < 27 ? kWView + row * 283 + 256 + k : -1) : kWView + row * 283 + k;
+    case F_RGB: return row < 3 ? kWRgb + row * 128 + k : -1;
+    case B_RGB: return k < 3 ? kWRgb + k * 128 + row : -1;
+    case B_VIEW: return kWView + k * 283 + row;
+    case B_HEAD: return nat ? (k == 0 ? kWSigma + row : -1) : kWFeat + k * 256 + row;
+    default: {
+      const int l = 7 - (kind - B_PTS7);
+      return pts_weight_off(l) + k * pts_in_dim(l) + row;
+    }
+  }
+}
+
+__host__ __device__ __forceinline__ int frag_src_index(int desc, int lane, int j) {
+  const int kind = desc >> 16, mt = (desc >> 8) & 0xFF, ks = desc & 0xFF;
+  const Step st = step_of(kind);
+  const int row = mt * 32 + (lane & 31), h = lane >> 5;
+  const bool nat = ks >= st.ks_acc;
+  const int k = frag_column(nat ? ks - st.ks_acc : ks, h, j, nat);
+  return src_index(kind, row, k, nat);
+}
+
+__host__ __device__ __forceinline__ int bias_src_index(int i) {
+  if (i < 2048) return pts_bias_off(i >> 8) + (i & 255);
+  if (i < 2048 + 288) { const int r = i - 2048; return r < 256 ? kBFeat + r : (r == 256 ? kBSigma : -1); }
+  if (i < 2048 + 288 + 128) return kBView + (i - 2048 - 288);
+  const int r = i - 2048 - 288 - 128;
+  return r < 3 ? kBRgb + r : -1;
+}
+
+}
diff --git a/project-nerf_amd/csrc/mlp_pack.hip b/project-nerf_amd/csrc/mlp_pack.hip
--- a/project-nerf_amd/csrc/mlp_pack.hip
+++ b/project-nerf_amd/csrc/mlp_pack.hip
@@ -1,48 +1,7 @@
 #include "common.h"
-#include "mlp_plan.h"
+#include "mlp_pack.h"
 
 namespace nerf {
-using namespace plan;
-
-struct FragTable {
-  int v[kFwdFrags + kBwdFrags];
-};
-
-constexpr FragTable make_frag_table() {
-  FragTable t{};
-  int f = 0;
-  for (int kind = 0; kind < kNumKinds; ++kind) {
-    const int ks = step_ks(kind);
-    for (int m = 0; m < step_of(kind).mt; ++m)
-      for (int k = 0; k < ks; ++k) t.v[f++] = (kind << 16) | (m << 8) | k;
-  }
-  return t;
-}
-__constant__ FragTable g_frag_table = make_frag_table();
-
-__device__ __forceinline__ int src_index(int kind, int row, int k, bool nat) {
-  if (kind <= F_PTS7) {
-    const int l = kind;
-    const int in_dim = pts_in_dim(l);
-    int col;
-    if (l == 0) col = k < 63 ? k : -1;
-    else if (l == 4) col = nat ? (k < 63 ? 256 + k : -1) : k;
-    else col = k;
-    return col < 0 ? -1 : pts_weight_off(l) + row * in_dim + col;
-  }
-  switch (kind) {
-    case F_HEAD: return row < 256 ? kWFeat + row * 256 + k : (row == 256 ? kWSigma + k : -1);
-    case F_VIEW: return nat ? (k < 27 ? kWView + row * 283 + 256 + k : -1) : kWView + row * 283 + k;
-    case F_RGB: return row < 3 ? kWRgb + row * 128 + k : -1;
-    case B_RGB: return k < 3 ? kWRgb + k * 128 + row : -1;
-    case B_VIEW: return kWView + k * 283 + row;
-    case B_HEAD: return nat ? (k == 0 ? kWSigma + row : -1) : kWFeat + k * 256 + row;
-    default: {
-      const int l = 7 - (kind - B_PTS7);
-      return pts_weight_off(l) + k * pts_in_dim(l) + row;
-    }
-  }
-}
 
 __global__ void __launch_bounds__(256) pack16_kernel(const float* __restrict__ params, __bf16* __restrict__ packed_fwd16) {
   const int total = kFwdFrags * 64;
@@ -73,27 +32,19 @@
   for (int t = blockIdx.x * blockDim.x + threadIdx.x; t < total; t += gridDim.x * blockDim.x) {
     const int frag = t >> 6, lane = t & 63;
     const int desc = g_frag_table.v[frag];
-    const int kind = desc >> 16, mt = (desc >> 8) & 0xFF, ks = desc & 0xFF;
-    const Step st = step_of(kind);
-    const int row = mt * 32 + (lane & 31), h = lane >> 5;
-    const bool nat = ks >= st.ks_acc;
     typedef __bf16 bf16x8 __attribute__((ext_vector_type(8)));
     bf16x8 out;
 #pragma unroll
     for (int j = 0; j < 8; ++j) {
-      const int k = frag_column(nat ? ks - st.ks_acc : ks, h, j, nat);
-      const int src = src_index(kind, row, k, nat);
+      const int src = frag_src_index(desc, lane, j);
       out[j] = (__bf16)(src >= 0 ? params[src] : 0.0f);
     }
     __bf16* dst = frag < kFwdFrags ? packed_fwd + (size_t)frag * 512 : packed_bwd + (size_t)(frag - kFwdFrags) * 512;
     *reinterpret_cast<bf16x8*>(dst + lane * 8) = out;
   }
   for (int i = blockIdx.x * blockDim.x + threadIdx.x; i < kBiasFloats; i += gridDim.x * blockDim.x) {
-    float b = 0.0f;
-    if (i < 2048) b = params[pts_bias_off(i >> 8) + (i & 255)];
-    else if (i < 2048 + 288) { const int r = i - 2048; b = r < 256 ? params[kBFeat + r] : (r == 256 ? params[kBSigma] : 0.0f); }
-    else if (i < 2048 + 288 + 128) b = params[kBView + (i - 2048 - 288)];
-    else { const int r = i - 2048 - 288 - 128; b = r < 3 ? params[kBRgb + r] : 0.0f; }
+    const int src = bias_src_index(i);
+    const float b = src >= 0 ? params[src] : 0.0f;
     bias[i] = b;
   }
 }
diff --git a/project-nerf_amd/csrc/mlp_wgrad.h b/project-nerf_amd/csrc/mlp_wgrad.h
--- a/project-nerf_amd/csrc/mlp_wgrad.h
+++ b/project-nerf_amd/csrc/mlp_wgrad.h
@@ -50,6 +50,35 @@
   int debug;
 };
 
+__device__ __forceinline__ float wgrad_tile_sum(const WgradJob& job, const float* __restrict__ tile, int i) {
+  float s0 = 0.0f, s1 = 0.0f, s2 = 0.0f, s3 = 0.0f;
+  int t = 0;
+  for (; t + 4 <= job.n_parts; t += 4) {
+    s0 += tile[(long long)(t + 0) * job.p_stride + i];
+    s1 += tile[(long long)(t + 1) * job.p_stride + i];
+    s2 += tile[(long long)(t + 2) * job.p_stride + i];
+    s3 += tile[(long long)(t + 3) * job.p_stride + i];
+  }
+  for (; t < job.n_parts; ++t) s0 += tile[(long long)t * job.p_stride + i];
+  return (s0 + s1) + (s2 + s3);
+}
+__host__ __device__ __forceinline__ int wgrad_tile_elems(const WgradJob& job) { return job.o_valid * job.w_ld + job.o_valid + job.n2; }
+__host__ __device__ __forceinline__ int wgrad_tile_param(const WgradJob& job, int i) {
+  const int n_w = job.o_valid * job.w_ld, n_b = n_w + job.o_valid, n_all = n_b + job.n2;
+  return i < n_w ? job.w_off + i
+       : i < n_b ? ((job.ones || job.bias_nat_col >= 0) ? job.bias_off + (i - n_w) : -1)
+       : i < n_all - 1 ? job.w2_off + (i - n_b)
+                       : job.bias2_off;
+}
+__host__ __device__ __forceinline__ int wgrad_param_tile_elem(const WgradJob& job, int p) {
+  const int n_w = job.o_valid * job.w_ld, n_b = n_w + job.o_valid, n_all = n_b + job.n2;
+  if (p >= job.w_off && p < job.w_off + n_w) return p - job.w_off;
+  if ((job.ones || job.bias_nat_col >= 0) && p >= job.bias_off && p < job.bias_off + job.o_valid) return n_w + (p - job.bias_off);
+  if (job.n2 > 0 && p >= job.w2_off && p < job.w2_off + job.n2 - 1) return n_b + (p - job.w2_off);
+  if (job.n2 > 0 && p == job.bias2_off) return n_all - 1;
+  return -1;
+}
+
 static inline WgradJob make_job(const char* w, size_t a_off, int a_bytes, int mt_a, size_t b_off, int nt_acc, size_t bn_off, int nt_nat,
                                 int kind) {
   WgradJob j{};
@@ -68,7 +97,8 @@
   { WgradJob j = make_job(w, o.dsmall, 1024, 1, o.hc2, 2, 0, 0, 9); j.a_nat = 1; j.split_n = 1; j.w_off = c3; j.w_ld = 64; j.o_valid = 3; j.acc_valid = 64; wa.jobs[4] = j; }
 }
 
+enum WgradMode : int { kWgradAll = 0, kWgradDeferSum = 1, kWgradPlanOnly = 2 };
 int wgrad_launch(WgradArgs& args, int64_t n_samples, float* grads, hipStream_t stream, float* slab = nullptr,
-                 size_t slab_bytes = 0, size_t zero_lo = 0, size_t zero_hi = 0);
+                 size_t slab_bytes = 0, size_t zero_lo = 0, size_t zero_hi = 0, WgradMode mode = kWgradAll);
 
 }
diff --git a/project-nerf_amd/csrc/mlp_wgrad.hip b/project-nerf_amd/csrc/mlp_wgrad.hip
--- a/project-nerf_amd/csrc/mlp_wgrad.hip
+++ b/project-nerf_amd/csrc/mlp_wgrad.hip
@@ -645,24 +645,12 @@
 
 __global__ void __launch_bounds__(256) wgrad_reduce_kernel(const WgradArgs args) {
   const WgradJob& job = args.jobs[blockIdx.y];
-  const int n_w = job.o_valid * job.w_ld, n_b = n_w + job.o_valid, n_all = n_b + job.n2;
+  const int n_all = wgrad_tile_elems(job);
   const float* tile = args.slab + job.slab_off;
   for (int i = blockIdx.x * blockDim.x + threadIdx.x; i < n_all; i += gridDim.x * blockDim.x) {
-    float s0 = 0.0f, s1 = 0.0f, s2 = 0.0f, s3 = 0.0f;
-    int t = 0;
-    for (; t + 4 <= job.n_parts; t += 4) {
-      s0 += tile[(long long)(t + 0) * job.p_stride + i];
-      s1 += tile[(long long)(t + 1) * job.p_stride + i];
-      s2 += tile[(long long)(t + 2) * job.p_stride + i];
-      s3 += tile[(long long)(t + 3) * job.p_stride + i];
-    }
-    for (; t < job.n_parts; ++t) s0 += tile[(long long)t * job.p_stride + i];
-    const float sum = (s0 + s1) + (s2 + s3);
-    float* dst = i < n_w ? args.grads + job.w_off + i
-               : i < n_b ? ((job.ones || job.bias_nat_col >= 0) ? args.grads + job.bias_off + (i - n_w) : nullptr)
-               : i < n_all - 1 ? args.grads + job.w2_off + (i - n_b)
-                               : args.grads + job.bias2_off;
-    if (dst != nullptr) *dst = args.slab_accumulate ? *dst + sum : sum;
+    const float sum = wgrad_tile_sum(job, tile, i);
+    const int p = wgrad_tile_param(job, i);
+    if (p >= 0) args.grads[p] = args.slab_accumulate ? args.grads[p] + sum : sum;
   }
 }
 
@@ -671,7 +659,8 @@
 using namespace nerf;
 
 int nerf_launch_wgrad(const char* stash, const StashLayout& sl, const char* work, const BwdLayout& bl,
-                      int64_t n, float* grads, int part, hipStream_t stream, size_t zero_lo, size_t zero_hi) {
+                      int64_t n, float* grads, int part, hipStream_t stream, size_t zero_lo, size_t zero_hi, WgradMode mode,
+                      WgradArgs* plan_out) {
   WgradArgs args{};
   const size_t np = (size_t)sl.n_pad, eb = sl.fp8 ? 1 : 2;
   if (sl.fp8 != bl.fp8) return fail(NERF_EINVAL, "nerf_mlp_bwd: stash and workspace disagree on the image width");
@@ -745,11 +734,13 @@
   }
   args.n_jobs = nj;
   float* slab = bl.slab_bytes ? reinterpret_cast<float*>(const_cast<char*>(work) + bl.slab) : nullptr;
-  return wgrad_launch(args, n, grads, stream, slab, bl.slab_bytes, zero_lo, zero_hi);
+  const int rc = wgrad_launch(args, n, grads, stream, slab, bl.slab_bytes, zero_lo, zero_hi, mode);
+  if (plan_out != nullptr) *plan_out = args;
+  return rc;
 }
 
 int nerf::wgrad_launch(WgradArgs& args, int64_t n, float* grads, hipStream_t stream, float* slab, size_t slab_bytes,
-                       size_t zero_lo, size_t zero_hi) {
+                       size_t zero_lo, size_t zero_hi, WgradMode mode) {
   int nj = args.n_jobs;
   const int overhead = options().wgrad_overhead;
   for (int j = 0; j < nj; ++j) {
@@ -787,8 +778,9 @@
   int n_cu = 0;
   if (int rc = device_cu_count(&n_cu); rc != NERF_OK) return rc;
   const bool fp8 = args.amax != nullptr;
-  if (int rc = ensure_dynamic_lds(fp8 ? (const void*)mlp_wgrad_kernel<true> : (const void*)mlp_wgrad_kernel<false>, kWgLds + kWgScratch,
-                                  "nerf_mlp_bwd (wgrad)"); rc != NERF_OK) return rc;
+  if (mode != kWgradPlanOnly)
+    if (int rc = ensure_dynamic_lds(fp8 ? (const void*)mlp_wgrad_kernel<true> : (const void*)mlp_wgrad_kernel<false>, kWgLds + kWgScratch,
+                                    "nerf_mlp_bwd (wgrad)"); rc != NERF_OK) return rc;
   bool small = args.amax == nullptr && !options().wgrad_big_only, p4 = false;
   for (int j = 0; j < args.n_jobs; ++j) {
     const WgradJob& jb = args.jobs[j];
@@ -832,11 +824,12 @@
       off += (long long)count * jb.p_stride;
     }
     if (ok && (size_t)off * sizeof(float) <= slab_bytes) args.slab = slab;
-    if (args.slab != nullptr && small && hipMemsetAsync(slab, 0, (size_t)off * sizeof(float), stream) != hipSuccess)
+    if (args.slab != nullptr && small && mode != kWgradPlanOnly && hipMemsetAsync(slab, 0, (size_t)off * sizeof(float), stream) != hipSuccess)
       return fail(NERF_ELAUNCH, "tiny-MLP wgrad: memset failed");
     if (args.slab == nullptr && small) return fail(NERF_EINVAL, "tiny-MLP wgrad (option \"deterministic\"): partial tiles need %zu bytes, %zu given%s",
                                 (size_t)off * sizeof(float), slab_bytes, ok ? "" : " (a job's workgroups are not contiguous)");
   }
+  if (mode == kWgradPlanOnly) return NERF_OK;
   if (args.slab == nullptr && zero_hi > zero_lo &&
       hipMemsetAsync(grads + zero_lo, 0, sizeof(float) * (zero_hi - zero_lo), stream) != hipSuccess)
     return fail(NERF_ELAUNCH, "nerf_mlp_bwd: memset failed");
@@ -852,7 +845,7 @@
   }
   if (fp8) hipLaunchKernelGGL(mlp_wgrad_kernel<true>, dim3(grid), dim3(512), kWgLds + kWgScratch, stream, args);
   else hipLaunchKernelGGL(mlp_wgrad_kernel<false>, dim3(grid), dim3(512), kWgLds + kWgScratch, stream, args);
-  if (args.slab != nullptr) {
+  if (args.slab != nullptr && mode != kWgradDeferSum) {
     if (int rc = check_launch("nerf_mlp_bwd (wgrad)"); rc != NERF_OK) return rc;
     hipLaunchKernelGGL(wgrad_reduce_kernel, dim3(160, args.n_jobs), dim3(256), 0, stream, args);
     return check_launch("nerf_mlp_bwd (wgrad reduce)");
diff --git a/project-nerf_amd/csrc/step_tail.hip b/project-nerf_amd/csrc/step_tail.hip
--- /dev/null
+++ b/project-nerf_amd/csrc/step_tail.hip
@@ -0,0 +1,255 @@
+#include <string.h>
+#include "adam.h"
+#include "common.h"
+#include "composite_sums.h"
+#include "mlp_pack.h"
+#include "mlp_stash.h"
+#include "mlp_wgrad.h"
+
+namespace nerf {
+
+struct TailItem {
+  int p0;
+  int ld;
+  int nr, nc;
+  int frag[4];
+};
+constexpr int kTailMaxItems = 640, kTailBiasRun = 256;
+struct TailTable {
+  int n;
+  TailItem v[kTailMaxItems];
+};
+
+constexpr int tail_frag(int kind, int mt, int ks) {
+  return (kind >= B_RGB ? kFwdFrags : 0) + step_frag0(kind) + mt * step_ks(kind) + ks;
+}
+
+constexpr void tail_region(TailTable& t, int w_off, int ld, int O, int c0, int C, int fk, int f_mt0, int fks0, int bk, int b_single) {
+  for (int ot = 0; 32 * ot < O; ++ot)
+    for (int ib = 0; 32 * ib < C; ++ib) {
+      TailItem it{};
+      it.p0 = w_off + 32 * ot * ld + c0 + 32 * ib;
+      it.ld = ld;
+      it.nr = O - 32 * ot < 32 ? O - 32 * ot : 32;
+      it.nc = C - 32 * ib < 32 ? C - 32 * ib : 32;
+      it.frag[0] = tail_frag(fk, f_mt0 + ot, fks0 + 2 * ib);
+      it.frag[1] = tail_frag(fk, f_mt0 + ot, fks0 + 2 * ib + 1);
+      it.frag[2] = bk < 0 ? -1 : tail_frag(bk, ib, b_single >= 0 ? b_single : 2 * ot);
+      it.frag[3] = bk < 0 || b_single >= 0 ? -1 : tail_frag(bk, ib, 2 * ot + 1);
+      t.v[t.n++] = it;
+    }
+}
+
+constexpr TailTable make_tail_table() {
+  TailTable t{};
+  tail_region(t, kW0, 63, 256, 0, 63, F_PTS0, 0, 0, -1, -1);
+  for (int l = 1; l < 8; ++l) {
+    tail_region(t, pts_weight_off(l), pts_in_dim(l), 256, 0, 256, F_PTS0 + l, 0, 0, B_PTS7 + (7 - l), -1);
+    if (l == 4) tail_region(t, kW4, 319, 256, 256, 63, F_PTS4, 0, step_of(F_PTS4).ks_acc, -1, -1);
+  }
+  tail_region(t, kWFeat, 256, 256, 0, 256, F_HEAD, 0, 0, B_HEAD, -1);
+  tail_region(t, kWSigma, 256, 1, 0, 256, F_HEAD, 8, 0, B_HEAD, step_of(B_HEAD).ks_acc);
+  tail_region(t, kWView, 283, 128, 0, 256, F_VIEW, 0, 0, B_VIEW, -1);
+  tail_region(t, kWView, 283, 128, 256, 27, F_VIEW, 0, step_of(F_VIEW).ks_acc, -1, -1);
+  tail_region(t, kWRgb, 128, 3, 0, 128, F_RGB, 0, 0, B_RGB, 0);
+  for (int i = 0; i < kBiasFloats; i += kTailBiasRun) {
+    TailItem it{};
+    it.p0 = -1;
+    it.ld = i;
+    it.nc = kBiasFloats - i < kTailBiasRun ? kBiasFloats - i : kTailBiasRun;
+    it.frag[0] = it.frag[1] = it.frag[2] = it.frag[3] = -1;
+    t.v[t.n++] = it;
+  }
+  return t;
+}
+constexpr TailTable kTailTable = make_tail_table();
+static_assert(kTailTable.n <= kTailMaxItems, "item table");
+static __constant__ TailTable g_tail = make_tail_table();
+
+struct TailArgs {
+  WgradArgs w;
+  const float* sum_ws;
+  int n_blocks;
+  float* loss;
+  float *params, *exp_avg, *exp_avg_sq;
+  const float* grad_scale;
+  float lr, beta1, beta2, eps, wd, inv_bc1, inv_sqrt_bc2;
+  __bf16 *packed_fwd, *packed_bwd;
+  float* bias;
+};
+
+__device__ __forceinline__ float tail_step_param(const TailArgs& a, int p, int j, int e) {
+  float g;
+  if (j >= 0) {
+    const WgradJob& job = a.w.jobs[j];
+    const float sum = wgrad_tile_sum(job, a.w.slab + job.slab_off, e);
+    g = a.w.slab_accumulate ? a.w.grads[p] + sum : sum;
+    a.w.grads[p] = g;
+  } else {
+    g = a.w.grads[p];
+  }
+  const float gs = a.grad_scale ? *a.grad_scale : 1.0f;
+  float pp = a.params[p], mm = a.exp_avg[p], vv = a.exp_avg_sq[p];
+  adam_update_fused(pp, g * gs, mm, vv, a.lr, a.beta1, a.beta2, a.eps, a.wd, a.inv_bc1, a.inv_sqrt_bc2);
+  a.exp_avg[p] = mm;
+  a.exp_avg_sq[p] = vv;
+  a.params[p] = pp;
+  return pp;
+}
+
+__device__ __forceinline__ void tail_find(const TailArgs& a, int p, int& j_out, int& e_out) {
+  j_out = -1;
+  e_out = 0;
+  if (a.w.slab == nullptr) return;
+  for (int j = 0; j < a.w.n_jobs; ++j) {
+    const int e = wgrad_param_tile_elem(a.w.jobs[j], p);
+    if (e >= 0) { j_out = j; e_out = e; return; }
+  }
+}
+
+constexpr int kTailThreads = 256, kTailLd = 33;
+
+__global__ void __launch_bounds__(kTailThreads) vanilla_step_tail_kernel(const TailArgs a) {
+  __shared__ __bf16 blk[32 * kTailLd];
+  const int tid = threadIdx.x;
+  if (blockIdx.x == 0 && a.loss != nullptr) composite_sums<true>(a.sum_ws, a.n_blocks, a.loss, nullptr, nullptr);
+  for (int it = blockIdx.x; it < g_tail.n; it += gridDim.x) {
+    struct { int p0, ld, nr, nc; } item = {g_tail.v[it].p0, g_tail.v[it].ld, g_tail.v[it].nr, g_tail.v[it].nc};
+    if (item.p0 < 0) {
+      if (tid < item.nc) {
+        const int i = item.ld + tid, p = bias_src_index(i);
+        float b = 0.0f;
+        if (p >= 0) {
+          int j, e;
+          tail_find(a, p, j, e);
+          b = tail_step_param(a, p, j, e);
+        }
+        a.bias[i] = b;
+      }
+      continue;
+    }
+    int j0, e0;
+    tail_find(a, item.p0, j0, e0);
+    __syncthreads();
+    const int c = tid & 31;
+#pragma unroll
+    for (int u = 0; u < 4; ++u) {
+      const int r = (tid >> 5) + 8 * u;
+      if (r < item.nr && c < item.nc) {
+        const int d = r * item.ld + c;
+        blk[r * kTailLd + c] = (__bf16)tail_step_param(a, item.p0 + d, j0, e0 + d);
+      }
+    }
+    __syncthreads();
+    const int frag = g_tail.v[it].frag[__builtin_amdgcn_readfirstlane(tid >> 6)], lane = tid & 63;
+    if (frag < 0) continue;
+    const int desc = g_frag_table.v[frag];
+    typedef __bf16 bf16x8 __attribute__((ext_vector_type(8)));
+    bf16x8 out;
+#pragma unroll
+    for (int jj = 0; jj < 8; ++jj) {
+      const int src = frag_src_index(desc, lane, jj);
+      __bf16 val = (__bf16)0.0f;
+      if (src >= 0) {
+        const int d = src - item.p0, r = d / item.ld, cc = d - r * item.ld;
+        if (d >= 0 && r < item.nr && cc < item.nc) val = blk[r * kTailLd + cc];
+      }
+      out[jj] = val;
+    }
+    __bf16* dst = frag < kFwdFrags ? a.packed_fwd + (size_t)frag * 512 : a.packed_bwd + (size_t)(frag - kFwdFrags) * 512;
+    *reinterpret_cast<bf16x8*>(dst + lane * 8) = out;
+  }
+}
+
+}
+
+using namespace nerf;
+
+int nerf_launch_wgrad(const char* stash, const StashLayout& sl, const char* work, const BwdLayout& bl,
+                      int64_t n, float* grads, int part, hipStream_t stream, size_t zero_lo, size_t zero_hi, WgradMode mode,
+                      WgradArgs* plan_out);
+
+extern "C" int nerf_vanilla_step_tail_selfcheck(void) {
+  static const FragTable ft = make_frag_table();
+  static const TailTable tt = make_tail_table();
+  static unsigned char frag_seen[kFwdFrags + kBwdFrags], bias_seen[kBiasFloats], param_seen[kParamCount];
+  memset(frag_seen, 0, sizeof(frag_seen));
+  memset(bias_seen, 0, sizeof(bias_seen));
+  memset(param_seen, 0, sizeof(param_seen));
+  for (int it = 0; it < tt.n; ++it) {
+    const TailItem& item = tt.v[it];
+    if (item.p0 < 0) {
+      NERF_REQUIRE(item.ld >= 0 && item.nc >= 1 && item.nc <= kTailBiasRun && item.ld + item.nc <= kBiasFloats, "step tail: bias run %d out of range", it);
+      for (int i = item.ld; i < item.ld + item.nc; ++i) {
+        NERF_REQUIRE(!bias_seen[i]++, "step tail: bias entry %d in two items", i);
+        const int p = bias_src_index(i);
+        NERF_REQUIRE(p < kParamCount, "step tail: bias entry %d reads parameter %d", i, p);
+        if (p >= 0) NERF_REQUIRE(!param_seen[p]++, "step tail: parameter %d in two items", p);
+      }
+      continue;
+    }
+    NERF_REQUIRE(item.nr >= 1 && item.nr <= 32 && item.nc >= 1 && item.nc <= 32 && item.ld >= item.nc && item.p0 >= 0 &&
+                 item.p0 + (item.nr - 1) * item.ld + item.nc <= kParamCount, "step tail: block %d out of range", it);
+    for (int r = 0; r < item.nr; ++r)
+      for (int c = 0; c < item.nc; ++c) {
+        const int p = item.p0 + r * item.ld + c;
+        NERF_REQUIRE(!param_seen[p]++, "step tail: parameter %d in two items", p);
+      }
+    for (int f = 0; f < 4; ++f) {
+      const int frag = item.frag[f];
+      if (frag < 0) continue;
+      NERF_REQUIRE(frag < kFwdFrags + kBwdFrags && !frag_seen[frag]++, "step tail: fragment %d of block %d out of range or in two items", frag, it);
+      for (int lane = 0; lane < 64; ++lane)
+        for (int j = 0; j < 8; ++j) {
+          const int src = frag_src_index(ft.v[frag], lane, j);
+          if (src < 0) continue;
+          const int d = src - item.p0, r = d / item.ld, c = d - r * item.ld;
+          NERF_REQUIRE(d >= 0 && r < item.nr && c < item.nc, "step tail: fragment %d reads parameter %d outside block %d", frag, src, it);
+        }
+    }
+  }
+  for (int f = 0; f < kFwdFrags + kBwdFrags; ++f) NERF_REQUIRE(frag_seen[f] == 1, "step tail: fragment %d in no item", f);
+  for (int i = 0; i < kBiasFloats; ++i) NERF_REQUIRE(bias_seen[i] == 1, "step tail: bias entry %d in no item", i);
+  for (int p = 0; p < kParamCount; ++p) NERF_REQUIRE(param_seen[p] == 1, "step tail: parameter %d in no item", p);
+  return NERF_OK;
+}
+
+extern "C" int nerf_vanilla_step_tail_available(int64_t n) {
+  return options().step_tail != 0 && n > 0 && n < (int64_t)1 << 31 && chain_use_stream(n, true) ? 1 : 0;
+}
+
+extern "C" int nerf_vanilla_step_tail(const void* workspace, int64_t n, const float* sum_ws, int64_t n_rays, float* loss_out,
+                                      float* params, float* grads, float* exp_avg, float* exp_avg_sq, int step, float lr, float beta1,
+                                      float beta2, float eps, float weight_decay, const float* grad_scale_dev, void* packed,
+                                      nerf_stream_t stream) {
+  NERF_REQUIRE(n >= 0 && n < (int64_t)1 << 31, "nerf_vanilla_step_tail: n=%lld out of range", (long long)n);
+  NERF_REQUIRE(step >= 1, "nerf_vanilla_step_tail: step=%d (counts from 1)", step);
+  NERF_REQUIRE(n_rays >= 0, "nerf_vanilla_step_tail: n_rays=%lld", (long long)n_rays);
+  if (n == 0) return NERF_OK;
+  NERF_REQUIRE(params && grads && exp_avg && exp_avg_sq, "nerf_vanilla_step_tail: NULL pointer (params / grads / exp_avg / exp_avg_sq)");
+  NERF_REQUIRE(packed != nullptr && ((uintptr_t)packed & 255) == 0, "nerf_vanilla_step_tail: packed is NULL or not 256-byte aligned");
+  NERF_REQUIRE((loss_out == nullptr) == (sum_ws == nullptr), "nerf_vanilla_step_tail: loss_out and sum_ws go together (both or neither)");
+  NERF_REQUIRE(loss_out == nullptr || n_rays > 0, "nerf_vanilla_step_tail: n_rays=%lld with a loss to sum", (long long)n_rays);
+  const BwdLayout bl = bwd_layout(n);
+  NERF_REQUIRE(bl.slab_bytes == 0 || (workspace != nullptr && ((uintptr_t)workspace & 255) == 0),
+               "nerf_vanilla_step_tail: workspace is NULL or not 256-byte aligned (the partial tiles of n=%lld samples live there)", (long long)n);
+  TailArgs a{};
+  const char* work = static_cast<const char*>(workspace);
+  if (int rc = nerf_launch_wgrad(work, stash_layout(n), work, bl, n, grads, 0, as_stream(stream), 0, 0, kWgradPlanOnly, &a.w); rc != NERF_OK)
+    return rc;
+  if (loss_out != nullptr) {
+    a.sum_ws = sum_ws;
+    a.n_blocks = (int)composite_mse_blocks(n_rays, true);
+    a.loss = loss_out;
+  }
+  a.params = params; a.exp_avg = exp_avg; a.exp_avg_sq = exp_avg_sq;
+  a.grad_scale = grad_scale_dev;
+  a.lr = lr; a.beta1 = beta1; a.beta2 = beta2; a.eps = eps; a.wd = weight_decay;
+  adam_bias_correction(beta1, beta2, step, &a.inv_bc1, &a.inv_sqrt_bc2);
+  char* base = static_cast<char*>(packed);
+  a.packed_fwd = reinterpret_cast<__bf16*>(base + plan::kPackFwdOff);
+  a.packed_bwd = reinterpret_cast<__bf16*>(base + plan::kPackBwdOff);
+  a.bias = reinterpret_cast<float*>(base + plan::kPackBiasOff);
+  hipLaunchKernelGGL(vanilla_step_tail_kernel, dim3(kTailTable.n), dim3(kTailThreads), 0, as_stream(stream), a);
+  return check_launch("nerf_vanilla_step_tail");
+}
diff --git a/project-nerf_amd/engine.py b/project-nerf_amd/engine.py
--- a/project-nerf_amd/engine.py
+++ b/project-nerf_amd/engine.py
@@ -54,6 +54,7 @@
         self._scalars = torch.zeros(2, 1024, device=self.device)
         self._slots = LapSlots(self._scalars)
         self._infer_stale = False
+        self._tail = None
         self.grid_resolution, self.bound, self.grid_threshold = int(grid_resolution), float(bound), float(grid_threshold)
         self.grid: Optional[Tensor] = None
         self.binary_grid: Optional[Tensor] = None
@@ -106,7 +107,7 @@
                                         first_ray=first_ray)
 
     def _grid_gradients(self, rays_o: Tensor, rays_d: Tensor, target: Tensor, n_samples: int, u, sync_grads, sync_grads_async, mark,
-                        prepared) -> Tensor:
+                        prepared, defer: bool = False) -> Tensor:
         mark = mark or (lambda name: None)
         if prepared is None:
             prepared = self.prepare_batch(rays_o, rays_d, n_samples, u=u)
@@ -131,10 +132,12 @@
         stash = self._grid_buf("stash", ops.mlp_stash_bytes(n))
         rgb, sigma = ops.mlp_fwd(self.packed, pts, dirs, None, stash)
         mark("fwd")
+        ws = self._grid_buf("bwd", ops.mlp_bwd_workspace_bytes(n))
+        if defer and self._tail_allowed(n, sync_grads, sync_grads_async):
+            return self._deferred_backward(stash, rgb, sigma, z, rays_d, target, slots, ws, n, mark, lambda t: t)
         loss, amax = self._slots.take()
         d_rgb, d_sigma, _ = ops.composite_mse_bwd(rgb, sigma, z, rays_d, self.bg, target, loss, slots=slots, amax_accum=amax)
         mark("loss")
-        ws = self._grid_buf("bwd", ops.mlp_bwd_workspace_bytes(n))
         if sync_grads_async is not None:
             ops.mlp_bwd_overlapped(self.packed, stash, rgb, sigma, d_rgb, d_sigma, self.grads, ws, sync_grads_async, amax=amax, mark=mark)
         else:
@@ -146,11 +149,11 @@
 
     def compute_gradients(self, rays_o: Tensor, rays_d: Tensor, target: Tensor, n_samples: int = 64,
                    u: Optional[Tensor] = None, sync_grads=None, sync_grads_async=None, mark=None,
-                   z: Optional[Tensor] = None, grid: bool = False, prepared=None) -> Tensor:
+                   z: Optional[Tensor] = None, grid: bool = False, prepared=None, _defer: bool = False) -> Tensor:
         if grid or prepared is not None:
             if z is not None:
                 raise ValueError("compute_gradients: the grid step draws its own depths (z is for the dense step)")
-            return self._grid_gradients(rays_o, rays_d, target, n_samples, u, sync_grads, sync_grads_async, mark, prepared)
+            return self._grid_gradients(rays_o, rays_d, target, n_samples, u, sync_grads, sync_grads_async, mark, prepared, _defer)
         mark = mark or (lambda name: None)
         R = rays_o.shape[0]
         n = R * n_samples
@@ -162,6 +165,9 @@
         stash = self._buf("stash", ops.mlp_stash_bytes(n))
         rgb, sigma = ops.mlp_fwd(self.packed, rays_o, rays_d, z, stash)
         mark("fwd")
+        if _defer and self._tail_allowed(n, sync_grads, sync_grads_async):
+            return self._deferred_backward(stash, rgb.view(R, n_samples, 3), sigma.view(R, n_samples), z, rays_d, target, None,
+                                           self._buf("bwd", ops.mlp_bwd_workspace_bytes(n)), n, mark, lambda t: t.view(n, -1).squeeze(-1))
         loss, amax = self._slots.take()
         d_rgb, d_sigma, _ = ops.composite_mse_bwd(rgb.view(R, n_samples, 3), sigma.view(R, n_samples), z, rays_d, self.bg,
                                                   target, loss, amax_accum=amax)
@@ -177,6 +183,29 @@
             sync_grads(self.grads)
         return LapSlots.keep(loss)
 
+    def _tail_allowed(self, n: int, sync_grads, sync_grads_async) -> bool:
+        return sync_grads is None and sync_grads_async is None and self.world_size == 1 and ops.vanilla_step_tail_available(n)
+
+    def _loss_storage(self) -> Tensor:
+        return torch.empty(1, device=self.device)
+
+    def _deferred_backward(self, stash, rgb, sigma, z, rays_d, target, slots, ws, n, mark, flat) -> Tensor:
+        fp8 = bool(ops._lib.get_option("stash_fp8"))
+        if fp8:
+            loss, amax = self._slots.take()
+            d_rgb, d_sigma, _ = ops.composite_mse_bwd(rgb, sigma, z, rays_d, self.bg, target, loss, slots=slots, amax_accum=amax)
+            out, loss_out = None, None
+        else:
+            amax = None
+            d_rgb, d_sigma, _ = ops.composite_mse_bwd(rgb, sigma, z, rays_d, self.bg, target, None, slots=slots, defer_sums=True)
+            loss_out = self._loss_storage()
+            out = loss_out[0]
+        mark("loss")
+        ops.mlp_bwd(self.packed, stash, rgb, sigma, flat(d_rgb), flat(d_sigma), self.grads, ws, amax=amax, mark=mark, defer_sum=True)
+        mark("wgrad")
+        self._tail = (ws, n, z.shape[0], loss_out)
+        return LapSlots.keep(loss) if fp8 else out
+
     def apply_gradients(self) -> None:
         self.step_count += 1
         ops.adam_step(self.params, self.grads, self.exp_avg, self.exp_avg_sq, self.step_count, self.lr,
@@ -186,9 +215,18 @@
     def train_step(self, rays_o: Tensor, rays_d: Tensor, target: Tensor, n_samples: int = 64,
                    u: Optional[Tensor] = None, sync_grads=None, sync_grads_async=None, mark=None,
                    z: Optional[Tensor] = None, grid: bool = False, prepared=None) -> Tensor:
+        self._tail = None
         loss = self.compute_gradients(rays_o, rays_d, target, n_samples, u=u, sync_grads=sync_grads,
-                                      sync_grads_async=sync_grads_async, mark=mark, z=z, grid=grid, prepared=prepared)
-        self.apply_gradients()
+                                      sync_grads_async=sync_grads_async, mark=mark, z=z, grid=grid, prepared=prepared, _defer=True)
+        if self._tail is not None:
+            ws, n, n_rays, loss_out = self._tail
+            self._tail = None
+            self.step_count += 1
+            ops.vanilla_step_tail(ws, n, self.params, self.grads, self.exp_avg, self.exp_avg_sq, self.step_count, self.lr, self.packed,
+                                  n_rays=n_rays, loss_out=loss_out)
+            self._infer_stale = True
+        else:
+            self.apply_gradients()
         if mark is not None:
             mark("adam+pack")
         return loss
diff --git a/project-nerf_amd/ops.py b/project-nerf_amd/ops.py
--- a/project-nerf_amd/ops.py
+++ b/project-nerf_amd/ops.py
@@ -421,8 +421,8 @@
 
 
 def composite_mse_bwd(rgb: Tensor, sigma: Tensor, z: Tensor, rays_d: Tensor, bg: Optional[Tensor], target: Tensor,
-                      loss_accum: Tensor, slots: Optional[Tensor] = None, amax_accum: Optional[Tensor] = None,
-                      loss_weight: Optional[float] = None, want_pred: bool = False):
+                      loss_accum: Optional[Tensor], slots: Optional[Tensor] = None, amax_accum: Optional[Tensor] = None,
+                      loss_weight: Optional[float] = None, want_pred: bool = False, defer_sums: bool = False):
     lib = _lib.load()
     rgb, sigma, z, rays_d, target = _dev(rgb, "rgb"), _dev(sigma, "sigma"), _dev(z, "z"), _dev(rays_d, "rays_d"), _dev(target, "target")
     R, S = z.shape
@@ -431,6 +431,11 @@
     d_rgb, d_sigma = torch.empty_like(rgb), torch.empty_like(sigma)
     pred = torch.empty(R, 3, device=z.device) if want_pred else None
     w = 1.0 / (3 * R) if loss_weight is None else loss_weight
+    if defer_sums:
+        _lib.check(lib.nerf_composite_mse_bwd_deferred(_p(rgb), _p(sigma), _p(slots), _p(z), _p(rays_d), _p(bg), bg_rows, _p(target), w, R, S,
+                                                       _p(pred), _p(d_rgb), _p(d_sigma), _p(sum_ws(z.device)), _stream()),
+                   "nerf_composite_mse_bwd_deferred")
+        return d_rgb, d_sigma, pred
     _lib.check(lib.nerf_composite_mse_bwd(_p(rgb), _p(sigma), _p(slots), _p(z), _p(rays_d), _p(bg), bg_rows, _p(target), w, R, S,
                                           _p(pred), _p(loss_accum), _p(d_rgb), _p(d_sigma), _p(amax_accum), _p(sum_ws(z.device)), _stream()),
                "nerf_composite_mse_bwd")
@@ -556,7 +561,7 @@
 
 def mlp_bwd(packed: Tensor, stash: Tensor, rgb: Tensor, sigma: Tensor, d_rgb: Tensor, d_sigma: Tensor,
             grads: Optional[Tensor] = None, workspace: Optional[Tensor] = None, amax: Optional[Tensor] = None,
-            mark=None) -> Tensor:
+            mark=None, defer_sum: bool = False) -> Tensor:
     lib = _lib.load()
     rgb, sigma = _dev(rgb, "rgb"), _dev(sigma, "sigma")
     d_rgb, d_sigma = _dev(d_rgb, "d_rgb"), _dev(d_sigma, "d_sigma")
@@ -565,7 +570,7 @@
         grads = torch.empty(MLP_PARAM_COUNT, device=rgb.device, dtype=torch.float32)
     if workspace is None:
         workspace = torch.empty(lib.nerf_mlp_bwd_workspace_bytes(n), device=rgb.device, dtype=torch.uint8)
-    if amax is None:
+    if amax is None and not defer_sum:
         _lib.check(lib.nerf_mlp_bwd(_p(packed), _p(stash), _p(rgb), _p(sigma), _p(d_rgb), _p(d_sigma), n,
                                     _p(grads), _p(workspace), _stream()), "nerf_mlp_bwd")
     else:
@@ -573,7 +578,10 @@
                                              _p(workspace), _p(amax), _stream()), "nerf_mlp_bwd_dgrad_ex")
         if mark is not None:
             mark("dgrad")
-        _lib.check(lib.nerf_mlp_bwd_wgrad(_p(stash), _p(workspace), n, _p(grads), _stream()), "nerf_mlp_bwd_wgrad")
+        if defer_sum:
+            _lib.check(lib.nerf_mlp_bwd_wgrad_deferred(_p(stash), _p(workspace), n, _p(grads), _stream()), "nerf_mlp_bwd_wgrad_deferred")
+        else:
+            _lib.check(lib.nerf_mlp_bwd_wgrad(_p(stash), _p(workspace), n, _p(grads), _stream()), "nerf_mlp_bwd_wgrad")
     return grads
 
 
@@ -1042,6 +1050,24 @@
                "nerf_adam_step")
 
 
+def vanilla_step_tail_available(n: int) -> bool:
+    return bool(_lib.load().nerf_vanilla_step_tail_available(n))
+
+
+def vanilla_step_tail(workspace: Tensor, n: int, params: Tensor, grads: Tensor, exp_avg: Tensor, exp_avg_sq: Tensor, step: int,
+                      lr: float, packed: Tensor, n_rays: int = 0, loss_out: Optional[Tensor] = None, beta1: float = 0.9,
+                      beta2: float = 0.999, eps: float = 1e-8, weight_decay: float = 0.0,
+                      grad_scale: Optional[Tensor] = None) -> None:
+    lib = _lib.load()
+    for t, nm in ((params, "params"), (grads, "grads"), (exp_avg, "exp_avg"), (exp_avg_sq, "exp_avg_sq")):
+        if _dev(t, nm) is not t or t.numel() != MLP_PARAM_COUNT:
+            raise ValueError(f"{nm} must be contiguous with {MLP_PARAM_COUNT} elements")
+    sums = None if loss_out is None else sum_ws(params.device)
+    _lib.check(lib.nerf_vanilla_step_tail(_p(workspace), n, _p(sums), n_rays, _p(loss_out), _p(params), _p(grads), _p(exp_avg),
+                                          _p(exp_avg_sq), step, lr, beta1, beta2, eps, weight_decay, _p(grad_scale), _p(packed),
+                                          _stream()), "nerf_vanilla_step_tail")
+
+
 SMALL_GROUP = 65536
 
 
```

New measurement: 3.888 million rays/s, median of 2. About the same (+0.4%).
